# ODD2/DFD-CLIP

Hardware: AMD Instinct MI355X
Metric: 1-sec clips/sec (30x224x224 frames) ViT-B/16 (higher is better)
Workload: dtype bf16

## Files before the change

### dfd-clip_amd/build.py

```python
import hashlib
import os
import shutil
import subprocess
import sys
from concurrent.futures import ThreadPoolExecutor

PKG_DIR = os.path.dirname(os.path.abspath(__file__))
CSRC = os.path.join(PKG_DIR, "csrc")
OBJ_DIR = os.path.join(CSRC, "build")
LIB_PATH = os.path.join(PKG_DIR, "libdfdclip_hip.so")
INCLUDE = os.path.join(os.path.dirname(PKG_DIR), "include")
ARCH = "gfx950"
FLAGS = ["-O3", "-fPIC", "-std=c++17", f"--offload-arch={ARCH}", "-Wall", "-Wno-unused-function"]
NO_SCRATCH = {"gemm256e.hip": "gemm256e_kernel", "attention_mfma_xrow.hip": "attn_mfma_xrow_kernel"}


def _hipcc():
    exe = shutil.which("hipcc") or "/opt/rocm/bin/hipcc"
    if not os.path.exists(exe):
        raise RuntimeError("hipcc not found: the HIP kernels cannot be built")
    return exe


def sources():
    return sorted(f for f in os.listdir(CSRC) if f.endswith(".hip"))


def _digest(paths):
    h = hashlib.sha256()
    for p in paths:
        with open(p, "rb") as f:
            h.update(f.read())
    h.update(" ".join(FLAGS).encode())
    return h.hexdigest()


def scratch_users(report, kernel_substr):
    import re
    out, name = {}, None
    for line in report.splitlines():
        m = re.search(r"remark: Function Name: (\S+)", line)
        if m:
            name = m.group(1)
            continue
        m = re.search(r"ScratchSize \[bytes/lane\]: (\d+)", line)
        if m and name and kernel_substr in name and int(m.group(1)) > 0:
            out[name] = int(m.group(1))
    return out


def build(force=False, verbose=False, extra_flags=()):
    os.makedirs(OBJ_DIR, exist_ok=True)
    hipcc = _hipcc()
    headers = [os.path.join(CSRC, f) for f in sorted(os.listdir(CSRC)) if f.endswith(".hpp")]
    headers.append(os.path.join(INCLUDE, "dfdclip.h"))
    headers.append(os.path.join(INCLUDE, "dfdclip_ext.h"))
    headers.append(os.path.join(INCLUDE, "dfdclip_explain.h"))
    jobs, objs = [], []
    for src in sources():
        sp = os.path.join(CSRC, src)
        obj = os.path.join(OBJ_DIR, src[:-4] + ".o")
        stamp = obj + ".sha"
        dig = _digest([sp] + headers) + " ".join(extra_flags)
        objs.append(obj)
        if not force and os.path.exists(obj) and os.path.exists(stamp) and open(stamp).read() == dig:
            continue
        jobs.append((sp, obj, stamp, dig))

    def compile_one(job):
        sp, obj, stamp, dig = job
        guard = NO_SCRATCH.get(os.path.basename(sp))
        cmd = [hipcc, *FLAGS, *extra_flags, *(["-Rpass-analysis=kernel-resource-usage"] if guard else []), "-c", sp, "-o", obj]
        r = subprocess.run(cmd, capture_output=True, text=True)
        if r.returncode != 0:
            raise RuntimeError(f"hipcc failed for {sp}:\n{r.stderr}")
        if guard:
            bad = scratch_users(r.stderr, guard)
            if bad:
                raise RuntimeError(f"{sp}: kernels with hand-counted vmcnt waits must not use scratch, but: {bad}")
        elif verbose and r.stderr.strip():
            print(r.stderr, file=sys.stderr)
        with open(stamp, "w") as f:
            f.write(dig)
        return sp

    if jobs:
        with ThreadPoolExecutor(max_workers=min(6, len(jobs))) as ex:
            for done in ex.map(compile_one, jobs):
                if verbose:
                    print("built", os.path.basename(done))
    if jobs or not os.path.exists(LIB_PATH):
        r = subprocess.run([hipcc, "-shared", "-fPIC", f"--offload-arch={ARCH}", "-o", LIB_PATH, *objs],
                           capture_output=True, text=True)
        if r.returncode != 0:
            raise RuntimeError(f"link failed:\n{r.stderr}")
    return LIB_PATH


if __name__ == "__main__":
    print(build(force="--force" in sys.argv, verbose=True))
```

### dfd-clip_amd/capi.py

```python
import ctypes
import os
from ctypes import POINTER, Structure, c_char_p, c_double, c_float, c_int, c_int32, c_int64, c_size_t, c_uint32, c_void_p

import torch

PKG_DIR = os.path.dirname(os.path.abspath(__file__))
LIB_PATH = os.path.join(PKG_DIR, "libdfdclip_hip.so")

F32, BF16 = 0, 1
EPI_BIAS, EPI_BIAS_QUICKGELU, EPI_BIAS_RESIDUAL, EPI_PATCH_EMBED, EPI_QKV_EXPORT, EPI_RESIDUAL_POS, EPI_BIAS_GELU = range(7)
ABI_VERSION = 17

_DTYPE = {torch.float32: F32, torch.bfloat16: BF16}
FP8 = 2
FP8_MAX = 448.0
FP8_MIN_ROWS = 1024


class DfdError(RuntimeError):
    pass


GEMM_STREAM_OUT = 1
GEMM_SPARE_IF_FREE = 2


class GemmExtra(Structure):
    _fields_ = [("pos", c_void_p), ("cls", c_void_p), ("k_export", c_void_p), ("v_export", c_void_p),
                ("tokens", c_int32), ("frames_per_clip", c_int32), ("residual", c_void_p), ("qkv_first", c_int32),
                ("drop_rng", c_void_p), ("drop_site", c_uint32), ("drop_p", c_float), ("flags", c_uint32)]


OPTIM_SGD, OPTIM_ADAMW = 0, 1


class OptimExtra(Structure):
    _fields_ = [("kind", c_int32), ("reserved", c_int32), ("beta1", c_double), ("beta2", c_double), ("eps", c_double),
                ("step", c_int64), ("exp_avg_sq", c_void_p)]


class DropoutDesc(Structure):
    _fields_ = [("rng_state", c_void_p), ("site", c_uint32), ("p", c_float)]


class Dropout:
    __slots__ = ("rng", "site", "p")

    def __init__(self, rng, site, p):
        assert rng.is_cuda and rng.dtype == torch.int64 and rng.numel() == 2 and 0.0 <= p < 1.0
        self.rng, self.site, self.p = rng, int(site), float(p)

    def desc(self):
        return DropoutDesc(self.rng.data_ptr(), self.site, self.p)


def _drop(d):
    return ctypes.byref(d.desc()) if d is not None and d.p > 0 else None


SIGNATURES = {
    "dfd_last_error": (c_char_p, []),
    "dfd_abi_version": (c_int, []),
    "dfd_gemm_last_path": (c_int, []),
    "dfd_gemm_set_variant": (c_int, [c_int]),
    "dfd_dropout": (c_int, [c_void_p, c_int, c_void_p, c_int, c_int64, POINTER(DropoutDesc), c_void_p]),
    "dfd_device_check": (c_int, []),
    "dfd_layernorm": (c_int, [c_void_p, c_int64, c_void_p, c_void_p, c_void_p, c_int64, c_int, c_int64, c_int, c_float, c_float, c_void_p]),
    "dfd_layernorm2": (c_int, [c_void_p, c_int64, c_void_p, c_void_p, c_void_p, c_void_p, c_void_p, c_int64, c_int, c_int64, c_int, c_float,
                               c_float, c_void_p]),
    "dfd_add_layernorm": (c_int, [c_void_p, c_int64, c_void_p, c_void_p, c_int64, c_int, c_int, c_void_p, c_void_p, c_void_p, c_int64,
                                  c_int, c_int64, c_int, c_float, c_float, c_void_p]),
    "dfd_patchify": (c_int, [c_void_p, c_void_p, c_int, c_int, c_int, c_int, c_int, c_void_p]),
    "dfd_preprocess_u8": (c_int, [c_void_p, c_int, c_int, c_int, c_int, c_int, c_int, POINTER(c_float), POINTER(c_float),
                                  c_void_p, c_int, c_int, c_int, c_void_p]),
    "dfd_preprocess_geometry": (c_int, [c_int, c_int, c_int, POINTER(c_int), POINTER(c_int), POINTER(c_int), POINTER(c_int)]),
    "dfd_gemm": (c_int, [c_void_p, c_int64, c_void_p, c_int64, c_int, c_void_p, c_int64, c_int, c_void_p, c_int,
                         POINTER(GemmExtra), c_int64, c_int, c_int, c_void_p]),
    "dfd_gemm_fp8": (c_int, [c_void_p, c_int64, c_void_p, c_int64, c_void_p, c_int64, c_int, c_void_p, c_void_p, c_float, c_int,
                             POINTER(GemmExtra), c_int64, c_int, c_int, c_void_p]),
    "dfd_gemm_at_b_workspace": (c_size_t, [c_int64, c_int, c_int, c_int]),
    "dfd_gemm_at_b": (c_int, [c_void_p, c_int64, c_void_p, c_int64, c_int, c_void_p, c_int64, c_int, c_int, c_void_p, c_void_p]),
    "dfd_adapter_norm_gelu": (c_int, [c_void_p, c_int, c_void_p, c_int, c_void_p, c_void_p, c_int, c_int, c_int, c_int, c_float,
                                      c_void_p]),
    "dfd_attention_fwd": (c_int, [c_void_p, c_int64, c_void_p, c_int64, c_int, c_int, c_int, c_int, c_int, c_float, c_void_p]),
    "dfd_linear_rows": (c_int, [c_void_p, c_int64, c_void_p, c_void_p, c_void_p, c_int64, c_int, c_int, c_int, c_int, c_void_p]),
    "dfd_linear_rows_t_workspace": (c_size_t, [c_int, c_int, c_int]),
    "dfd_linear_rows_t": (c_int, [c_void_p, c_int64, c_void_p, c_void_p, c_void_p, c_int64, c_void_p, c_int64, c_int, c_int, c_int, c_int, c_void_p,
                                  c_void_p]),
    "dfd_decoder_attn_workspace": (c_size_t, [c_int, c_int, c_int, c_int]),
    "dfd_decoder_attn_fwd": (c_int, [c_void_p, c_void_p, c_void_p, c_int, c_void_p, c_void_p, c_void_p, c_void_p, c_void_p, c_void_p,
                                     c_void_p, c_int, c_int, c_int, c_int, c_int, c_int, c_void_p]),
    "dfd_decoder_attn_modes_fwd": (c_int, [c_void_p, c_void_p, c_int, c_void_p, c_void_p, c_int, c_void_p, c_void_p, c_int, c_int, c_int,
                                           c_int, c_int, c_void_p]),
    "dfd_decoder_attn_modes_bwd": (c_int, [c_void_p, c_void_p, c_int, c_void_p, c_void_p, c_int, c_void_p, c_void_p, c_int, c_int, c_int,
                                           c_int, c_int, c_void_p]),
    "dfd_decoder_attn_bwd_workspace": (c_size_t, [c_int, c_int, c_int, c_int]),
    "dfd_decoder_attn_bwd": (c_int, [c_void_p, c_void_p, c_void_p, c_int, c_void_p, c_void_p, c_void_p, c_void_p, c_void_p, c_void_p,
                                     c_void_p, c_void_p, c_void_p, c_void_p, c_void_p, c_int, c_void_p, c_int, c_int, c_int, c_int,
                                     c_int, c_void_p]),
    "dfd_adapter_norm_gelu_bwd_workspace": (c_size_t, [c_int, c_int, c_int, c_int]),
    "dfd_adapter_norm_gelu_bwd": (c_int, [c_void_p, c_int, c_void_p, c_void_p, c_int, c_void_p, c_void_p, c_void_p, c_void_p, c_void_p,
                                          c_int, c_int, c_int, c_int, c_float, c_void_p]),
    "dfd_linear_rows_bwd_weight": (c_int, [c_void_p, c_int64, c_void_p, c_int64, c_void_p, c_void_p, c_int, c_int, c_int, c_void_p]),
    "dfd_transpose_f32": (c_int, [c_void_p, c_void_p, c_int, c_int, c_void_p]),
    "dfd_sgd_blocks": (c_int64, [c_int64, c_int, c_int, c_int]),
    "dfd_sgd_step": (c_int, [c_void_p, c_int, c_int64, c_float, c_float, c_float, c_int, c_void_p, POINTER(OptimExtra)]),
    "dfd_layernorm_bwd": (c_int, [c_void_p, c_int64, c_void_p, c_void_p, c_int64, c_void_p, c_int64, c_void_p, c_void_p, c_void_p,
                                  c_int, c_int, c_float, c_int, c_void_p]),
    "dfd_quickgelu": (c_int, [c_void_p, c_void_p, c_void_p, c_int64, POINTER(DropoutDesc), c_void_p]),
    "dfd_head_bwd": (c_int, [c_void_p, c_void_p, c_void_p, c_void_p, c_void_p, c_void_p, c_void_p, c_void_p, c_int, c_int, c_int,
                             c_void_p]),
    "dfd_head_fwd": (c_int, [c_void_p, c_int64, c_void_p, c_void_p, c_void_p, c_void_p, c_void_p, c_void_p, c_int, c_int,
                             c_int, c_float, POINTER(DropoutDesc), c_void_p]),
    "dfd_adapter_bn_workspace": (c_size_t, [c_int64, c_int, c_int]),
    "dfd_adapter_bn_stats": (c_int, [c_void_p, c_int, c_void_p, c_void_p, c_void_p, c_void_p, c_void_p, c_int64, c_int, c_int, c_int,
                                     c_int, c_float, c_float, c_void_p]),
    "dfd_adapter_bn_apply": (c_int, [c_void_p, c_int, c_void_p, c_void_p, c_int, c_void_p, c_void_p, c_void_p, c_void_p,
                                     POINTER(DropoutDesc), c_int64, c_int, c_int, c_int, c_void_p]),
    "dfd_adapter_bn_bwd": (c_int, [c_void_p, c_void_p, c_int, c_void_p, c_int, c_void_p, c_void_p, c_void_p, c_void_p,
                                   POINTER(DropoutDesc), c_void_p, c_int64, c_int, c_int, c_int, c_int, c_void_p]),
    "dfd_gelu_erf": (c_int, [c_void_p, c_int, c_void_p, c_int, c_int64, POINTER(DropoutDesc), c_void_p]),
    "dfd_gelu_erf_bwd": (c_int, [c_void_p, c_int, c_void_p, c_int, c_void_p, c_int, c_int64, POINTER(DropoutDesc), c_void_p]),
    "dfd_compinv_loss_workspace": (c_size_t, [c_int, c_int]),
    "dfd_compinv_loss_fwd": (c_int, [c_void_p, c_void_p, c_int, c_int, c_int, c_int, c_int, c_int, c_void_p, c_void_p, c_void_p,
                                     c_void_p, c_void_p]),
    "dfd_compinv_loss_bwd": (c_int, [c_void_p, c_void_p, c_int, c_int, c_int, c_int, c_int, c_int, c_void_p, c_void_p, c_void_p,
                                     c_void_p, c_void_p, c_void_p]),
}

EXT_SIGNATURES = {
    "dfd_layernorm_dual": (c_int, [c_void_p, c_int64, c_void_p, c_void_p, c_void_p, c_int64, c_void_p, c_int64, c_int64, c_int, c_float,
                                   c_float, c_void_p]),
    "dfd_layernorm2_dual": (c_int, [c_void_p, c_int64, c_void_p, c_void_p, c_void_p, c_void_p, c_void_p, c_int64, c_void_p, c_int64,
                                    c_int64, c_int, c_float, c_float, c_void_p]),
    "dfd_add_layernorm_dual": (c_int, [c_void_p, c_int64, c_void_p, c_void_p, c_int64, c_int, c_int, c_void_p, c_void_p, c_void_p, c_int64,
                                       c_void_p, c_int64, c_int64, c_int, c_float, c_float, c_void_p]),
}

EXPLAIN_SIGNATURES = {
    "dfd_decoder_attn_map": (c_int, [c_void_p, c_void_p, c_int, c_void_p, c_void_p, c_void_p, c_void_p, c_void_p, c_void_p, c_int, c_int,
                                     c_int, c_int, c_int, c_void_p]),
}

HOOK_SIGNATURES = {
    "dfd_attention_set_variant": (c_int, [c_int]),
}

_lib = None


def load_library(path=None):
    global _lib
    if _lib is not None and path is None:
        return _lib
    path = path or LIB_PATH
    if not os.path.exists(path):
        raise DfdError(f"{path} not found: the HIP kernel library is not built and there is no fallback path")
    lib = ctypes.CDLL(path)
    for name, (res, args) in {**SIGNATURES, **EXT_SIGNATURES, **EXPLAIN_SIGNATURES, **HOOK_SIGNATURES}.items():
        try:
            fn = getattr(lib, name)
        except AttributeError:
            raise DfdError(f"{path} does not export {name}")
        fn.restype = res
        fn.argtypes = args
    if lib.dfd_abi_version() != ABI_VERSION:
        raise DfdError(f"{path}: ABI version {lib.dfd_abi_version()} != {ABI_VERSION}")
    _lib = lib
    return lib


def _check(rc, what):
    if rc != 0:
        raise DfdError(f"{what} failed ({rc}): {load_library().dfd_last_error().decode()}")


def _stream():
    return c_void_p(torch._C._cuda_getCurrentRawStream(torch._C._cuda_getDevice()))


def _ptr(t):
    return c_void_p(t.data_ptr()) if t is not None else c_void_p(0)


def _dev(*tensors):
    for t in tensors:
        if t is not None and not t.is_cuda:
            raise DfdError("HIP kernels need device tensors; got a CPU tensor (there is no CPU path)")


def _out_dtype(t):
    return FP8 if t.element_size() == 1 else _DTYPE[t.dtype]


def layernorm(x, gamma, beta, out, eps=1e-5, out_inv_scale=0.0):
    _dev(x, gamma, beta, out)
    assert x.dtype == torch.float32 and x.dim() == 2 and out.shape == x.shape
    assert x.stride(1) == 1 and out.stride(1) == 1
    _check(load_library().dfd_layernorm(_ptr(x), x.stride(0), _ptr(gamma), _ptr(beta), _ptr(out), out.stride(0),
                                        _out_dtype(out), x.shape[0], x.shape[1], eps, float(out_inv_scale), _stream()), "dfd_layernorm")
    return out


def layernorm2(x, gamma_a, beta_a, gamma_b, beta_b, out, eps=1e-5, out_inv_scale=0.0):
    _dev(x, gamma_a, beta_a, gamma_b, beta_b, out)
    assert x.dtype == torch.float32 and x.dim() == 2 and x.stride(1) == 1 and out.stride(1) == 1 and out.shape == x.shape
    _check(load_library().dfd_layernorm2(_ptr(x), x.stride(0), _ptr(gamma_a), _ptr(beta_a), _ptr(gamma_b), _ptr(beta_b), _ptr(out),
                                         out.stride(0), _out_dtype(out), x.shape[0], x.shape[1], eps, float(out_inv_scale), _stream()),
           "dfd_layernorm2")
    return out


def add_layernorm(x, delta, gamma, beta, out, eps=1e-5, delta2=None, store_x=True, out_inv_scale=0.0):
    _dev(x, delta, gamma, beta, out, delta2)
    assert x.dtype == torch.float32 and x.dim() == 2 and out.shape == x.shape and delta.shape == x.shape
    assert x.stride(1) == 1 and out.stride(1) == 1 and delta.stride(1) == 1
    assert delta2 is None or (delta2.dtype == delta.dtype and delta2.shape == x.shape and delta2.stride() == delta.stride())
    _check(load_library().dfd_add_layernorm(_ptr(x), x.stride(0), _ptr(delta), _ptr(delta2), delta.stride(0), _DTYPE[delta.dtype],
                                            int(bool(store_x)), _ptr(gamma), _ptr(beta), _ptr(out), out.stride(0), _out_dtype(out),
                                            x.shape[0], x.shape[1], eps, float(out_inv_scale), _stream()), "dfd_add_layernorm")
    return out


def _dual_outputs(x, out16, out8, out8_inv_scale):
    assert out16.dtype == torch.bfloat16 and out8.element_size() == 1 and out16.shape == x.shape and out8.shape == x.shape
    assert out16.stride(1) == 1 and out8.stride(1) == 1 and out8_inv_scale > 0


def layernorm_dual(x, gamma, beta, out16, out8, out8_inv_scale, eps=1e-5):
    _dev(x, gamma, beta, out16, out8)
    assert x.dtype == torch.float32 and x.dim() == 2 and x.stride(1) == 1
    _dual_outputs(x, out16, out8, out8_inv_scale)
    _check(load_library().dfd_layernorm_dual(_ptr(x), x.stride(0), _ptr(gamma), _ptr(beta), _ptr(out16), out16.stride(0), _ptr(out8),
                                             out8.stride(0), x.shape[0], x.shape[1], eps, float(out8_inv_scale), _stream()),
           "dfd_layernorm_dual")
    return out16, out8


def layernorm2_dual(x, gamma_a, beta_a, gamma_b, beta_b, out16, out8, out8_inv_scale, eps=1e-5):
    _dev(x, gamma_a, beta_a, gamma_b, beta_b, out16, out8)
    assert x.dtype == torch.float32 and x.dim() == 2 and x.stride(1) == 1
    _dual_outputs(x, out16, out8, out8_inv_scale)
    _check(load_library().dfd_layernorm2_dual(_ptr(x), x.stride(0), _ptr(gamma_a), _ptr(beta_a), _ptr(gamma_b), _ptr(beta_b), _ptr(out16),
                                              out16.stride(0), _ptr(out8), out8.stride(0), x.shape[0], x.shape[1], eps,
                                              float(out8_inv_scale), _stream()), "dfd_layernorm2_dual")
    return out16, out8


def add_layernorm_dual(x, delta, gamma, beta, out16, out8, out8_inv_scale, eps=1e-5, delta2=None, store_x=True):
    _dev(x, delta, gamma, beta, out16, out8, delta2)
    assert x.dtype == torch.float32 and x.dim() == 2 and delta.shape == x.shape and x.stride(1) == 1 and delta.stride(1) == 1
    assert delta2 is None or (delta2.dtype == delta.dtype and delta2.shape == x.shape and delta2.stride() == delta.stride())
    _dual_outputs(x, out16, out8, out8_inv_scale)
    _check(load_library().dfd_add_layernorm_dual(_ptr(x), x.stride(0), _ptr(delta), _ptr(delta2), delta.stride(0), _DTYPE[delta.dtype],
                                                 int(bool(store_x)), _ptr(gamma), _ptr(beta), _ptr(out16), out16.stride(0), _ptr(out8),
                                                 out8.stride(0), x.shape[0], x.shape[1], eps, float(out8_inv_scale), _stream()),
           "dfd_add_layernorm_dual")
    return out16, out8


def patchify(frames, out, res, patch):
    _dev(frames, out)
    assert frames.dtype == torch.float32 and frames.is_contiguous() and out.is_contiguous()
    n = frames.shape[0]
    _check(load_library().dfd_patchify(_ptr(frames), _ptr(out), _DTYPE[out.dtype], n, res, patch, out.shape[1], _stream()),
           "dfd_patchify")
    return out


def preprocess_geometry(in_h, in_w, res):
    v = [c_int() for _ in range(4)]
    _check(load_library().dfd_preprocess_geometry(in_h, in_w, res, *[ctypes.byref(i) for i in v]), "dfd_preprocess_geometry")
    return tuple(i.value for i in v)


def preprocess_u8(frames, out, res, patch, mean, std, antialias=True, patch_rows=True):
    _dev(frames, out)
    assert frames.dtype == torch.uint8 and frames.dim() == 4 and frames.shape[1] == 3
    assert frames.is_contiguous() and out.is_contiguous()
    n, _, h, w = frames.shape
    m3 = (c_float * 3)(*[float(v) for v in mean])
    s3 = (c_float * 3)(*[float(v) for v in std])
    if patch_rows:
        assert out.dim() == 2 and out.shape[0] == n * (res // patch) ** 2
        kpad = out.shape[1]
    else:
        assert tuple(out.shape) == (n, 3, res, res)
        kpad = 0
    _check(load_library().dfd_preprocess_u8(_ptr(frames), n, h, w, res, patch, int(bool(antialias)), m3, s3, _ptr(out),
                                            _DTYPE[out.dtype], 1 if patch_rows else 0, kpad, _stream()), "dfd_preprocess_u8")
    return out


_profile = {"epilogue": None, "events": [], "base": None}


def profile_gemm(epilogue=None):
    _profile["epilogue"] = epilogue
    _profile["events"] = []
    _profile["base"] = None
    if epilogue is not None:
        _profile["base"] = torch.cuda.Event(enable_timing=True)
        _profile["base"].record()


def profile_gemm_collect():
    base = _profile["base"]
    spans = [(base.elapsed_time(a), base.elapsed_time(b), flops) for a, b, flops in _profile["events"]]
    profile_gemm(None)
    return spans


def gemm(a, w, c, bias=None, epilogue=EPI_BIAS, m=None, pos=None, cls=None, k_export=None, v_export=None, tokens=0,
         frames_per_clip=0, residual=None, qkv_first=0, drop=None, stream_out=False, spare_cus=0, tile_blocks=0, spare_if_free=False):
    _dev(a, w, c, bias, pos, cls, k_export, v_export, residual)
    assert a.dtype == w.dtype and a.stride(1) == 1 and w.stride(1) == 1 and c.stride(1) == 1
    M = a.shape[0] if m is None else m
    N, K = w.shape
    assert a.shape[1] == K
    assert residual is None or (residual.dtype == c.dtype and residual.stride(0) == c.stride(0))
    assert drop is None or epilogue == EPI_RESIDUAL_POS
    assert 0 <= epilogue <= EPI_BIAS_GELU, f"unknown epilogue {epilogue}"
    extra = GemmExtra(_ptr(pos).value, _ptr(cls).value, _ptr(k_export).value, _ptr(v_export).value, tokens, frames_per_clip,
                      _ptr(residual).value, qkv_first, drop.rng.data_ptr() if drop is not None and drop.p > 0 else None,
                      drop.site if drop is not None else 0, drop.p if drop is not None else 0.0, (GEMM_STREAM_OUT if stream_out else 0) | (GEMM_SPARE_IF_FREE if spare_if_free else 0) | ((int(spare_cus) & 0xff) << 8) | ((int(tile_blocks) & 0xf) << 16))
    timed = _profile["epilogue"] == epilogue
    if timed:
        e0, e1 = torch.cuda.Event(enable_timing=True), torch.cuda.Event(enable_timing=True)
        e0.record()
    _check(load_library().dfd_gemm(_ptr(a), a.stride(0), _ptr(w), w.stride(0), _DTYPE[a.dtype], _ptr(c), c.stride(0),
                                   _DTYPE[c.dtype], _ptr(bias), epilogue, ctypes.byref(extra), M, N, K, _stream()), "dfd_gemm")
    if timed:
        e1.record()
        _profile["events"].append((e0, e1, 2.0 * M * N * K))
    return c


def gemm_fp8(a, w, c, col_scale, bias=None, epilogue=EPI_BIAS, m=None, out_inv_scale=0.0, pos=None, k_export=None, v_export=None,
             tokens=0, frames_per_clip=0, qkv_first=0, stream_out=False, spare_cus=0, spare_if_free=False):
    _dev(a, w, c, col_scale, bias, pos, k_export, v_export)
    assert a.element_size() == 1 and w.element_size() == 1 and a.stride(1) == 1 and w.stride(1) == 1 and c.stride(1) == 1
    assert col_scale.dtype == torch.float32 and col_scale.is_contiguous()
    M = a.shape[0] if m is None else m
    N, K = w.shape
    assert a.shape[1] == K and col_scale.numel() == N
    c_dtype = FP8 if c.element_size() == 1 else _DTYPE[c.dtype]
    extra = GemmExtra(_ptr(pos).value, None, _ptr(k_export).value, _ptr(v_export).value, tokens, frames_per_clip, None, qkv_first,
                      None, 0, 0.0, (GEMM_STREAM_OUT if stream_out else 0) | (GEMM_SPARE_IF_FREE if spare_if_free else 0) | ((int(spare_cus) & 0xff) << 8))
    timed = _profile["epilogue"] == epilogue
    if timed:
        e0, e1 = torch.cuda.Event(enable_timing=True), torch.cuda.Event(enable_timing=True)
        e0.record()
    _check(load_library().dfd_gemm_fp8(_ptr(a), a.stride(0), _ptr(w), w.stride(0), _ptr(c), c.stride(0), c_dtype, _ptr(col_scale),
                                       _ptr(bias), float(out_inv_scale), epilogue, ctypes.byref(extra), M, N, K, _stream()),
           "dfd_gemm_fp8")
    if timed:
        e1.record()
        _profile["events"].append((e0, e1, 2.0 * M * N * K))
    return c


def gemm_set_variant(variant):
    return load_library().dfd_gemm_set_variant(int(variant))


def gemm_last_path():
    return load_library().dfd_gemm_last_path()


def gemm_at_b_workspace_bytes(R, Ma, Nb, dtype):
    return load_library().dfd_gemm_at_b_workspace(R, Ma, Nb, _DTYPE[dtype])


def gemm_at_b(a, b, c, workspace):
    _dev(a, b, c, workspace)
    assert a.dtype == b.dtype and a.stride(1) == 1 and b.stride(1) == 1 and c.is_contiguous() and c.dtype == torch.float32
    R, Ma = a.shape
    Nb = b.shape[1]
    assert b.shape[0] == R and tuple(c.shape) == (Ma, Nb)
    assert workspace.numel() * workspace.element_size() >= gemm_at_b_workspace_bytes(R, Ma, Nb, a.dtype)
    _check(load_library().dfd_gemm_at_b(_ptr(a), a.stride(0), _ptr(b), b.stride(0), _DTYPE[a.dtype], _ptr(c), R, Ma, Nb,
                                        _ptr(workspace), _stream()), "dfd_gemm_at_b")
    return c


def adapter_norm_gelu(a, y, weight, bias, frames, patches, x, joint, eps=1e-5):
    _dev(a, y, weight, bias)
    assert (a.dtype == y.dtype or a.dtype == torch.float32) and a.is_contiguous() and y.is_contiguous()
    assert weight.is_contiguous() and bias.is_contiguous()
    _check(load_library().dfd_adapter_norm_gelu(_ptr(a), _DTYPE[a.dtype], _ptr(y), _DTYPE[y.dtype], _ptr(weight), _ptr(bias), frames,
                                                patches, x, int(joint), eps, _stream()), "dfd_adapter_norm_gelu")
    return y


def adapter_norm_gelu_bwd_workspace_bytes(frames, patches, x, joint):
    return load_library().dfd_adapter_norm_gelu_bwd_workspace(frames, patches, x, int(joint))


def adapter_norm_gelu_bwd(a, dy, da, weight, bias, dweight, dbias, workspace, frames, patches, x, joint, eps=1e-5):
    _dev(a, dy, da, weight, bias, dweight, dbias, workspace)
    assert dy.dtype == da.dtype and (a.dtype == dy.dtype or a.dtype == torch.float32)
    assert a.is_contiguous() and dy.is_contiguous() and da.is_contiguous()
    _check(load_library().dfd_adapter_norm_gelu_bwd(_ptr(a), _DTYPE[a.dtype], _ptr(dy), _ptr(da), _DTYPE[dy.dtype], _ptr(weight), _ptr(bias),
                                                    _ptr(dweight), _ptr(dbias), _ptr(workspace), frames, patches, x, int(joint),
                                                    eps, _stream()), "dfd_adapter_norm_gelu_bwd")
    return da


def attention_set_variant(variant):
    return load_library().dfd_attention_set_variant(int(variant))


def attention_fwd(qkv, out, n_frames, tokens, heads, head_dim=64):
    _dev(qkv, out)
    assert qkv.dtype == out.dtype and qkv.stride(1) == 1 and out.stride(1) == 1
    _check(load_library().dfd_attention_fwd(_ptr(qkv), qkv.stride(0), _ptr(out), out.stride(0), _DTYPE[qkv.dtype], n_frames,
                                            tokens, heads, head_dim, head_dim ** -0.5, _stream()), "dfd_attention_fwd")
    return out


def linear_rows(x, w, bias, y, epilogue=EPI_BIAS):
    _dev(x, w, bias, y)
    assert x.dtype == torch.float32 and w.dtype == torch.float32 and y.dtype == torch.float32
    assert x.stride(1) == 1 and y.stride(1) == 1 and w.is_contiguous()
    B, K = x.shape
    N = w.shape[0]
    _check(load_library().dfd_linear_rows(_ptr(x), x.stride(0), _ptr(w), _ptr(bias), _ptr(y), y.stride(0), epilogue, B, N, K,
                                          _stream()), "dfd_linear_rows")
    return y


def linear_rows_t_workspace_bytes(B, N, K):
    return load_library().dfd_linear_rows_t_workspace(B, N, K)


def linear_rows_t(x, wt, bias, y, workspace, epilogue=EPI_BIAS, residual=None):
    _dev(x, wt, bias, y, workspace, residual)
    assert residual is None or (residual.dtype == torch.float32 and residual.stride(1) == 1 and residual.shape == y.shape)
    assert x.dtype == torch.float32 and wt.dtype == torch.float32 and y.dtype == torch.float32
    assert x.stride(1) == 1 and y.stride(1) == 1 and wt.is_contiguous()
    B, K = x.shape
    N = wt.shape[1]
    assert wt.shape[0] == K and workspace.numel() * workspace.element_size() >= linear_rows_t_workspace_bytes(B, N, K)
    _check(load_library().dfd_linear_rows_t(_ptr(x), x.stride(0), _ptr(wt), _ptr(bias), _ptr(residual),
                                            residual.stride(0) if residual is not None else 0, _ptr(y), y.stride(0), epilogue, B, N, K,
                                            _ptr(workspace), _stream()), "dfd_linear_rows_t")
    return y


def decoder_attn_workspace_bytes(B, heads, d, splits):
    return load_library().dfd_decoder_attn_workspace(B, heads, d, splits)


class KvLayoutDesc(ctypes.Structure):
    _fields_ = [("row_stride", c_int64), ("frame_stride", c_int64), ("pos", c_void_p)]


def _kv_layout(x, other, pos, B, T, patches, D):
    if other is not None:
        assert other.dtype == x.dtype and other.shape == x.shape and other.stride() == x.stride()
    if x.is_contiguous() and pos is None:
        assert x.numel() == B * T * patches * D
        return None, None
    if x.is_contiguous():
        rs, fs = D, patches * D
    else:
        assert x.dim() == 3 and x.shape == (B * T, patches, D) and x.stride(2) == 1, "strided K/V must be [B*T, patches, D] views"
        fs, rs = x.stride(0), x.stride(1)
    if pos is not None:
        assert pos.dtype == torch.float32 and pos.is_contiguous() and pos.shape == (T, D) and pos.device == x.device
    lay = KvLayoutDesc(rs, fs, pos.data_ptr() if pos is not None else None)
    return ctypes.byref(lay), lay


def decoder_attn_fwd(q, k, v, frame_mask, mix, stats, workspace, splits, B, T, patches, heads, d=64, mix_softmax=None,
                     ext_weights=None, pos=None):
    _dev(q, k, v, frame_mask, mix, stats, workspace, mix_softmax, ext_weights)
    assert q.dtype == torch.float32 and q.is_contiguous()
    assert frame_mask.dtype == torch.uint8 and frame_mask.is_contiguous()
    assert ext_weights is None or (ext_weights.is_contiguous() and ext_weights.numel() == B * heads * T * patches)
    lay, _keep = _kv_layout(k, v, pos, B, T, patches, heads * d)
    _check(load_library().dfd_decoder_attn_fwd(_ptr(q), _ptr(k), _ptr(v), _DTYPE[k.dtype], lay, _ptr(frame_mask), _ptr(ext_weights),
                                               _ptr(mix), _ptr(mix_softmax), _ptr(stats), _ptr(workspace), splits, B, T, patches,
                                               heads, d, _stream()),
           "dfd_decoder_attn_fwd")
    return mix


ATTN_MODE_BITS = {"frame": 1, "temporal": 2}


def decoder_attn_modes_fwd(q, k, frame_mask, modes, scores, weights, B, T, patches, heads, d=64, pos=None):
    _dev(q, k, frame_mask, scores, weights)
    assert q.is_contiguous() and scores.is_contiguous() and weights.is_contiguous()
    assert scores.numel() == B * heads * T * patches == weights.numel()
    lay, _keep = _kv_layout(k, None, pos, B, T, patches, heads * d)
    _check(load_library().dfd_decoder_attn_modes_fwd(_ptr(q), _ptr(k), _DTYPE[k.dtype], lay, _ptr(frame_mask), modes, _ptr(scores),
                                                     _ptr(weights), B, T, patches, heads, d, _stream()),
           "dfd_decoder_attn_modes_fwd")
    return weights


def decoder_attn_map(q, k, frame_mask, stats, aff, B, T, patches, heads, d=64, ext_weights=None, branches=None, pos=None):
    _dev(q, k, frame_mask, stats, aff, ext_weights, branches)
    assert q.dtype == torch.float32 and q.is_contiguous()
    assert frame_mask.dtype == torch.uint8 and frame_mask.is_contiguous()
    n = B * heads * T * patches
    assert aff.dtype == torch.float32 and aff.is_contiguous() and aff.numel() == n
    assert stats is None or (stats.dtype == torch.float32 and stats.is_contiguous() and stats.numel() == B * heads * 2)
    assert ext_weights is None or (ext_weights.dtype == torch.float32 and ext_weights.is_contiguous() and ext_weights.numel() == n)
    assert branches is None or (branches.dtype == torch.float32 and branches.is_contiguous() and branches.numel() == 2 * n)
    lay, _keep = _kv_layout(k, None, pos, B, T, patches, heads * d)
    _check(load_library().dfd_decoder_attn_map(_ptr(q), _ptr(k), _DTYPE[k.dtype], lay, _ptr(frame_mask), _ptr(stats), _ptr(ext_weights),
                                               _ptr(aff), _ptr(branches), B, T, patches, heads, d, _stream()),
           "dfd_decoder_attn_map")
    return aff


def decoder_attn_modes_bwd(scores, v, dmix, modes, dwv_ws, dscores, B, T, patches, heads, d=64, pos=None):
    _dev(scores, v, dmix, dwv_ws, dscores)
    assert scores.is_contiguous() and dmix.is_contiguous()
    assert dwv_ws.numel() >= B * heads * T * patches and dscores.numel() == B * heads * T * patches
    lay, _keep = _kv_layout(v, None, pos, B, T, patches, heads * d)
    _check(load_library().dfd_decoder_attn_modes_bwd(_ptr(scores), _ptr(v), _DTYPE[v.dtype], lay, _ptr(dmix), modes, _ptr(dwv_ws),
                                                     _ptr(dscores), B, T, patches, heads, d, _stream()),
           "dfd_decoder_attn_modes_bwd")
    return dscores


def head_fwd(x, gamma, beta, proj, feat, raw, logits, eps=1e-5, drop=None):
    _dev(x, gamma, beta, proj, feat, raw, logits)
    B, D = x.shape
    assert proj.is_contiguous() and proj.shape[0] == D and feat.is_contiguous()
    _check(load_library().dfd_head_fwd(_ptr(x), x.stride(0), _ptr(gamma), _ptr(beta), _ptr(proj), _ptr(feat), _ptr(raw),
                                       _ptr(logits), B, D, proj.shape[1], eps, _drop(drop), _stream()), "dfd_head_fwd")
    return logits



BN_EVAL, BN_TRAIN, BN_TRAIN_UPDATE = 0, 1, 2


def adapter_bn_workspace_bytes(frames, patches, width):
    return load_library().dfd_adapter_bn_workspace(frames, patches, width)


def _bn_shape(t, frames, patches, width):
    assert t.is_contiguous() and t.numel() == frames * patches * width, (tuple(t.shape), frames, patches, width)


def adapter_bn_stats(y, stats, workspace, frames, patches, T, mode, running_mean=None, running_var=None,
                     num_batches_tracked=None, momentum=0.1, eps=1e-5):
    _dev(y, stats, workspace, running_mean, running_var, num_batches_tracked)
    width = y.shape[-1]
    _bn_shape(y, frames, patches, width)
    assert stats.dtype == torch.float32 and stats.is_contiguous() and stats.numel() == 2 * T
    for b in (running_mean, running_var):
        assert b is None or (b.dtype == torch.float32 and b.is_contiguous() and b.numel() == T)
    assert num_batches_tracked is None or num_batches_tracked.dtype == torch.int64
    assert workspace.numel() * workspace.element_size() >= adapter_bn_workspace_bytes(frames, patches, width)
    _check(load_library().dfd_adapter_bn_stats(_ptr(y), _DTYPE[y.dtype], _ptr(stats), _ptr(running_mean), _ptr(running_var),
                                               _ptr(num_batches_tracked), _ptr(workspace), frames, patches, width, T, int(mode),
                                               momentum, eps, _stream()), "dfd_adapter_bn_stats")
    return stats


def adapter_bn_apply(y, out, frames, patches, T, stats=None, gamma=None, beta=None, residual=None, pos=None, drop=None):
    _dev(y, out, stats, gamma, beta, residual, pos)
    width = y.shape[-1]
    _bn_shape(y, frames, patches, width)
    _bn_shape(out, frames, patches, width)
    assert residual is None or (residual.dtype == out.dtype and residual.is_contiguous() and residual.numel() == out.numel())
    assert pos is None or (pos.dtype == torch.float32 and pos.is_contiguous() and pos.numel() == T * width)
    _check(load_library().dfd_adapter_bn_apply(_ptr(y), _DTYPE[y.dtype], _ptr(residual), _ptr(out), _DTYPE[out.dtype], _ptr(stats),
                                               _ptr(gamma), _ptr(beta), _ptr(pos), _drop(drop), frames, patches, width, T,
                                               _stream()), "dfd_adapter_bn_apply")
    return out


def adapter_bn_bwd(y, dout, dy, stats, gamma, dgamma, dbeta, workspace, frames, patches, T, train, drop=None):
    _dev(y, dout, dy, stats, gamma, dgamma, dbeta, workspace)
    width = y.shape[-1]
    for t in (y, dout, dy):
        _bn_shape(t, frames, patches, width)
    assert dy.dtype == y.dtype and dout.dtype in (y.dtype, torch.float32)
    assert workspace.numel() * workspace.element_size() >= adapter_bn_workspace_bytes(frames, patches, width)
    _check(load_library().dfd_adapter_bn_bwd(_ptr(y), _ptr(dout), _DTYPE[dout.dtype], _ptr(dy), _DTYPE[y.dtype], _ptr(stats),
                                             _ptr(gamma), _ptr(dgamma), _ptr(dbeta), _drop(drop), _ptr(workspace), frames,
                                             patches, width, T, int(bool(train)), _stream()), "dfd_adapter_bn_bwd")
    return dy


def gelu_erf(a, out, drop=None):
    _dev(a, out)
    assert a.is_contiguous() and out.is_contiguous() and a.numel() == out.numel()
    _check(load_library().dfd_gelu_erf(_ptr(a), _DTYPE[a.dtype], _ptr(out), _DTYPE[out.dtype], a.numel(), _drop(drop), _stream()),
           "dfd_gelu_erf")
    return out


def gelu_erf_bwd(a, dh, da, drop=None):
    _dev(a, dh, da)
    assert a.is_contiguous() and dh.is_contiguous() and da.is_contiguous() and a.numel() == dh.numel() == da.numel()
    assert dh.dtype == da.dtype
    _check(load_library().dfd_gelu_erf_bwd(_ptr(a), _DTYPE[a.dtype], _ptr(dh), _DTYPE[dh.dtype], _ptr(da), _DTYPE[da.dtype], a.numel(),
                                           _drop(drop), _stream()), "dfd_gelu_erf_bwd")
    return da


def dropout(x, out, drop):
    _dev(x, out)
    assert x.is_contiguous() and out.is_contiguous() and x.numel() == out.numel() and drop is not None
    _check(load_library().dfd_dropout(_ptr(x), _DTYPE[x.dtype], _ptr(out), _DTYPE[out.dtype], x.numel(),
                                      ctypes.byref(drop.desc()), _stream()), "dfd_dropout")
    return out



def decoder_attn_bwd_workspace_bytes(B, T, heads, d=64):
    return load_library().dfd_decoder_attn_bwd_workspace(B, T, heads, d)


def decoder_attn_bwd(q, k, v, frame_mask, dmix, mix_softmax, stats, dq, dpos, workspace, B, T, patches, heads, d=64, dk=None,
                     dv=None, ext_weights=None, ext_dscores=None, pos=None):
    _dev(q, k, v, frame_mask, dmix, mix_softmax, stats, dq, dpos, workspace, dk, dv, ext_weights, ext_dscores)
    assert q.is_contiguous() and dmix.is_contiguous()
    assert mix_softmax is None or mix_softmax.is_contiguous()
    lay, _keep = _kv_layout(k, v, pos, B, T, patches, heads * d)
    _check(load_library().dfd_decoder_attn_bwd(_ptr(q), _ptr(k), _ptr(v), _DTYPE[k.dtype], lay, _ptr(frame_mask), _ptr(dmix),
                                               _ptr(mix_softmax), _ptr(stats), _ptr(ext_weights), _ptr(ext_dscores), _ptr(dq),
                                               _ptr(dpos), _ptr(dk), _ptr(dv),
                                               _DTYPE[dk.dtype] if dk is not None else F32, _ptr(workspace), B, T, patches,
                                               heads, d, _stream()), "dfd_decoder_attn_bwd")
    return dq


def linear_rows_bwd_weight(dy, x, dw, db=None):
    _dev(dy, x, dw, db)
    assert dy.stride(1) == 1 and x.stride(1) == 1 and dw.is_contiguous()
    B, N = dy.shape
    K = x.shape[1]
    assert tuple(dw.shape) == (N, K)
    _check(load_library().dfd_linear_rows_bwd_weight(_ptr(dy), dy.stride(0), _ptr(x), x.stride(0), _ptr(dw), _ptr(db), B, N, K,
                                                     _stream()), "dfd_linear_rows_bwd_weight")
    return dw


def transpose(src, dst):
    _dev(src, dst)
    assert src.is_contiguous() and dst.is_contiguous() and src.dtype == torch.float32
    R, C = src.shape
    _check(load_library().dfd_transpose_f32(_ptr(src), _ptr(dst), R, C, _stream()), "dfd_transpose_f32")
    return dst


def sgd_blocks(numel, rows=0, cols=0, mirrored=False):
    return int(load_library().dfd_sgd_blocks(int(numel), int(rows), int(cols), 1 if mirrored else 0))


def adamw_extra(beta1, beta2, eps, step, exp_avg_sq):
    _dev(exp_avg_sq)
    assert exp_avg_sq.dtype == torch.int64 and exp_avg_sq.is_contiguous() and exp_avg_sq.dim() == 1
    return OptimExtra(OPTIM_ADAMW, 0, float(beta1), float(beta2), float(eps), int(step), exp_avg_sq.data_ptr())


def sgd_step(table, n, total_blocks, lr, momentum, weight_decay, first_step, extra=None):
    _dev(table)
    assert table.dtype == torch.int64 and table.is_contiguous() and table.shape == (n, 7)
    _check(load_library().dfd_sgd_step(_ptr(table), int(n), int(total_blocks), float(lr), float(momentum), float(weight_decay),
                                       1 if first_step else 0, _stream(), None if extra is None else ctypes.byref(extra)), "dfd_sgd_step")


def layernorm_bwd(x, gamma, dy, dx, dgamma, dbeta, xhat_ws, accumulate_dx=False, eps=1e-5):
    _dev(x, gamma, dy, dx, dgamma, dbeta, xhat_ws)
    rows, cols = x.shape
    _check(load_library().dfd_layernorm_bwd(_ptr(x), x.stride(0), _ptr(gamma), _ptr(dy), dy.stride(0), _ptr(dx), dx.stride(0),
                                            _ptr(dgamma), _ptr(dbeta), _ptr(xhat_ws), rows, cols, eps, int(accumulate_dx),
                                            _stream()), "dfd_layernorm_bwd")
    return dx


def quickgelu(u, out, du=None, drop=None):
    _dev(u, out, du)
    assert u.is_contiguous() and out.is_contiguous() and (du is None or du.is_contiguous())
    _check(load_library().dfd_quickgelu(_ptr(u), _ptr(du), _ptr(out), u.numel(), _drop(drop), _stream()), "dfd_quickgelu")
    return out


def head_bwd(raw, dlogits, proj, feat, dfeat_ext, dz, dfeat, dproj):
    _dev(raw, dlogits, proj, feat, dfeat_ext, dz, dfeat, dproj)
    B, od = raw.shape
    D = proj.shape[0]
    assert dlogits.is_contiguous() and proj.is_contiguous() and feat.is_contiguous()
    _check(load_library().dfd_head_bwd(_ptr(raw), _ptr(dlogits), _ptr(proj), _ptr(feat), _ptr(dfeat_ext), _ptr(dz), _ptr(dfeat),
                                       _ptr(dproj), B, D, od, _stream()), "dfd_head_bwd")
    return dfeat



def compinv_loss_workspace_bytes(P, D):
    return int(load_library().dfd_compinv_loss_workspace(int(P), int(D)))


def _compinv_check(k, v, B, T, P, L):
    assert k.dtype == v.dtype and k.shape == v.shape and k.is_contiguous() and v.is_contiguous()
    assert k.dim() == 3 and k.shape[0] == L and k.shape[1] == B * T * P, (tuple(k.shape), B, T, P, L)


def compinv_loss_fwd(k, v, B, T, P, workspace, match, norm, recon=None):
    _dev(k, v, workspace, match, norm, recon)
    L, _, D = k.shape
    _compinv_check(k, v, B, T, P, L)
    assert workspace.dtype == torch.float32 and workspace.numel() * 4 >= compinv_loss_workspace_bytes(P, D)
    assert match.dtype == norm.dtype == torch.float32 and (recon is None or recon.dtype == torch.float32)
    _check(load_library().dfd_compinv_loss_fwd(_ptr(k), _ptr(v), _DTYPE[k.dtype], B, T, P, D, L, _ptr(workspace), _ptr(match),
                                               _ptr(norm), _ptr(recon), _stream()), "dfd_compinv_loss_fwd")
    return match


def compinv_loss_bwd(k, v, B, T, P, workspace, norm, grad, dk, dv):
    _dev(k, v, workspace, norm, grad, dk, dv)
    L, _, D = k.shape
    _compinv_check(k, v, B, T, P, L)
    assert dk.dtype == dv.dtype == k.dtype and dk.shape == dv.shape == k.shape and dk.is_contiguous() and dv.is_contiguous()
    assert grad.dtype == norm.dtype == torch.float32 and grad.numel() == 1 and norm.numel() == 1
    _check(load_library().dfd_compinv_loss_bwd(_ptr(k), _ptr(v), _DTYPE[k.dtype], B, T, P, D, L, _ptr(workspace), _ptr(norm),
                                               _ptr(grad), _ptr(dk), _ptr(dv), _stream()), "dfd_compinv_loss_bwd")
    return dk, dv
```

### dfd-clip_amd/csrc/gemm.hip

```cpp
#include "gemm_args.hpp"
#include "gelu.hpp"

namespace {

constexpr int BM = 128, BN = 128;
constexpr int ROW_BYTES = 64;
constexpr int ROW_STRIDE = 80;
constexpr int TILE_BYTES = BM * ROW_STRIDE;
constexpr int EPI_SPLITK_SLAB = 100;

template <typename CT> __device__ __forceinline__ void store_c(void* C, int64_t off, float v) {
  static_cast<CT*>(C)[off] = from_f32<CT>(v);
}

template <typename CT, int EPI>
__device__ __forceinline__ void epilogue_elem(const GemmArgs& a, int64_t m, int n, float acc) {
  if (m >= a.M || n >= a.N) return;
  if constexpr (EPI == DFD_EPI_BIAS) {
    store_c<CT>(a.C, m * a.ldc + n, acc + (a.bias ? a.bias[n] : 0.f));
  } else if constexpr (EPI == DFD_EPI_BIAS_QUICKGELU) {
    store_c<CT>(a.C, m * a.ldc + n, quick_gelu(acc + (a.bias ? a.bias[n] : 0.f)));
  } else if constexpr (EPI == DFD_EPI_BIAS_GELU) {
    store_c<CT>(a.C, m * a.ldc + n, gelu_erf(acc + (a.bias ? a.bias[n] : 0.f)));
  } else if constexpr (EPI == DFD_EPI_BIAS_RESIDUAL) {
    float* c = static_cast<float*>(a.C) + m * a.ldc + n;
    *c = *c + (acc + (a.bias ? a.bias[n] : 0.f));
  } else if constexpr (EPI == DFD_EPI_PATCH_EMBED) {
    const int P = a.tokens - 1;
    const int64_t frame = m / P;
    const int p = (int)(m - frame * P);
    float* c = static_cast<float*>(a.C);
    c[(frame * a.tokens + 1 + p) * a.ldc + n] = acc + a.pos[(int64_t)(1 + p) * a.N + n];
    if (p == 0) c[(frame * a.tokens) * a.ldc + n] = a.cls[n] + a.pos[n];
  } else if constexpr (EPI == DFD_EPI_RESIDUAL_POS) {
    const int64_t frame = m / (a.tokens - 1);
    const float p = a.pos ? a.pos[(frame % a.frames_per_clip) * a.N + n] : 0.f;
    CT* c = static_cast<CT*>(a.C) + m * a.ldc + n;
    const CT* rsd = a.residual ? static_cast<const CT*>(a.residual) + m * a.ldc + n : c;
    *c = from_f32<CT>(to_f32(*rsd) + dfd_drop_one(a.drop, (uint64_t)m * a.N + n, acc) + p);
  } else if constexpr (EPI == DFD_EPI_QKV_EXPORT) {
    const float v = acc + (a.bias ? a.bias[n] : 0.f);
    store_c<CT>(a.C, m * a.ldc + n, v);
    const int D = a.N / (3 - a.qkv_first);
    const int ne = n + a.qkv_first * D;
    if (a.k_export != nullptr && ne >= D) {
      const int64_t frame = m / a.tokens;
      const int tok = (int)(m - frame * a.tokens);
      if (tok > 0) {
        const bool is_v = ne >= 2 * D;
        const int cc = ne - (is_v ? 2 * D : D);
        const float e = v + (a.pos ? a.pos[(frame % a.frames_per_clip) * D + cc] : 0.f);
        store_c<CT>(is_v ? a.v_export : a.k_export, (frame * (a.tokens - 1) + tok - 1) * D + cc, e);
      }
    }
  }
}

template <typename T, typename CT, int EPI>
__global__ __launch_bounds__(256) void gemm128_kernel(const GemmArgs a) {
  __shared__ __attribute__((aligned(16))) unsigned char smem[4 * TILE_BYTES];
  const int tid = threadIdx.x;
  const int lane = tid & 63, wave = tid >> 6;
  const int r = lane & 31, h = lane >> 5;
  const int wm = wave >> 1, wn = wave & 1;
  const int64_t m0 = (int64_t)blockIdx.y * BM;
  const int n0 = blockIdx.x * BN;
  constexpr int KSTEP = ROW_BYTES / (int)sizeof(T);
  const int nk_all = a.K / KSTEP;
  const int per = (nk_all + (int)gridDim.z - 1) / (int)gridDim.z;
  const int kt0 = (int)blockIdx.z * per;
  const int nk = min(per, nk_all - kt0) > 0 ? min(per, nk_all - kt0) : 0;

  const unsigned char* Ab = static_cast<const unsigned char*>(a.A);
  const unsigned char* Wb = static_cast<const unsigned char*>(a.W);
  uint4 ra[2], rb[2];
  int srow[2], scol[2];
  bool va[2], vb[2];
  const unsigned char* pa[2];
  const unsigned char* pb[2];
#pragma unroll
  for (int i = 0; i < 2; ++i) {
    const int c = tid + 256 * i;
    srow[i] = c >> 2;
    scol[i] = (c & 3) * 16;
    va[i] = (m0 + srow[i]) < a.M;
    vb[i] = (n0 + srow[i]) < a.N;
    pa[i] = Ab + ((m0 + srow[i]) * a.lda) * (int64_t)sizeof(T) + scol[i];
    pb[i] = Wb + ((int64_t)(n0 + srow[i]) * a.ldw) * (int64_t)sizeof(T) + scol[i];
  }
  auto load_tile = [&](int kt) {
#pragma unroll
    for (int i = 0; i < 2; ++i) {
      ra[i] = va[i] ? *reinterpret_cast<const uint4*>(pa[i] + (int64_t)(kt0 + kt) * ROW_BYTES) : uint4{0, 0, 0, 0};
      rb[i] = vb[i] ? *reinterpret_cast<const uint4*>(pb[i] + (int64_t)(kt0 + kt) * ROW_BYTES) : uint4{0, 0, 0, 0};
    }
  };
  auto store_tile = [&](int buf) {
#pragma unroll
    for (int i = 0; i < 2; ++i) {
      *reinterpret_cast<uint4*>(smem + buf * TILE_BYTES + srow[i] * ROW_STRIDE + scol[i]) = ra[i];
      *reinterpret_cast<uint4*>(smem + (2 + buf) * TILE_BYTES + srow[i] * ROW_STRIDE + scol[i]) = rb[i];
    }
  };

  f32x16 acc[2][2];
#pragma unroll
  for (int i = 0; i < 2; ++i)
#pragma unroll
    for (int j = 0; j < 2; ++j)
#pragma unroll
      for (int e = 0; e < 16; ++e) acc[i][j][e] = 0.f;

  if (nk > 0) {
    load_tile(0);
    store_tile(0);
  }
  __syncthreads();
  for (int kt = 0; kt < nk; ++kt) {
    const int buf = kt & 1;
    if (kt + 1 < nk) load_tile(kt + 1);
    const unsigned char* As = smem + buf * TILE_BYTES + (wm * 64 + r) * ROW_STRIDE;
    const unsigned char* Bs = smem + (2 + buf) * TILE_BYTES + (wn * 64 + r) * ROW_STRIDE;
    if constexpr (sizeof(T) == 2) {
#pragma unroll
      for (int s = 0; s < 2; ++s) {
        bf16x8 fa[2], fb[2];
#pragma unroll
        for (int i = 0; i < 2; ++i) {
          fa[i] = *reinterpret_cast<const bf16x8*>(As + i * 32 * ROW_STRIDE + s * 32 + h * 16);
          fb[i] = *reinterpret_cast<const bf16x8*>(Bs + i * 32 * ROW_STRIDE + s * 32 + h * 16);
        }
#pragma unroll
        for (int i = 0; i < 2; ++i)
#pragma unroll
          for (int j = 0; j < 2; ++j) acc[i][j] = __builtin_amdgcn_mfma_f32_32x32x16_bf16(fa[i], fb[j], acc[i][j], 0, 0, 0);
      }
    } else {
      f32x4 fa[2][2], fb[2][2];
#pragma unroll
      for (int i = 0; i < 2; ++i)
#pragma unroll
        for (int q = 0; q < 2; ++q) {
          fa[i][q] = *reinterpret_cast<const f32x4*>(As + i * 32 * ROW_STRIDE + h * 32 + q * 16);
          fb[i][q] = *reinterpret_cast<const f32x4*>(Bs + i * 32 * ROW_STRIDE + h * 32 + q * 16);
        }
#pragma unroll
      for (int s = 0; s < 8; ++s)
#pragma unroll
        for (int i = 0; i < 2; ++i)
#pragma unroll
          for (int j = 0; j < 2; ++j)
            acc[i][j] = __builtin_amdgcn_mfma_f32_32x32x2f32(fa[i][s >> 2][s & 3], fb[j][s >> 2][s & 3], acc[i][j], 0, 0, 0);
    }
    if (kt + 1 < nk) store_tile(buf ^ 1);
    __syncthreads();
  }

#pragma unroll
  for (int i = 0; i < 2; ++i)
#pragma unroll
    for (int j = 0; j < 2; ++j)
#pragma unroll
      for (int e = 0; e < 16; ++e) {
        const int64_t m = m0 + wm * 64 + i * 32 + (e & 3) + 8 * (e >> 2) + 4 * h;
        const int n = n0 + wn * 64 + j * 32 + r;
        if constexpr (EPI == EPI_SPLITK_SLAB) {
          if (m < a.M && n < a.N) static_cast<float*>(a.C)[((int64_t)blockIdx.z * a.M + m) * a.ldc + n] = acc[i][j][e];
        } else {
          epilogue_elem<CT, EPI>(a, m, n, acc[i][j][e]);
        }
      }
}

template <typename T, typename CT>
int launch_gemm128(const GemmArgs& a, int epi, hipStream_t st) {
  const dim3 grid((a.N + BN - 1) / BN, (unsigned)((a.M + BM - 1) / BM)), block(256);
#define EPI_CASE(E)                                                                    \
  case E:                                                                              \
    hipLaunchKernelGGL((gemm128_kernel<T, CT, E>), grid, block, 0, st, a);             \
    break;
  switch (epi) {
    EPI_CASE(DFD_EPI_BIAS)
    EPI_CASE(DFD_EPI_BIAS_QUICKGELU)
    EPI_CASE(DFD_EPI_BIAS_GELU)
    EPI_CASE(DFD_EPI_QKV_EXPORT)
    EPI_CASE(DFD_EPI_RESIDUAL_POS)
    default:
      if constexpr (sizeof(CT) == 4) {
        switch (epi) {
          EPI_CASE(DFD_EPI_BIAS_RESIDUAL)
          EPI_CASE(DFD_EPI_PATCH_EMBED)
          default:
            dfd_set_error("dfd_gemm: unknown epilogue %d", epi);
            return DFD_ERR_INVALID_ARG;
        }
      } else {
        dfd_set_error("dfd_gemm: epilogue %d needs an f32 C", epi);
        return DFD_ERR_INVALID_ARG;
      }
  }
#undef EPI_CASE
  DFD_CHECK_LAUNCH("dfd_gemm");
  return DFD_OK;
}

template <typename T>
__global__ __launch_bounds__(256) void transpose_pad_kernel(const T* __restrict__ src, int64_t lds_, T* __restrict__ dst, int64_t R,
                                                            int C, int64_t Rp) {
  __shared__ T tile[32][33];
  const int c0 = blockIdx.x * 32;
  const int64_t r0 = (int64_t)blockIdx.y * 32;
  const int tx = threadIdx.x & 31, ty = threadIdx.x >> 5;
  for (int i = ty; i < 32; i += 8) tile[i][tx] = (r0 + i < R && c0 + tx < C) ? src[(r0 + i) * lds_ + c0 + tx] : from_f32<T>(0.f);
  __syncthreads();
  for (int i = ty; i < 32; i += 8)
    if (c0 + i < C && r0 + tx < Rp) dst[(int64_t)(c0 + i) * Rp + r0 + tx] = tile[tx][i];
}

__global__ void slab_reduce_kernel(const float* __restrict__ slabs, float* __restrict__ out, int64_t n, int splits) {
  const int64_t i = (int64_t)blockIdx.x * blockDim.x + threadIdx.x;
  if (i >= n) return;
  float s = 0.f;
  for (int z = 0; z < splits; ++z) s += slabs[(int64_t)z * n + i];
  out[i] = s;
}

void at_b_plan(int64_t R, int Ma, int Nb, int64_t* Rp, int* splits) {
  const int tiles = ((Ma + BM - 1) / BM) * ((Nb + BN - 1) / BN);
  int sp = (1024 + tiles - 1) / tiles;
  const int64_t steps = (R + 31) / 32;
  if (sp > steps / 8) sp = (int)(steps / 8 > 0 ? steps / 8 : 1);
  if (sp > 512) sp = 512;
  *splits = sp;
  *Rp = (R + 31) / 32 * 32;
}

template <typename T>
int launch_at_b(const void* A, int64_t lda, const void* B, int64_t ldb, float* C, int64_t R, int Ma, int Nb, void* workspace,
                hipStream_t st) {
  int64_t Rp;
  int splits;
  at_b_plan(R, Ma, Nb, &Rp, &splits);
  T* At = static_cast<T*>(workspace);
  T* Bt = At + (int64_t)Ma * Rp;
  size_t off = (size_t)(Ma + Nb) * Rp * sizeof(T);
  off = (off + 255) / 256 * 256;
  float* slabs = reinterpret_cast<float*>(static_cast<unsigned char*>(workspace) + off);
  const dim3 tb(256);
  hipLaunchKernelGGL((transpose_pad_kernel<T>), dim3((Ma + 31) / 32, (unsigned)(Rp / 32)), tb, 0, st, static_cast<const T*>(A), lda, At, R, Ma, Rp);
  hipLaunchKernelGGL((transpose_pad_kernel<T>), dim3((Nb + 31) / 32, (unsigned)(Rp / 32)), tb, 0, st, static_cast<const T*>(B), ldb, Bt, R, Nb, Rp);
  GemmArgs a{};
  a.A = At; a.W = Bt; a.C = slabs; a.lda = Rp; a.ldw = Rp; a.ldc = Nb; a.M = Ma; a.N = Nb; a.K = (int)Rp;
  const dim3 grid((Nb + BN - 1) / BN, (Ma + BM - 1) / BM, splits);
  hipLaunchKernelGGL((gemm128_kernel<T, float, EPI_SPLITK_SLAB>), grid, tb, 0, st, a);
  const int64_t n = (int64_t)Ma * Nb;
  hipLaunchKernelGGL(slab_reduce_kernel, dim3((unsigned)((n + 255) / 256)), tb, 0, st, slabs, C, n, splits);
  DFD_CHECK_LAUNCH("dfd_gemm_at_b");
  return DFD_OK;
}

}

static int fill_extra(GemmArgs& a, int epilogue, const dfd_gemm_extra* extra, int c_dtype, int64_t ldc, int64_t M, int N) {
  if (epilogue == DFD_EPI_PATCH_EMBED) {
    DFD_REQUIRE(extra && extra->pos && extra->cls && extra->tokens > 1, "dfd_gemm: PATCH_EMBED needs extra.pos, extra.cls, extra.tokens");
    DFD_REQUIRE(M % (extra->tokens - 1) == 0, "dfd_gemm: PATCH_EMBED M=%lld is not a whole number of frames", (long long)M);
    DFD_REQUIRE(c_dtype == DFD_F32 && ldc >= N, "dfd_gemm: PATCH_EMBED writes an f32 token matrix");
  } else {
    DFD_REQUIRE(ldc >= N, "dfd_gemm: ldc=%lld < N", (long long)ldc);
  }
  if (epilogue == DFD_EPI_QKV_EXPORT) {
    DFD_REQUIRE(extra && extra->tokens > 1 && (extra->qkv_first == 0 || extra->qkv_first == 1) && N % (3 - extra->qkv_first) == 0,
                "dfd_gemm: QKV_EXPORT needs extra.tokens, qkv_first in {0, 1} and N a multiple of the column blocks present");
    DFD_REQUIRE(M % extra->tokens == 0, "dfd_gemm: QKV_EXPORT M=%lld is not a whole number of frames", (long long)M);
    DFD_REQUIRE(!extra->k_export == !extra->v_export, "dfd_gemm: QKV_EXPORT needs both k_export and v_export or neither");
    DFD_REQUIRE(!extra->pos || extra->frames_per_clip > 0, "dfd_gemm: QKV_EXPORT with pos needs frames_per_clip");
  }
  if (epilogue == DFD_EPI_RESIDUAL_POS) {
    DFD_REQUIRE(extra && extra->tokens > 1, "dfd_gemm: RESIDUAL_POS needs extra.tokens (patches per frame + 1)");
    DFD_REQUIRE(!extra->pos || extra->frames_per_clip > 0, "dfd_gemm: RESIDUAL_POS with pos needs frames_per_clip");
  }
  if (extra) {
    a.pos = extra->pos; a.cls = extra->cls; a.k_export = extra->k_export; a.v_export = extra->v_export;
    a.residual = epilogue == DFD_EPI_RESIDUAL_POS ? extra->residual : nullptr;
    a.tokens = extra->tokens; a.frames_per_clip = extra->frames_per_clip > 0 ? extra->frames_per_clip : 1;
    a.qkv_first = epilogue == DFD_EPI_QKV_EXPORT ? extra->qkv_first : 0;
    a.stream_out = (extra->flags & DFD_GEMM_STREAM_OUT) ? 1 : 0;
    a.spare_cus = (int)((extra->flags >> DFD_GEMM_SPARE_CUS_SHIFT) & 0xff);
    a.spare_if_free = (extra->flags & DFD_GEMM_SPARE_IF_FREE) ? 1 : 0;
    a.tile_rows = 32 * (int)((extra->flags >> DFD_GEMM_TILE_BLOCKS_SHIFT) & 0xf);
    DFD_REQUIRE(a.tile_rows == 0 || a.tile_rows == 224 || a.tile_rows == 256, "dfd_gemm: tile blocks must be 0, 7 or 8");
    if (epilogue == DFD_EPI_RESIDUAL_POS && extra->drop_rng && extra->drop_p > 0.f) {
      DFD_REQUIRE(extra->drop_p < 1.f, "dfd_gemm: drop_p=%f", (double)extra->drop_p);
      const dfd_dropout_t dd{extra->drop_rng, extra->drop_site, extra->drop_p};
      a.drop = dfd_make_drop(&dd);
    }
  }
  return DFD_OK;
}

static thread_local int g_last_path = 0;
static thread_local int g_gemm_variant = 0;
extern "C" int dfd_gemm_last_path(void) { return g_last_path; }
extern "C" int dfd_gemm_set_variant(int variant) {
  const int old = g_gemm_variant;
  g_gemm_variant = variant;
  return old;
}

static int try_persistent_kernels(GemmArgs& a, int c_dtype, int epilogue, bool f8, hipStream_t st, int* path) {
  const int epi_p = epilogue == DFD_EPI_QKV_EXPORT && a.k_export == nullptr ? DFD_EPI_BIAS : epilogue;
  a.no_dynamic = g_gemm_variant != 3;
  int rc = g_gemm_variant == 1 ? 1 : (f8 ? dfd_gemm256e_f8_try : dfd_gemm256e_try)(a, c_dtype, epi_p, st);
  *path = 257;
  if (rc != 1) return rc;
  rc = (f8 ? dfd_gemm256p_f8_try : dfd_gemm256p_try)(a, c_dtype, epi_p, st);
  *path = 256;
  return rc;
}

extern "C" int dfd_gemm(const void* A, int64_t lda, const void* W, int64_t ldw, int ab_dtype, void* C, int64_t ldc,
                        int c_dtype, const float* bias, int epilogue, const dfd_gemm_extra* extra, int64_t M, int N,
                        int K, void* stream) {
  DFD_REQUIRE(A && W && C, "dfd_gemm: null pointer");
  DFD_REQUIRE(M >= 0 && N > 0 && K > 0, "dfd_gemm: bad shape M=%lld N=%d K=%d", (long long)M, N, K);
  DFD_REQUIRE(ab_dtype == DFD_F32 || ab_dtype == DFD_BF16, "dfd_gemm: ab_dtype=%d", ab_dtype);
  DFD_REQUIRE(c_dtype == DFD_F32 || c_dtype == DFD_BF16, "dfd_gemm: c_dtype=%d", c_dtype);
  DFD_REQUIRE(!(ab_dtype == DFD_F32 && c_dtype == DFD_BF16), "dfd_gemm: f32 operands with bf16 output unsupported");
  DFD_REQUIRE(K % 32 == 0, "dfd_gemm: K=%d must be a multiple of 32", K);
  const int esz = ab_dtype == DFD_F32 ? 4 : 2;
  DFD_REQUIRE(lda >= K && ldw >= K && (lda * esz) % 16 == 0 && (ldw * esz) % 16 == 0, "dfd_gemm: lda=%lld ldw=%lld must be >= K and 16-byte multiples", (long long)lda, (long long)ldw);
  DFD_REQUIRE(dfd_aligned16(A) && dfd_aligned16(W), "dfd_gemm: A and W must be 16-byte aligned");
  GemmArgs a{};
  a.A = A; a.W = W; a.C = C; a.bias = bias;
  a.lda = lda; a.ldw = ldw; a.ldc = ldc; a.M = M; a.N = N; a.K = K;
  { const int rc = fill_extra(a, epilogue, extra, c_dtype, ldc, M, N); if (rc != DFD_OK) return rc; }
  if (M == 0) return DFD_OK;
  hipStream_t st = static_cast<hipStream_t>(stream);
  if (ab_dtype == DFD_BF16) {
    int path = 0;
    int rc = try_persistent_kernels(a, c_dtype, epilogue, false, st, &path);
    if (rc == 0) g_last_path = path;
    if (rc <= 0) return rc;
    rc = dfd_gemm256_try(a, c_dtype, epilogue, st);
    if (rc == 0) g_last_path = 256;
    if (rc <= 0) return rc;
  }
  g_last_path = 128;
  if (ab_dtype == DFD_F32) return launch_gemm128<float, float>(a, epilogue, st);
  if (c_dtype == DFD_BF16) return launch_gemm128<bf16_t, bf16_t>(a, epilogue, st);
  return launch_gemm128<bf16_t, float>(a, epilogue, st);
}

extern "C" int dfd_gemm_fp8(const void* A, int64_t lda, const void* W, int64_t ldw, void* C, int64_t ldc, int c_dtype,
                            const float* col_scale, const float* bias, float out_inv_scale, int epilogue,
                            const dfd_gemm_extra* extra, int64_t M, int N, int K, void* stream) {
  DFD_REQUIRE(A && W && C && col_scale, "dfd_gemm_fp8: null pointer");
  DFD_REQUIRE(M >= 0 && N > 0 && K > 0, "dfd_gemm_fp8: bad shape M=%lld N=%d K=%d", (long long)M, N, K);
  DFD_REQUIRE(c_dtype == DFD_BF16 || c_dtype == DFD_FP8, "dfd_gemm_fp8: c_dtype=%d", c_dtype);
  DFD_REQUIRE(epilogue == DFD_EPI_BIAS || epilogue == DFD_EPI_BIAS_QUICKGELU || epilogue == DFD_EPI_BIAS_GELU || epilogue == DFD_EPI_QKV_EXPORT,
              "dfd_gemm_fp8: epilogue %d not served (BIAS, BIAS_QUICKGELU, BIAS_GELU, QKV_EXPORT)", epilogue);
  DFD_REQUIRE(c_dtype == DFD_BF16 || (epilogue != DFD_EPI_QKV_EXPORT && out_inv_scale > 0.f), "dfd_gemm_fp8: fp8 output needs out_inv_scale > 0 and a plain / QuickGELU / GELU epilogue");
  DFD_REQUIRE(lda >= K && ldw >= K && ldc >= N, "dfd_gemm_fp8: leading dimensions");
  GemmArgs a{};
  a.A = A; a.W = W; a.C = C; a.bias = bias; a.col_scale = col_scale; a.out_inv_scale = out_inv_scale;
  a.lda = lda; a.ldw = ldw; a.ldc = ldc; a.M = M; a.N = N; a.K = K;
  { const int rc = fill_extra(a, epilogue, extra, c_dtype, ldc, M, N); if (rc != DFD_OK) return rc; }
  if (M == 0) return DFD_OK;
  int path = 0;
  const int rc = try_persistent_kernels(a, c_dtype, epilogue, true, static_cast<hipStream_t>(stream), &path);
  if (rc == 1) {
    dfd_set_error("dfd_gemm_fp8: shape not served (needs M >= 1024, N %% 256 == 0, K %% 128 == 0, K >= 256, 16-byte aligned rows; got M=%lld N=%d K=%d)",
                  (long long)M, N, K);
    return DFD_ERR_INVALID_ARG;
  }
  return rc;
}

bool dfd_gemm_tn_supported(const void* A, int64_t lda, const void* B, int64_t ldb, int Ma, int Nb);
int dfd_gemm_tn_splits(int64_t R, int Ma, int Nb);
int dfd_gemm_tn_launch(const void* A, int64_t lda, const void* B, int64_t ldb, float* C, int64_t R, int Ma, int Nb,
                       float* slabs, hipStream_t st);

extern "C" size_t dfd_gemm_at_b_workspace(int64_t R, int Ma, int Nb, int dtype) {
  if (R <= 0 || Ma <= 0 || Nb <= 0) return 0;
  int64_t Rp;
  int splits;
  at_b_plan(R, Ma, Nb, &Rp, &splits);
  const size_t esz = dtype == DFD_F32 ? 4 : 2;
  size_t bytes = (size_t)(Ma + Nb) * Rp * esz;
  bytes = (bytes + 255) / 256 * 256;
  bytes += (size_t)splits * Ma * Nb * sizeof(float) + 256;
  if (dtype == DFD_BF16 && Ma % 128 == 0 && Nb % 128 == 0) {
    const size_t tn = (size_t)dfd_gemm_tn_splits(R, Ma, Nb) * Ma * Nb * sizeof(float) + 256;
    if (tn > bytes) bytes = tn;
  }
  return bytes;
}

extern "C" int dfd_gemm_at_b(const void* A, int64_t lda, const void* B, int64_t ldb, int dtype, float* C, int64_t R, int Ma,
                             int Nb, void* workspace, void* stream) {
  DFD_REQUIRE(A && B && C && workspace, "dfd_gemm_at_b: null pointer");
  DFD_REQUIRE(R > 0 && Ma > 0 && Nb > 0 && lda >= Ma && ldb >= Nb, "dfd_gemm_at_b: bad shape");
  DFD_REQUIRE(R < (int64_t)1 << 31, "dfd_gemm_at_b: R too large");
  DFD_REQUIRE(dtype == DFD_F32 || dtype == DFD_BF16, "dfd_gemm_at_b: dtype=%d", dtype);
  DFD_REQUIRE((reinterpret_cast<uintptr_t>(workspace) & 255) == 0, "dfd_gemm_at_b: workspace must be 256-byte aligned");
  hipStream_t st = static_cast<hipStream_t>(stream);
  if (dtype == DFD_BF16 && dfd_gemm_tn_supported(A, lda, B, ldb, Ma, Nb))
    return dfd_gemm_tn_launch(A, lda, B, ldb, C, R, Ma, Nb, static_cast<float*>(workspace), st);
  if (dtype == DFD_F32) return launch_at_b<float>(A, lda, B, ldb, C, R, Ma, Nb, workspace, st);
  return launch_at_b<bf16_t>(A, lda, B, ldb, C, R, Ma, Nb, workspace, st);
}
```

### dfd-clip_amd/csrc/gemm256e.hip

```cpp
#include <mutex>
#include <unordered_map>

#include "gemm256p_common.hpp"

namespace {

constexpr int UNIT = 128 * ROWB;
constexpr int DEPTH = 6;
constexpr int NB = 2 * (DEPTH - 1);

template <int EPI, int RB, bool F8, bool CF8>
__global__ __launch_bounds__(512) void gemm256e_kernel(const GemmArgs a, int tiles_m, int tiles_n) {
  static_assert(!F8 || RB == 8, "fp8 form: 256-row tiles only");
  static_assert(!CF8 || (F8 && EPI != DFD_EPI_QKV_EXPORT), "fp8 output: fp8 operands, plain, QuickGELU or GELU epilogue");
  constexpr int ESZ = F8 ? 1 : 2;
  constexpr int TMU = 32 * RB;
  constexpr int WROWS = 16 * RB;
  constexpr int HB = RB - 4;
  constexpr int NCV = F8 ? 2 : 1;
  constexpr int S1 = CF8 ? RB : 2 * RB;
  constexpr int S2 = 4 * RB;
  __shared__ __attribute__((aligned(1024))) unsigned char smem[RING + 8 * STAGE];
  const int tid = threadIdx.x;
  const int lane = tid & 63;
  const int wave = __builtin_amdgcn_readfirstlane(tid >> 6);
  const int wr = wave >> 2, wc = wave & 3;
  const int ntiles = tiles_m * tiles_n;

  const int G = gridDim.x, bid = blockIdx.x;
  const int xcd = bid & 7, q8 = G >> 3, r8 = G & 7;
  const int pos = xcd_position();

  const OperandSrds<F8, CF8> srd(a);
  const __amdgpu_buffer_rsrc_t srdA = srd.A, srdW = srd.W, srdC = srd.C;
  const v4i srdB = words(a.bias ? a.bias : reinterpret_cast<const float*>(a.W), a.bias ? a.N * 4 : 0);
  [[maybe_unused]] const v4i srdS = words(F8 ? a.col_scale : reinterpret_cast<const float*>(a.W), F8 ? a.N * 4 : 0);
  const int cnt_x = q8 + (xcd < r8 ? 1 : 0), off_x = pos - (bid >> 3);
  const v4i srdT = words(reinterpret_cast<const float*>(a.sched ? a.sched : reinterpret_cast<const uint32_t*>(a.W)), a.sched ? 8 * 128 : 0);

  const uint32_t lda2 = (uint32_t)(a.lda * ESZ), ldw2 = (uint32_t)(a.ldw * ESZ);
  const uint32_t a_last = (uint32_t)(a.M - 1) * lda2;
  uint32_t vA[2][2], vW[2];
  auto set_a = [&](const Tile& t, int ha) {
    int l = lane;
    asm volatile("" : "+v"(l));
    const uint32_t pr = (uint32_t)(l >> 3), pp = (uint32_t)(l & 7);
    const uint32_t ch0 = (pp ^ (pr >> 1)) << 4;
    const uint32_t row0 = ((uint32_t)t.m0 + (uint32_t)(WROWS * (wave >> 2) + 64 * ha + 16 * (wave & 3))) * lda2 + pr * lda2;
    vA[ha][0] = min(row0, a_last) + ch0;
    vA[ha][1] = min(row0 + 8u * lda2, a_last) + (ch0 ^ 64u);
  };
  auto set_w = [&](const Tile& t, int hb) {
    int l = lane;
    asm volatile("" : "+v"(l));
    const uint32_t pr = (uint32_t)(l >> 3), pp = (uint32_t)(l & 7);
    const uint32_t ch0 = (pp ^ (pr >> 1)) << 4;
    vW[hb] = ((uint32_t)t.n0 + (uint32_t)(64 * (wave >> 1) + 32 * hb + 16 * (wave & 1))) * ldw2 + pr * ldw2 + ch0;
  };
  auto issue = [&](int kind, int kr) {
    unsigned char* d = smem + ((kind & 1) ? 0 : 4 * UNIT) + (2 * (kind >> 1) + (kr & 1)) * UNIT + wave * 16 * ROWB;
    if (kind & 1) {
      __builtin_amdgcn_raw_ptr_buffer_load_lds(srdA, (lds_ptr_t)d, 16, vA[kind >> 1][0], kr * ROWB, 0, 0);
      __builtin_amdgcn_raw_ptr_buffer_load_lds(srdA, (lds_ptr_t)(d + 8 * ROWB), 16, vA[kind >> 1][1], kr * ROWB, 0, 0);
    } else {
      __builtin_amdgcn_raw_ptr_buffer_load_lds(srdW, (lds_ptr_t)d, 16, vW[kind >> 1], kr * ROWB, 0, 0);
      __builtin_amdgcn_raw_ptr_buffer_load_lds(srdW, (lds_ptr_t)(d + 8 * ROWB), 16, vW[kind >> 1] ^ 64u, kr * ROWB + 8 * (int)ldw2, 0, 0);
    }
  };

  const unsigned char* rdA[2];
  const unsigned char* rdW[2];
  {
    const int fr = lane & 15, fq = lane >> 4;
    const int sw = (fr >> 1) & 7;
#pragma unroll
    for (int ks = 0; ks < 2; ++ks) {
      const int cs = ((4 * ks + fq) ^ sw) << 4;
      rdA[ks] = smem + (wr * 64 + fr) * ROWB + cs;
      rdW[ks] = smem + 4 * UNIT + (wc * 32 + fr) * ROWB + cs;
    }
  }

  struct Opnd {
    v8i v;
  };
  Opnd Aa[4], X[2], Y[2];
  f32x4 acc[RB][4];
  auto read_op = [&](Opnd& o, const unsigned char* p0, const unsigned char* p1) {
    const v4i x0 = *reinterpret_cast<const v4i*>(p0), x1 = *reinterpret_cast<const v4i*>(p1);
    o.v = v8i{x0[0], x0[1], x0[2], x0[3], x1[0], x1[1], x1[2], x1[3]};
  };
  auto read_a = [&](int slot, int ha) {
#pragma unroll
    for (int i = 0; i < 4; ++i)
      if (ha == 0 || i < HB) read_op(Aa[i], rdA[0] + (2 * ha + slot) * UNIT + i * 16 * ROWB, rdA[1] + (2 * ha + slot) * UNIT + i * 16 * ROWB);
  };
  auto read_w = [&](Opnd (&w)[2], int slot, int hb) {
#pragma unroll
    for (int j = 0; j < 2; ++j) read_op(w[j], rdW[0] + (2 * hb + slot) * UNIT + j * 16 * ROWB, rdW[1] + (2 * hb + slot) * UNIT + j * 16 * ROWB);
  };
  auto chunk = [](const Opnd& o, int ks) {
    return __builtin_bit_cast(bf16x8, ks == 0 ? __builtin_shufflevector(o.v, o.v, 0, 1, 2, 3) : __builtin_shufflevector(o.v, o.v, 4, 5, 6, 7));
  };
  auto quadrant = [&](const Opnd (&w)[2], int ha, int hb) {
    asm volatile("s_waitcnt lgkmcnt(0)" ::: "memory");
    __builtin_amdgcn_sched_barrier(0);
    __builtin_amdgcn_s_setprio(1);
    if constexpr (F8) {
#pragma unroll
      for (int i = 0; i < 4; ++i)
#pragma unroll
        for (int j = 0; j < 2; ++j)
          acc[4 * ha + i][2 * hb + j] = __builtin_amdgcn_mfma_scale_f32_16x16x128_f8f6f4(w[j].v, Aa[i].v, acc[4 * ha + i][2 * hb + j], 0, 0, 0, 0x7f7f7f7f, 0,
                                                                                          0x7f7f7f7f);
#pragma unroll
      for (int i = 0; i < 4; ++i)
#pragma unroll
        for (int j = 0; j < 2; ++j) asm volatile("" : "+v"(acc[4 * ha + i][2 * hb + j]));
    } else {
#pragma unroll
      for (int ks = 0; ks < 2; ++ks)
#pragma unroll
        for (int i = 0; i < (ha == 0 ? 4 : HB); ++i)
#pragma unroll
          for (int j = 0; j < 2; ++j)
            acc[4 * ha + i][2 * hb + j] = __builtin_amdgcn_mfma_f32_16x16x32_bf16(chunk(w[j], ks), chunk(Aa[i], ks), acc[4 * ha + i][2 * hb + j], 0, 0, 0);
    }
    __builtin_amdgcn_s_setprio(0);
    __builtin_amdgcn_sched_barrier(0);
    __builtin_amdgcn_s_barrier();
    __builtin_amdgcn_sched_barrier(0);
  };

  const int nk = a.K / (F8 ? 128 : TK);
  int idx = pos;
  Tile cur = decode_tile(idx, tiles_m, tiles_n, TMU);
  set_a(cur, 0);
  set_a(cur, 1);
  set_w(cur, 0);
  set_w(cur, 1);
#pragma unroll
  for (int v = 0; v <= DEPTH; ++v) issue(v & 3, v >> 2);
  wait_vm<NB>();
  __builtin_amdgcn_s_barrier();
  if (wr == 1) __builtin_amdgcn_s_barrier();
  __builtin_amdgcn_sched_barrier(0);
  int s_prev = 0;

  [[maybe_unused]] unsigned char* const ep = smem + RING + wave * STAGE;
  const int D = EPI == DFD_EPI_QKV_EXPORT ? a.N / (3 - a.qkv_first) : 0;

  const int nk_ = a.K / (F8 ? 128 : TK);
  const bool dyn = !F8 && a.sched != nullptr && nk_ >= 6;
  const bool drawer = dyn && wave == 0;
  for (;;) {
    int nidx = idx + G;
    bool has_next = nidx < ntiles;
    Tile nxt = has_next ? decode_tile(nidx, tiles_m, tiles_n, TMU) : cur;
    uint32_t drawn = 1;
    if (drawer) {
      const uint32_t coff = (uint32_t)(xcd * 128);
      uint64_t saved_exec;
      asm volatile(
          "s_mov_b64 %1, exec\n\t"
          "s_mov_b64 exec, 1\n\t"
          "s_nop 4\n\t"
          "buffer_atomic_add %0, %2, %3, 0 offen sc0\n\t"
          "s_mov_b64 exec, %1"
          : "+v"(drawn), "=&s"(saved_exec)
          : "v"(coff), "s"(srdT)
          : "memory");
    }
#pragma unroll
    for (int i = 0; i < RB; ++i)
#pragma unroll
      for (int j = 0; j < 4; ++j) acc[i][j] = f32x4{0.f, 0.f, 0.f, 0.f};
    read_w(X, 0, 0);
    asm volatile("s_waitcnt lgkmcnt(0)" ::: "memory");
    __builtin_amdgcn_sched_barrier(0);
    float bv;
    [[maybe_unused]] float sv;
    auto load_col_vectors = [&] {
      int lb = lane;
      asm volatile("" : "+v"(lb));
      const uint32_t coff = (uint32_t)((cur.n0 + wc * 64 + lb) * 4);
      const uint32_t boff = a.bias ? coff : 0xffffffffu;
      asm volatile("s_nop 4\n\tbuffer_load_dword %0, %1, %2, 0 offen" : "=&v"(bv) : "v"(boff), "s"(srdB) : "memory");
      if constexpr (F8) asm volatile("s_nop 4\n\tbuffer_load_dword %0, %1, %2, 0 offen" : "=&v"(sv) : "v"(coff), "s"(srdS) : "memory");
    };
    auto park_col_vectors = [&] {
      int lb = lane;
      asm volatile("" : "+v"(lb), "+v"(bv));
      *reinterpret_cast<float*>(ep + lb * 4) = bv;
      if constexpr (F8) {
        asm volatile("" : "+v"(sv));
        *reinterpret_cast<float*>(ep + 256 + lb * 4) = sv;
      }
    };

    auto ktile = [&](int kt, auto par_c, auto head_c, auto end_c) {
      constexpr int PAR = decltype(par_c)::value, HEAD = decltype(head_c)::value, END = decltype(end_c)::value;
      auto seg_tail = [&](auto p_c) {
        constexpr int p = decltype(p_c)::value;
        constexpr int c = p + DEPTH + 1, kind = c & 3, dk = c >> 2;
        constexpr bool wraps = END < dk;
        const int kr = wraps ? dk - END - 1 : kt + dk;
        issue(kind, kr);
        if constexpr (END == dk) {
          if (kind == 0) set_w(nxt, 0);
          else if (kind == 1) set_a(nxt, 0);
          else if (kind == 2) set_w(nxt, 1);
          else set_a(nxt, 1);
        }
        constexpr bool stores_young = HEAD < 2 && 4 * HEAD + p <= DEPTH - 2;
        constexpr bool cv_young = END <= 1 && 4 * (1 - END) + p <= DEPTH - 2;
        if constexpr (stores_young) {
          if (drawer) {
            if (s_prev == 0) wait_vm<NB + 1>();
            else if (EPI != DFD_EPI_QKV_EXPORT || s_prev == S1) wait_vm<NB + S1 + 1>();
            else wait_vm<NB + S2 + 1>();
          } else {
            if (s_prev == 0) wait_vm<NB>();
            else if (EPI != DFD_EPI_QKV_EXPORT || s_prev == S1) wait_vm<NB + S1>();
            else wait_vm<NB + S2>();
          }
        } else {
          wait_vm<NB + (cv_young ? NCV : 0)>();
        }
        if constexpr (HEAD < 2 && 4 * HEAD + p == DEPTH - 1) {
          if (drawer) {
            const uint32_t slot_addr = (uint32_t)(uintptr_t)(lds_ptr_t)(smem + RING + 1024);
            asm volatile("" : "+v"(drawn));
            const uint32_t lane0 = (uint32_t)__builtin_amdgcn_readfirstlane((int)drawn);
            asm volatile("ds_write_b32 %0, %1\n\ts_waitcnt lgkmcnt(0)" ::"v"(slot_addr), "v"(lane0) : "memory");
          }
        }
        if constexpr (END <= 1 && 4 * (1 - END) + p == DEPTH - 1) {
          park_col_vectors();
        }
        __builtin_amdgcn_sched_barrier(0);
        __builtin_amdgcn_s_barrier();
        __builtin_amdgcn_sched_barrier(0);
      };
      using P0 = std::integral_constant<int, 0>;
      using P1 = std::integral_constant<int, 1>;
      using P2 = std::integral_constant<int, 2>;
      using P3 = std::integral_constant<int, 3>;
      if constexpr (END == 1) load_col_vectors();
      read_a(PAR, 0);
      seg_tail(P0{});
      quadrant(PAR ? Y : X, 0, 0);
      read_w(PAR ? X : Y, PAR, 1);
      seg_tail(P1{});
      quadrant(PAR ? X : Y, 0, 1);
      read_a(PAR, 1);
      seg_tail(P2{});
      quadrant(PAR ? X : Y, 1, 1);
      if constexpr (END != 0) read_w(PAR ? X : Y, PAR ^ 1, 0);
      seg_tail(P3{});
      quadrant(PAR ? Y : X, 1, 0);
    };
    using C0 = std::integral_constant<int, 0>;
    using C1 = std::integral_constant<int, 1>;
    using C2 = std::integral_constant<int, 2>;
    using C3 = std::integral_constant<int, 3>;
    using C4 = std::integral_constant<int, 4>;
    bool short_k = false;
    if constexpr (EPI == DFD_EPI_RESIDUAL_POS) short_k = nk == 4;
    if (short_k) {
      if constexpr (EPI == DFD_EPI_RESIDUAL_POS) {
        ktile(0, C0{}, C0{}, C3{});
        ktile(1, C1{}, C1{}, C2{});
        ktile(2, C0{}, C2{}, C1{});
        ktile(3, C1{}, C2{}, C0{});
      }
    } else {
      ktile(0, C0{}, C0{}, C4{});
      ktile(1, C1{}, C1{}, C4{});
      if (dyn) {
        uint32_t n;
        const uint32_t slot_addr = (uint32_t)(uintptr_t)(lds_ptr_t)(smem + RING + 1024);
        asm volatile("ds_read_b32 %0, %1\n\ts_waitcnt lgkmcnt(0)" : "=&v"(n) : "v"(slot_addr) : "memory");
        n = (uint32_t)__builtin_amdgcn_readfirstlane((int)n) - a.sched_base[xcd];
        const uint32_t r = n / (uint32_t)cnt_x;
        has_next = r < (uint32_t)(ntiles / G + 1);
        nidx = (int)((r + 1) * (uint32_t)G + (uint32_t)off_x + (n - r * (uint32_t)cnt_x));
        has_next = has_next && nidx < ntiles;
        nxt = has_next ? decode_tile(nidx, tiles_m, tiles_n, TMU) : cur;
      }
      for (int kt = 2; kt < nk - 4; kt += 2) {
        ktile(kt, C0{}, C2{}, C4{});
        ktile(kt + 1, C1{}, C2{}, C4{});
      }
      ktile(nk - 4, C0{}, C2{}, C3{});
      ktile(nk - 3, C1{}, C2{}, C2{});
      ktile(nk - 2, C0{}, C2{}, C1{});
      ktile(nk - 1, C1{}, C2{}, C0{});
    }

    f32x4 b4[4];
    [[maybe_unused]] f32x4 cs4[4];
    const int le = opaque_lane();
#pragma unroll
    for (int j = 0; j < 4; ++j) {
      b4[j] = *reinterpret_cast<const f32x4*>(ep + (j * 16 + (le >> 4) * 4) * 4);
      if constexpr (F8) cs4[j] = *reinterpret_cast<const f32x4*>(ep + 256 + (j * 16 + (le >> 4) * 4) * 4);
    }
    asm volatile("s_waitcnt lgkmcnt(0)" ::: "memory");
    const int stores = tile_epilogue<EPI, RB, F8, CF8>(a, acc, b4, cs4, ep, cur, wr, wc, le, D, srdC);
    if (!has_next) break;
    s_prev = countable_stores<RB>(stores, cur, wr, a.M);
    idx = nidx;
    cur = nxt;
  }
  wait_vm<0>();
  if (wr == 0) __builtin_amdgcn_s_barrier();
}

struct SchedSlot {
  uint32_t* dev = nullptr;
  uint32_t base[8] = {0, 0, 0, 0, 0, 0, 0, 0};
};

bool sched_prepare(GemmArgs& a, hipStream_t st, int grid, int64_t ntiles) {
  static std::mutex mu;
  static std::unordered_map<hipStream_t, SchedSlot> slots;
  static uint32_t* pool = nullptr;
  static int used = 0;
  constexpr int MAX_SLOTS = 64;
  a.sched = nullptr;
  hipStreamCaptureStatus cap = hipStreamCaptureStatusNone;
  if (hipStreamIsCapturing(st, &cap) != hipSuccess || cap != hipStreamCaptureStatusNone) {
    (void)hipGetLastError();
    return true;
  }
  std::lock_guard<std::mutex> lock(mu);
  auto it = slots.find(st);
  if (it == slots.end()) {
    if (pool == nullptr) {
      if (hipMalloc(reinterpret_cast<void**>(&pool), MAX_SLOTS * 8 * 128) != hipSuccess || hipMemset(pool, 0, MAX_SLOTS * 8 * 128) != hipSuccess) {
        (void)hipGetLastError();
        pool = nullptr;
        return true;
      }
    }
    if (used >= MAX_SLOTS) return true;
    SchedSlot sl;
    sl.dev = pool + used * 8 * 32;
    ++used;
    it = slots.emplace(st, sl).first;
  }
  SchedSlot& sl = it->second;
  a.sched = sl.dev;
  const int q8 = grid >> 3, r8 = grid & 7;
  const int64_t full = ntiles / grid, rem = ntiles % grid;
  for (int x = 0; x < 8; ++x) {
    a.sched_base[x] = sl.base[x];
    const int cnt = q8 + (x < r8 ? 1 : 0);
    const int off = x < r8 ? x * (q8 + 1) : r8 * (q8 + 1) + (x - r8) * q8;
    int64_t last = rem - off;
    last = last < 0 ? 0 : (last > cnt ? cnt : last);
    sl.base[x] += (uint32_t)(full * cnt + last);
  }
  return true;
}

struct Gemm256e {
  static constexpr const char* name = "ping-pong";
  static constexpr bool spare_if_free = true;
  static constexpr bool serves(int epi, bool f8) {
    return epi == DFD_EPI_BIAS || epi == DFD_EPI_BIAS_QUICKGELU || epi == DFD_EPI_BIAS_GELU || epi == DFD_EPI_QKV_EXPORT || (!f8 && epi == DFD_EPI_RESIDUAL_POS);
  }
  static bool depth_ok(const GemmArgs& a, int esz, int nk, int epi) {
    if ((nk < 6 && !(epi == DFD_EPI_RESIDUAL_POS && nk == 4)) || (nk & 1)) return false;
    return (a.ldw * esz) % 128 == 0;
  }
  static void prepare(GemmArgs& a, hipStream_t st, const TilePlan& p, bool f8) {
    if (!f8 && a.K / TK >= 6 && a.no_dynamic == 0) sched_prepare(a, st, p.grid, p.ntiles);
    else a.sched = nullptr;
  }
  template <int EPI, int RB, bool F8, bool CF8>
  static void run(int grid, hipStream_t st, const GemmArgs& a, int tiles_m, int tiles_n) {
    hipLaunchKernelGGL((gemm256e_kernel<EPI, RB, F8, CF8>), dim3(grid), dim3(512), 0, st, a, tiles_m, tiles_n);
  }
};

}

int dfd_gemm256e_try(const GemmArgs& a, int c_dtype, int epi, hipStream_t st) { return try_persistent<Gemm256e, false>(a, c_dtype, epi, st); }

int dfd_gemm256e_f8_try(const GemmArgs& a, int c_dtype, int epi, hipStream_t st) { return try_persistent<Gemm256e, true>(a, c_dtype, epi, st); }
```

### dfd-clip_amd/csrc/gemm256p.hip

```cpp
#include "gemm256p_common.hpp"

namespace {

template <int EPI, int RB, bool F8, bool CF8>
__global__ __launch_bounds__(512) void gemm256p_kernel(const GemmArgs a, int tiles_m, int tiles_n) {
  static_assert(!F8 || RB == 8, "fp8 form: 256-row tiles only");
  static_assert(!CF8 || (F8 && EPI != DFD_EPI_QKV_EXPORT), "fp8 output: fp8 operands, plain, QuickGELU or GELU epilogue");
  constexpr int ESZ = F8 ? 1 : 2;
  constexpr int TMU = 32 * RB;
  constexpr int WROWS = 16 * RB;
  constexpr int HB = RB - 4;
  __shared__ __attribute__((aligned(1024))) unsigned char smem[RING + 8 * STAGE];
  const int tid = threadIdx.x;
  const int lane = tid & 63;
  const int wave = __builtin_amdgcn_readfirstlane(tid >> 6);
  const int wr = wave >> 2, wc = wave & 3;
  const int ntiles = tiles_m * tiles_n;

  const int G = gridDim.x;
  const int pos = xcd_position();

  const OperandSrds<F8, CF8> srd(a);
  const __amdgpu_buffer_rsrc_t srdA = srd.A, srdW = srd.W, srdC = srd.C;
  [[maybe_unused]] const __amdgpu_buffer_rsrc_t srdS = make_srd(F8 ? a.col_scale : reinterpret_cast<const float*>(a.W), F8 ? a.N * 4 : 0);
  const __amdgpu_buffer_rsrc_t srdB = make_srd(a.bias ? a.bias : reinterpret_cast<const float*>(a.W), a.bias ? a.N * 4 : 0);

  uint32_t vA[4], vW[4];
  const uint32_t lda2 = (uint32_t)(a.lda * ESZ), ldw2 = (uint32_t)(a.ldw * ESZ);
  const uint32_t a_last = (uint32_t)(a.M - 1) * lda2;
  auto set_a = [&](const Tile& t) {
    int l = lane;
    asm volatile("" : "+v"(l));
    const uint32_t pr = (uint32_t)(l >> 3), pp = (uint32_t)(l & 7);
    const uint32_t ch0 = (pp ^ (pr >> 1)) << 4;
    const uint32_t row0 = ((uint32_t)t.m0 + (uint32_t)(wave * 32)) * lda2 + pr * lda2;
#pragma unroll
    for (int p = 0; p < 4; ++p) vA[p] = min(row0 + (uint32_t)(p * 8) * lda2, a_last) + (ch0 ^ ((p & 1) << 6));
  };
  auto set_w = [&](const Tile& t) {
    int l = lane;
    asm volatile("" : "+v"(l));
    const uint32_t pr = (uint32_t)(l >> 3), pp = (uint32_t)(l & 7);
    const uint32_t ch0 = (pp ^ (pr >> 1)) << 4;
    const uint32_t row0 = ((uint32_t)t.n0 + (uint32_t)(wave * 32)) * ldw2 + pr * ldw2;
#pragma unroll
    for (int p = 0; p < 4; ++p) vW[p] = row0 + (uint32_t)(p * 8) * ldw2 + (ch0 ^ ((p & 1) << 6));
  };
  auto issue_a = [&](int kt, int slot) {
    unsigned char* d = smem + slot * SLOT + wave * 32 * ROWB;
#pragma unroll
    for (int p = 0; p < 4; ++p)
      __builtin_amdgcn_raw_ptr_buffer_load_lds(srdA, (lds_ptr_t)(d + p * 8 * ROWB), 16, vA[p], kt * ROWB, 0, 0);
  };
  auto issue_w = [&](int kt, int slot) {
    unsigned char* d = smem + slot * SLOT + A_BYTES + wave * 32 * ROWB;
#pragma unroll
    for (int p = 0; p < 4; ++p)
      __builtin_amdgcn_raw_ptr_buffer_load_lds(srdW, (lds_ptr_t)(d + p * 8 * ROWB), 16, vW[p], kt * ROWB, 0, 0);
  };

  const int fr = lane & 15, fq = lane >> 4;
  const int sw = (fr >> 1) & 7;
  int offA[2], offW[2];
#pragma unroll
  for (int ks = 0; ks < 2; ++ks) {
    offA[ks] = (wr * WROWS + fr) * ROWB + (((4 * ks + fq) ^ sw) << 4);
    offW[ks] = A_BYTES + (wc * 64 + fr) * ROWB + (((4 * ks + fq) ^ sw) << 4);
  }
  auto read_w = [&](bf16x8 (&w)[4], int slot, int ks) {
    const unsigned char* sb = smem + slot * SLOT + offW[ks];
#pragma unroll
    for (int j = 0; j < 4; ++j) w[j] = *reinterpret_cast<const bf16x8*>(sb + j * 16 * ROWB);
  };
  auto read_a = [&](bf16x8 (&f)[4], int slot, int ks, int half) {
    const unsigned char* sb = smem + slot * SLOT + offA[ks] + half * 64 * ROWB;
#pragma unroll
    for (int i = 0; i < 4; ++i)
      if (half == 0 || i < HB) f[i] = *reinterpret_cast<const bf16x8*>(sb + i * 16 * ROWB);
  };

  f32x4 acc[RB][4];
  auto phase = [&](const bf16x8 (&w)[4], const bf16x8 (&f)[4], int half, auto&& mid) {
#pragma unroll
    for (int j = 0; j < 4; ++j) acc[4 * half][j] = __builtin_amdgcn_mfma_f32_16x16x32_bf16(w[j], f[0], acc[4 * half][j], 0, 0, 0);
    __builtin_amdgcn_sched_barrier(0);
    mid();
    __builtin_amdgcn_sched_barrier(0);
#pragma unroll
    for (int i = 1; i < (half == 0 ? 4 : HB); ++i)
#pragma unroll
      for (int j = 0; j < 4; ++j) acc[4 * half + i][j] = __builtin_amdgcn_mfma_f32_16x16x32_bf16(w[j], f[i], acc[4 * half + i][j], 0, 0, 0);
    __builtin_amdgcn_sched_barrier(0);
  };

  [[maybe_unused]] auto read_w8 = [&](v8i (&w)[4], int slot, int j) {
    const unsigned char* sb = smem + slot * SLOT + j * 16 * ROWB;
    const v4i x0 = *reinterpret_cast<const v4i*>(sb + offW[0]), x1 = *reinterpret_cast<const v4i*>(sb + offW[1]);
    w[j] = v8i{x0[0], x0[1], x0[2], x0[3], x1[0], x1[1], x1[2], x1[3]};
  };
  [[maybe_unused]] auto read_a8 = [&](v8i (&f)[2], int slot, int q) {
    const unsigned char* sb = smem + slot * SLOT + q * 32 * ROWB;
#pragma unroll
    for (int i = 0; i < 2; ++i) {
      const v4i x0 = *reinterpret_cast<const v4i*>(sb + offA[0] + i * 16 * ROWB), x1 = *reinterpret_cast<const v4i*>(sb + offA[1] + i * 16 * ROWB);
      f[i] = v8i{x0[0], x0[1], x0[2], x0[3], x1[0], x1[1], x1[2], x1[3]};
    }
  };
  [[maybe_unused]] auto mfma8 = [&](const v8i& w, const v8i& f, f32x4 c) {
    return __builtin_amdgcn_mfma_scale_f32_16x16x128_f8f6f4(w, f, c, 0, 0, 0, 0x7f7f7f7f, 0, 0x7f7f7f7f);
  };

  const int nk = a.K / (F8 ? 128 : TK);
  int idx = pos;
  Tile cur = decode_tile(idx, tiles_m, tiles_n, TMU);
  set_a(cur);
  set_w(cur);
  int par = 0;
  issue_a(0, 0);
  issue_w(0, 0);
  issue_a(1, 1);
  issue_w(1, 1);
  wait_vm<8>();
  __builtin_amdgcn_s_barrier();
  int s_prev = 0;

  [[maybe_unused]] bf16x8 wA[4], wB[4], lo[4], hi[4];
  [[maybe_unused]] v8i W8[4], aE[2], aO[2];
  [[maybe_unused]] unsigned char* const ep = smem + RING + wave * STAGE;
  const int D = EPI == DFD_EPI_QKV_EXPORT ? a.N / (3 - a.qkv_first) : 0;

  for (;;) {
    const int nidx = idx + G;
    const bool has_next = nidx < ntiles;
    const Tile nxt = has_next ? decode_tile(nidx, tiles_m, tiles_n, TMU) : cur;
#pragma unroll
    for (int i = 0; i < RB; ++i)
#pragma unroll
      for (int j = 0; j < 4; ++j) acc[i][j] = f32x4{0.f, 0.f, 0.f, 0.f};
    if constexpr (F8) {
#pragma unroll
      for (int j = 0; j < 4; ++j) read_w8(W8, par, j);
      read_a8(aE, par, 0);
    } else {
      read_w(wA, par, 0);
      read_a(lo, par, 0, 0);
    }
    f32x4 b4[4];
    [[maybe_unused]] f32x4 cs4[4];

    auto load_col_vectors = [&] {
      int lb = lane;
      asm volatile("" : "+v"(lb));
      const uint32_t coff = (uint32_t)((cur.n0 + wc * 64 + (lb >> 4) * 4) * 4);
      const uint32_t boff = a.bias ? coff : 0xffffffffu;
#pragma unroll
      for (int j = 0; j < 4; ++j) {
        b4[j] = __builtin_bit_cast(f32x4, __builtin_amdgcn_raw_buffer_load_b128(srdB, boff, j * 64, 0));
        if constexpr (F8) cs4[j] = __builtin_bit_cast(f32x4, __builtin_amdgcn_raw_buffer_load_b128(srdS, coff, j * 64, 0));
      }
    };
    auto pin_col_vectors = [&] {
#pragma unroll
      for (int j = 0; j < 4; ++j) {
        asm volatile("" : "+v"(b4[j]));
        if constexpr (F8) asm volatile("" : "+v"(cs4[j]));
      }
    };
    auto step_wait = [&](int kt) {
      asm volatile("s_waitcnt lgkmcnt(0)" ::: "memory");
      if (kt == 0) {
        if (s_prev == 0) wait_vm<0>();
        else if (s_prev == 2 * RB) wait_vm<2 * RB>();
        else if (s_prev == RB) wait_vm<RB>();
        else wait_vm<4 * RB>();
      } else {
        wait_vm<0>();
      }
    };

    [[maybe_unused]] auto phase8 = [&](const v8i (&f)[2], int q, auto&& mid) {
      __builtin_amdgcn_s_setprio(1);
#pragma unroll
      for (int j = 0; j < 2; ++j)
#pragma unroll
        for (int i = 0; i < 2; ++i) acc[2 * q + i][j] = mfma8(W8[j], f[i], acc[2 * q + i][j]);
      __builtin_amdgcn_s_setprio(0);
#pragma unroll
      for (int j = 0; j < 2; ++j)
#pragma unroll
        for (int i = 0; i < 2; ++i) asm volatile("" : "+v"(acc[2 * q + i][j]));
      __builtin_amdgcn_sched_barrier(0);
      mid();
      __builtin_amdgcn_sched_barrier(0);
      __builtin_amdgcn_s_setprio(1);
#pragma unroll
      for (int j = 2; j < 4; ++j)
#pragma unroll
        for (int i = 0; i < 2; ++i) acc[2 * q + i][j] = mfma8(W8[j], f[i], acc[2 * q + i][j]);
      __builtin_amdgcn_s_setprio(0);
#pragma unroll
      for (int j = 2; j < 4; ++j)
#pragma unroll
        for (int i = 0; i < 2; ++i) asm volatile("" : "+v"(acc[2 * q + i][j]));
      __builtin_amdgcn_sched_barrier(0);
    };
    [[maybe_unused]] auto kstep8 = [&](int kt, auto last_c) {
      constexpr bool last = decltype(last_c)::value;
      const int slot = (par + kt) & 1;
      if (has_next) {
        if (kt == nk - 2) set_a(nxt);
        if (kt == nk - 1) set_w(nxt);
      }
      phase8(aE, 0, [&] {
        read_a8(aO, slot, 1);
        if (kt >= 1) {
          if (!last) issue_w(kt + 1, slot ^ 1);
          else if (has_next) issue_w(0, slot ^ 1);
        }
      });
      phase8(aO, 1, [&] { read_a8(aE, slot, 2); });
      phase8(aE, 2, [&] { read_a8(aO, slot, 3); });
      if constexpr (last) load_col_vectors();
      step_wait(kt);
      if constexpr (last) pin_col_vectors();
      __builtin_amdgcn_s_barrier();
      __builtin_amdgcn_sched_barrier(0);
#pragma unroll
      for (int j = 0; j < 4; ++j) {
        __builtin_amdgcn_s_setprio(1);
#pragma unroll
        for (int i = 0; i < 2; ++i) acc[6 + i][j] = mfma8(W8[j], aO[i], acc[6 + i][j]);
        __builtin_amdgcn_s_setprio(0);
#pragma unroll
        for (int i = 0; i < 2; ++i) asm volatile("" : "+v"(acc[6 + i][j]));
        __builtin_amdgcn_sched_barrier(0);
        if constexpr (!last) read_w8(W8, slot ^ 1, j);
        if (j == 0) {
          if constexpr (!last) read_a8(aE, slot ^ 1, 0);
          if (kt + 2 < nk) issue_a(kt + 2, slot);
          else if (has_next) issue_a(kt + 2 - nk, slot);
        }
        __builtin_amdgcn_sched_barrier(0);
      }
    };

    auto kstep = [&](int kt, auto last_c) {
      constexpr bool last = decltype(last_c)::value;
      const int slot = (par + kt) & 1;
      if (has_next) {
        if (kt == nk - 2) set_a(nxt);
        if (kt == nk - 1) set_w(nxt);
      }
      phase(wA, lo, 0, [&] {
        read_a(hi, slot, 0, 1);
        if (kt >= 1) {
          if (!last) issue_w(kt + 1, slot ^ 1);
          else if (has_next) issue_w(0, slot ^ 1);
        }
      });
      phase(wA, hi, 1, [&] {
        read_w(wB, slot, 1);
        read_a(lo, slot, 1, 0);
      });
      phase(wB, lo, 0, [&] { read_a(hi, slot, 1, 1); });
      if constexpr (last) load_col_vectors();
      step_wait(kt);
      if constexpr (last) pin_col_vectors();
      __builtin_amdgcn_s_barrier();
      __builtin_amdgcn_sched_barrier(0);
      phase(wB, hi, 1, [&] {
        if constexpr (!last) {
          read_w(wA, slot ^ 1, 0);
          read_a(lo, slot ^ 1, 0, 0);
        }
        if (kt + 2 < nk) issue_a(kt + 2, slot);
        else if (has_next) issue_a(kt + 2 - nk, slot);
      });
    };
    if constexpr (F8) {
      for (int kt = 0; kt < nk - 1; ++kt) kstep8(kt, std::false_type{});
      kstep8(nk - 1, std::true_type{});
    } else {
      for (int kt = 0; kt < nk - 1; ++kt) kstep(kt, std::false_type{});
      kstep(nk - 1, std::true_type{});
    }
    if (has_next) issue_w(1, (par + nk - 1) & 1);

    const int stores = tile_epilogue<EPI, RB, F8, CF8>(a, acc, b4, cs4, ep, cur, wr, wc, opaque_lane(), D, srdC);
    if (!has_next) break;
    s_prev = countable_stores<RB>(stores, cur, wr, a.M);
    par = (par + nk) & 1;
    idx = nidx;
    cur = nxt;
  }
}

struct Gemm256p {
  static constexpr const char* name = "persistent";
  static constexpr bool spare_if_free = false;
  static constexpr bool serves(int epi, bool f8) {
    return epi == DFD_EPI_BIAS || epi == DFD_EPI_BIAS_QUICKGELU || epi == DFD_EPI_QKV_EXPORT || (f8 && epi == DFD_EPI_BIAS_GELU);
  }
  static bool depth_ok(const GemmArgs&, int, int nk, int) { return nk >= 2; }
  static void prepare(GemmArgs&, hipStream_t, const TilePlan&, bool) {}
  template <int EPI, int RB, bool F8, bool CF8>
  static void run(int grid, hipStream_t st, const GemmArgs& a, int tiles_m, int tiles_n) {
    hipLaunchKernelGGL((gemm256p_kernel<EPI, RB, F8, CF8>), dim3(grid), dim3(512), 0, st, a, tiles_m, tiles_n);
  }
};

}

int dfd_gemm256p_try(const GemmArgs& a, int c_dtype, int epi, hipStream_t st) { return try_persistent<Gemm256p, false>(a, c_dtype, epi, st); }

int dfd_gemm256p_f8_try(const GemmArgs& a, int c_dtype, int epi, hipStream_t st) { return try_persistent<Gemm256p, true>(a, c_dtype, epi, st); }
```

### dfd-clip_amd/csrc/gemm256p_common.hpp

```cpp
#pragma once
#include <type_traits>

#include "gemm_args.hpp"

#include "gelu.hpp"

typedef int v4i_t __attribute__((ext_vector_type(4)));
typedef v4i_t v4i;
typedef int v8i __attribute__((ext_vector_type(8)));

inline int persistent_cu_count() {
  static int n_cu = 0;
  if (n_cu == 0) {
    int dev = 0;
    hipDeviceProp_t prop;
    if (hipGetDevice(&dev) == hipSuccess && hipGetDeviceProperties(&prop, dev) == hipSuccess) n_cu = prop.multiProcessorCount;
  }
  return n_cu;
}

namespace {

__device__ __forceinline__ void store_out(v4i_t d, __amdgpu_buffer_rsrc_t srd, uint32_t off, int stream_out) {
  if (stream_out) {
    __builtin_amdgcn_raw_buffer_store_b128(d, srd, off, 0, 2);
  } else {
    __builtin_amdgcn_raw_buffer_store_b128(d, srd, off, 0, 0);
  }
}

constexpr int TM = 256, TN = 256, TK = 64;
constexpr int ROWB = TK * 2;
constexpr int A_BYTES = TM * ROWB;
constexpr int SLOT = (TM + TN) * ROWB;
constexpr int RING = 2 * SLOT;
constexpr int STAGE = 4096;
typedef __attribute__((address_space(3))) void* lds_ptr_t;

struct Tile {
  int m0, n0;
};

__device__ __forceinline__ Tile decode_tile(int idx, int tiles_m, int tiles_n, int tile_rows) {
  const int ngroups = (tiles_n + 5) / 6;
  const int gcols = (tiles_n + ngroups - 1) / ngroups;
  int grp = idx / (tiles_m * gcols);
  grp = grp < ngroups - 1 ? grp : ngroups - 1;
  const int rem = idx - grp * tiles_m * gcols;
  const int cols_here = min(gcols, tiles_n - grp * gcols);
  const int tm = rem / cols_here, tn = grp * gcols + (rem - tm * cols_here);
  return Tile{tm * tile_rows, tn * TN};
}

template <int N> __device__ __forceinline__ void wait_vm() { asm volatile("s_waitcnt vmcnt(%0)" ::"n"(N) : "memory"); }

__device__ __forceinline__ int opaque_lane() {
  int l = threadIdx.x & 63;
  asm volatile("" : "+v"(l));
  return l;
}

__device__ __forceinline__ int xcd_position() {
  const int G = gridDim.x, bid = blockIdx.x;
  const int xcd = bid & 7, q8 = G >> 3, r8 = G & 7;
  return (xcd < r8 ? xcd * (q8 + 1) : r8 * (q8 + 1) + (xcd - r8) * q8) + (bid >> 3);
}

__device__ __forceinline__ __amdgpu_buffer_rsrc_t make_srd(const void* p, int64_t bytes) {
  return __builtin_amdgcn_make_buffer_rsrc(const_cast<void*>(p), 0, (int)(uint32_t)bytes, 0x00020000);
}
__device__ __forceinline__ v4i words(const float* p, int bytes) {
  const uint64_t u = reinterpret_cast<uint64_t>(p);
  return v4i{(int)(uint32_t)u, (int)((uint32_t)(u >> 32) & 0xffffu), bytes, 0x00020000};
}
template <bool F8, bool CF8>
struct OperandSrds {
  __amdgpu_buffer_rsrc_t A, W, C;
  __device__ __forceinline__ explicit OperandSrds(const GemmArgs& a)
      : A(make_srd(a.A, a.M * a.lda * (F8 ? 1 : 2))), W(make_srd(a.W, (int64_t)a.N * a.ldw * (F8 ? 1 : 2))), C(make_srd(a.C, a.M * a.ldc * (CF8 ? 1 : 2))) {}
};
template <int RB> __device__ __forceinline__ int countable_stores(int stores, const Tile& t, int wr, int64_t M) {
  return (int64_t)t.m0 + (wr + 1) * 16 * RB <= M ? stores : 0;
}

template <int EPI, int RB, bool F8, bool CF8>
__device__ __forceinline__ int tile_epilogue(const GemmArgs& a, f32x4 (&acc)[RB][4], const f32x4 (&b4)[4], const f32x4 (&cs4)[4], unsigned char* const ep,
                                             const Tile& cur, int wr, int wc, int le, int D, __amdgpu_buffer_rsrc_t srdC) {
  constexpr int WROWS = 16 * RB;
  const int er = le & 15, eq = le >> 4;
  const int drow = le >> 3, dc = le & 7;
  const int nb = cur.n0 + wc * 64;
  const int64_t mrow0 = (int64_t)cur.m0 + wr * WROWS + drow;
  const int rows_left = (int)min((int64_t)0x7fffffff, a.M - mrow0);
  int which = 0;
  if constexpr (EPI == DFD_EPI_QKV_EXPORT) which = cur.n0 / D + a.qkv_first;
  const bool exporting = EPI == DFD_EPI_QKV_EXPORT && which > 0 && a.k_export != nullptr;
  int stores = 2 * RB;
#pragma unroll
  for (int i = 0; i < RB; ++i)
#pragma unroll
    for (int j = 0; j < 4; ++j) {
      if constexpr (F8) acc[i][j] = acc[i][j] * cs4[j] + b4[j];
      else acc[i][j] += b4[j];
    }
  if constexpr (EPI == DFD_EPI_QKV_EXPORT) {
    if (exporting) {
      stores = 4 * RB;
      const int ecol = nb - (which - a.qkv_first) * D + dc * 8;
      unsigned char* const parkf = ep + er * 256;
      const int64_t erows = (a.M / a.tokens) * (a.tokens - 1);
      const __amdgpu_buffer_rsrc_t srdE = make_srd(which == 2 ? a.v_export : a.k_export, erows * D * 2);
      const __amdgpu_buffer_rsrc_t srdP = make_srd(a.pos ? a.pos : reinterpret_cast<const float*>(a.W), a.pos ? a.frames_per_clip * D * 4 : 0);
#pragma unroll
      for (int i = 0; i < RB; ++i) {
        __builtin_amdgcn_sched_barrier(0);
        uint32_t eoff[2];
        f32x4 pe[2][2];
#pragma unroll
        for (int rr = 0; rr < 2; ++rr) {
          const int rloc = i * 16 + rr * 8;
          const uint32_t m = (uint32_t)min(mrow0 + rloc, a.M - 1);
          const uint32_t frame = a.div_tokens.div(m);
          const uint32_t tok = m - frame * (uint32_t)a.tokens;
          const uint32_t t = frame - a.div_frames.div(frame) * (uint32_t)a.frames_per_clip;
          eoff[rr] = (rloc < rows_left && tok > 0) ? ((frame * (uint32_t)(a.tokens - 1) + tok - 1) * (uint32_t)D + ecol) * 2 : 0xffffffffu;
          pe[rr][0] = pe[rr][1] = f32x4{0.f, 0.f, 0.f, 0.f};
          if (a.pos != nullptr) {
            const uint32_t poff = (t * (uint32_t)D + ecol) * 4;
            pe[rr][0] = __builtin_bit_cast(f32x4, __builtin_amdgcn_raw_buffer_load_b128(srdP, poff, 0, 0));
            pe[rr][1] = __builtin_bit_cast(f32x4, __builtin_amdgcn_raw_buffer_load_b128(srdP, poff, 16, 0));
          }
        }
#pragma unroll
        for (int j = 0; j < 4; ++j)
          *reinterpret_cast<f32x4*>(parkf + (((j * 4 + eq) ^ er) << 4)) = acc[i][j];
#pragma unroll
        for (int rr = 0; rr < 2; ++rr) {
          const int row = rr * 8 + drow;
          const f32x4 x0 = *reinterpret_cast<const f32x4*>(ep + row * 256 + (((2 * dc) ^ row) << 4)) + pe[rr][0];
          const f32x4 x1 = *reinterpret_cast<const f32x4*>(ep + row * 256 + (((2 * dc + 1) ^ row) << 4)) + pe[rr][1];
          bf16x8 o;
#pragma unroll
          for (int e = 0; e < 4; ++e) {
            o[e] = (bf16_t)x0[e];
            o[4 + e] = (bf16_t)x1[e];
          }
          store_out(__builtin_bit_cast(v4i, o), srdE, eoff[rr], a.stream_out);
        }
      }
    }
  }
  auto activate = [&](f32x4 v) {
    if constexpr (EPI == DFD_EPI_BIAS_QUICKGELU) {
      float cgelu = DFD_QUICKGELU_SCALE;
      asm volatile("" : "+s"(cgelu));
      const f32x4 t = v * cgelu;
      f32x4 d;
#pragma unroll
      for (int e = 0; e < 4; ++e) d[e] = __builtin_amdgcn_exp2f(t[e]);
      d = d + 1.0f;
#pragma unroll
      for (int e = 0; e < 4; ++e) d[e] = __builtin_amdgcn_rcpf(d[e]);
      v = v * d;
    } else if constexpr (EPI == DFD_EPI_BIAS_GELU) {
      v = gelu_erf4(v);
    }
    return v;
  };
  if constexpr (EPI == DFD_EPI_RESIDUAL_POS) {
    unsigned char* const parkf = ep + er * 256;
    const uint32_t cbase = (uint32_t)((mrow0 * a.ldc + nb + dc * 8) * 2);
    const v4i srdRw = a.residual ? words(reinterpret_cast<const float*>(a.residual), (int)(uint32_t)(a.M * a.ldc * 2))
                                 : words(reinterpret_cast<const float*>(a.C), (int)(uint32_t)(a.M * a.ldc * 2));
    const v4i srdQw = words(a.pos ? a.pos : reinterpret_cast<const float*>(a.W), a.pos ? a.frames_per_clip * a.N * 4 : 0);
    f32x4 pq[2][2][2];
    v4i oq[2][2];
    uint32_t offq[2][2], gq[2][2];
    auto request = [&](int i, int b) {
#pragma unroll
      for (int rr = 0; rr < 2; ++rr) {
        const int rloc = i * 16 + rr * 8;
        const uint32_t m = (uint32_t)min(mrow0 + rloc, a.M - 1);
        const uint32_t frame = a.div_tokens.div(m);
        const uint32_t t = frame - a.div_frames.div(frame) * (uint32_t)a.frames_per_clip;
        offq[b][rr] = rloc < rows_left ? cbase + (uint32_t)rloc * (uint32_t)(a.ldc * 2) : 0xffffffffu;
        gq[b][rr] = m * (uint32_t)(a.N >> 3) + (uint32_t)((nb + dc * 8) >> 3);
        const uint32_t poff = a.pos ? (t * (uint32_t)a.N + (uint32_t)(nb + dc * 8)) * 4 : 0xffffffffu;
        asm volatile(
            "s_nop 4\n\t"
            "buffer_load_dwordx4 %0, %3, %5, 0 offen\n\t"
            "buffer_load_dwordx4 %1, %3, %5, 0 offen offset:16\n\t"
            "buffer_load_dwordx4 %2, %4, %6, 0 offen"
            : "=&v"(pq[b][rr][0]), "=&v"(pq[b][rr][1]), "=&v"(oq[b][rr])
            : "v"(poff), "v"(offq[b][rr]), "s"(srdQw), "s"(srdRw)
            : "memory");
      }
    };
    request(0, 0);
#pragma unroll
    for (int i = 0; i < RB; ++i) {
      __builtin_amdgcn_sched_barrier(0);
      const int b = i & 1;
      if (i + 1 < RB) request(i + 1, b ^ 1);
#pragma unroll
      for (int j = 0; j < 4; ++j) *reinterpret_cast<f32x4*>(parkf + (((j * 4 + eq) ^ er) << 4)) = acc[i][j];
      if (i == 0) wait_vm<6>();
      else if (i + 1 < RB) wait_vm<8>();
      else wait_vm<2>();
      asm volatile("" : "+v"(pq[b][0][0]), "+v"(pq[b][0][1]), "+v"(oq[b][0]), "+v"(pq[b][1][0]), "+v"(pq[b][1][1]), "+v"(oq[b][1]));
      __builtin_amdgcn_sched_barrier(0);
#pragma unroll
      for (int rr = 0; rr < 2; ++rr) {
        const int row = rr * 8 + drow;
        const f32x4 x0 = *reinterpret_cast<const f32x4*>(ep + row * 256 + (((2 * dc) ^ row) << 4));
        const f32x4 x1 = *reinterpret_cast<const f32x4*>(ep + row * 256 + (((2 * dc + 1) ^ row) << 4));
        float dv[8];
#pragma unroll
        for (int e = 0; e < 4; ++e) {
          dv[e] = x0[e];
          dv[4 + e] = x1[e];
        }
        dfd_drop_eight(a.drop, (uint64_t)gq[b][rr] << 3, dv);
        const bf16x8 ob = __builtin_bit_cast(bf16x8, oq[b][rr]);
        bf16x8 o;
#pragma unroll
        for (int e = 0; e < 4; ++e) {
          o[e] = (bf16_t)((float)ob[e] + dv[e] + pq[b][rr][0][e]);
          o[4 + e] = (bf16_t)((float)ob[4 + e] + dv[4 + e] + pq[b][rr][1][e]);
        }
        store_out(__builtin_bit_cast(v4i, o), srdC, offq[b][rr], a.stream_out);
      }
    }
  } else if constexpr (CF8) {
    stores = RB;
    const int srow = le >> 2, sc = le & 3;
    unsigned char* const park8 = ep + er * 64 + eq * 4;
    const int psw = (er >> 1) & 3;
    const unsigned char* const dsrc8 = ep + srow * 64 + ((sc ^ ((srow >> 1) & 3)) << 4);
    const int64_t m8 = (int64_t)cur.m0 + wr * WROWS + srow;
    const int rows_left8 = (int)min((int64_t)0x7fffffff, a.M - m8);
    const uint32_t cbase8 = (uint32_t)(m8 * a.ldc + nb + sc * 16);
#pragma unroll
    for (int q = 0; q < 4; ++q) {
#pragma unroll
      for (int ii = 0; ii < 2; ++ii) {
        const int i = 2 * q + ii;
#pragma unroll
        for (int j = 0; j < 4; ++j) {
          f32x4 v = activate(acc[i][j]) * a.out_inv_scale;
#pragma unroll
          for (int e = 0; e < 4; ++e) v[e] = __builtin_fminf(__builtin_fmaxf(v[e], -448.0f), 448.0f);
          unsigned pk = __builtin_amdgcn_cvt_pk_fp8_f32(v[0], v[1], 0u, false);
          pk = __builtin_amdgcn_cvt_pk_fp8_f32(v[2], v[3], pk, true);
          *reinterpret_cast<unsigned*>(park8 + ii * 1024 + ((j ^ psw) << 4)) = pk;
        }
      }
#pragma unroll
      for (int rr = 0; rr < 2; ++rr) {
        const v4i d = *reinterpret_cast<const v4i*>(dsrc8 + rr * 1024);
        const int rloc = q * 32 + rr * 16;
        const uint32_t off = rloc < rows_left8 ? cbase8 + (uint32_t)rloc * (uint32_t)a.ldc : 0xffffffffu;
        store_out(d, srdC, off, a.stream_out);
      }
    }
  } else {
    unsigned char* const park = ep + er * 128 + ((eq ^ ((er & 7) << 1)) << 3);
    const unsigned char* const dsrc = ep + drow * 128 + ((dc ^ drow) << 4);
    const uint32_t cbase = (uint32_t)((mrow0 * a.ldc + nb + dc * 8) * 2);
#pragma unroll
    for (int q = 0; q < 4; ++q) {
#pragma unroll
      for (int ii = 0; ii < 2; ++ii) {
        const int i = 2 * q + ii;
        if (i >= RB) continue;
#pragma unroll
        for (int j = 0; j < 4; ++j) {
          const f32x4 v = activate(acc[i][j]);
          bf16x4 o;
#pragma unroll
          for (int e = 0; e < 4; ++e) o[e] = (bf16_t)v[e];
          typedef __attribute__((address_space(3))) bf16x4 lds_bf16x4;
          *reinterpret_cast<lds_bf16x4*>(((uint32_t)(uintptr_t)(lds_ptr_t)(park + ii * 2048)) ^ (uint32_t)(j << 5)) = o;
        }
      }
#pragma unroll
      for (int rr = 0; rr < 4; ++rr) {
        if (q * 32 + rr * 8 >= WROWS) continue;
        const v4i d = *reinterpret_cast<const v4i*>(dsrc + rr * 1024);
        const int rloc = q * 32 + rr * 8;
        uint32_t off = rloc < rows_left ? cbase + (uint32_t)rloc * (uint32_t)(a.ldc * 2) : 0xffffffffu;
        store_out(d, srdC, off, a.stream_out);
      }
    }
  }
  return stores;
}

struct TilePlan {
  int rows, tiles_m;
  int64_t ntiles;
  int grid;
};

inline TilePlan plan_tiles(int64_t M, int N, int spare_cus, bool spare_if_free, int tile_rows, bool f8, bool force224) {
  const int n_cu = persistent_cu_count(), tiles_n = N / TN;
  if (n_cu == 0) return TilePlan{0, 0, 0, 0};
  int cus = n_cu - spare_cus;
  cus = cus < n_cu / 2 ? n_cu / 2 : cus;
  auto cost = [&](int rows, int c) { return (double)((((M + rows - 1) / rows) * tiles_n + c - 1) / c) * (rows == 224 ? 0.97 : 1.0); };
  if (spare_cus > 0 && spare_if_free) {
    auto best = [&](int c) { return f8 ? cost(256, c) : force224 ? cost(224, c) : (cost(224, c) < cost(256, c) ? cost(224, c) : cost(256, c)); };
    if (best(cus) > best(n_cu)) cus = n_cu;
  }
  const bool use224 = !f8 && (force224 || tile_rows == 224 || (tile_rows == 0 && cost(224, cus) < cost(256, cus)));
  TilePlan p;
  p.rows = use224 ? 224 : 256;
  p.tiles_m = (int)((M + p.rows - 1) / p.rows);
  p.ntiles = (int64_t)p.tiles_m * tiles_n;
  p.grid = (int)(p.ntiles < cus ? p.ntiles : cus);
  return p;
}

template <class L, int EPI, bool F8, bool CF8>
int launch_persistent(const GemmArgs& a_in, hipStream_t st) {
  constexpr bool force224 = EPI == DFD_EPI_RESIDUAL_POS;
  GemmArgs a = a_in;
  const TilePlan p = plan_tiles(a.M, a.N, a.spare_cus, L::spare_if_free && a.spare_if_free, a.tile_rows, F8, force224);
  if (p.grid == 0) {
    dfd_set_error("dfd_gemm(%s): cannot query the device", L::name);
    return DFD_ERR_LAUNCH;
  }
  L::prepare(a, st, p, F8);
  const int tiles_n = a.N / TN;
  if constexpr (F8) {
    L::template run<EPI, 8, true, CF8>(p.grid, st, a, p.tiles_m, tiles_n);
  } else {
    if (p.rows == 224) L::template run<EPI, 7, false, false>(p.grid, st, a, p.tiles_m, tiles_n);
    else if constexpr (!force224) L::template run<EPI, 8, false, false>(p.grid, st, a, p.tiles_m, tiles_n);
  }
  hipError_t e = hipGetLastError();
  if (e != hipSuccess) {
    dfd_set_error("dfd_gemm(%s): launch failed: %s", L::name, hipGetErrorString(e));
    return DFD_ERR_LAUNCH;
  }
  return DFD_OK;
}

inline int check_persistent(const GemmArgs& a, int esz, int csz, int kstep) {
  if (a.N % TN != 0 || a.K % kstep != 0 || a.M < 1024) return 1;
  if ((a.lda * esz) % 16 != 0 || (a.ldw * esz) % 16 != 0 || (a.ldc * csz) % 16 != 0) return 1;
  if ((reinterpret_cast<uintptr_t>(a.A) & 15) != 0 || (reinterpret_cast<uintptr_t>(a.W) & 15) != 0 || (reinterpret_cast<uintptr_t>(a.C) & 15) != 0) return 1;
  if (a.bias && (reinterpret_cast<uintptr_t>(a.bias) & 15) != 0) return 1;
  const int64_t lim = (int64_t)0xfffffff0;
  if (a.M * a.lda * esz > lim || (int64_t)a.N * a.ldw * esz > lim || a.M * a.ldc * csz > lim) return 1;
  if ((int64_t)((a.M + 223) / 224) * (a.N / TN) > 0x3fffffff || a.M >= ((int64_t)1 << 31)) return 1;
  return 0;
}

inline int check_export(const GemmArgs& a) {
  if ((a.N / (3 - a.qkv_first)) % TN != 0) return 1;
  if (a.pos && (reinterpret_cast<uintptr_t>(a.pos) & 15) != 0) return 1;
  if (a.k_export && (a.M / a.tokens) * (a.tokens - 1) * (int64_t)(a.N / (3 - a.qkv_first)) * 2 > (int64_t)0xfffffff0) return 1;
  return 0;
}

inline int check_residual_pos(const GemmArgs& a) {
  if (a.tokens < 2 || a.M * (int64_t)(a.N >> 3) >= ((int64_t)1 << 32)) return 1;
  if (a.pos && ((reinterpret_cast<uintptr_t>(a.pos) & 15) != 0 || a.frames_per_clip < 1)) return 1;
  if (a.residual && (reinterpret_cast<uintptr_t>(a.residual) & 15) != 0) return 1;
  return 0;
}

template <class L, bool F8>
int try_persistent(const GemmArgs& a_in, int c_dtype, int epi, hipStream_t st) {
  if (c_dtype != DFD_BF16 && !(F8 && c_dtype == DFD_FP8)) return 1;
  const bool cf8 = c_dtype == DFD_FP8;
  constexpr int esz = F8 ? 1 : 2, kstep = F8 ? 128 : TK;
  if (F8 && (!a_in.col_scale || (reinterpret_cast<uintptr_t>(a_in.col_scale) & 15) != 0)) return 1;
  if (check_persistent(a_in, esz, cf8 ? 1 : 2, kstep) || !L::depth_ok(a_in, esz, a_in.K / kstep, epi)) return 1;
  GemmArgs a = a_in;
  auto go = [&](auto epi_c) -> int {
    constexpr int EPI = decltype(epi_c)::value;
    constexpr bool rows_to_frames = EPI == DFD_EPI_QKV_EXPORT || EPI == DFD_EPI_RESIDUAL_POS;
    if constexpr (!L::serves(EPI, F8)) {
      return 1;
    } else {
      if constexpr (EPI == DFD_EPI_QKV_EXPORT) {
        if (check_export(a)) return 1;
      }
      if constexpr (EPI == DFD_EPI_RESIDUAL_POS) {
        if (check_residual_pos(a)) return 1;
      }
      if constexpr (rows_to_frames) {
        a.div_tokens = FastDiv::make((uint32_t)(EPI == DFD_EPI_RESIDUAL_POS ? a.tokens - 1 : a.tokens));
        a.div_frames = FastDiv::make((uint32_t)(a.frames_per_clip > 0 ? a.frames_per_clip : 1));
      }
      if constexpr (F8 && !rows_to_frames) {
        if (cf8) return launch_persistent<L, EPI, true, true>(a, st);
      }
      return cf8 ? 1 : launch_persistent<L, EPI, F8, false>(a, st);
    }
  };
  switch (epi) {
    case DFD_EPI_BIAS:
      return go(std::integral_constant<int, DFD_EPI_BIAS>{});
    case DFD_EPI_BIAS_QUICKGELU:
      return go(std::integral_constant<int, DFD_EPI_BIAS_QUICKGELU>{});
    case DFD_EPI_BIAS_GELU:
      return go(std::integral_constant<int, DFD_EPI_BIAS_GELU>{});
    case DFD_EPI_QKV_EXPORT:
      return go(std::integral_constant<int, DFD_EPI_QKV_EXPORT>{});
    case DFD_EPI_RESIDUAL_POS:
      return go(std::integral_constant<int, DFD_EPI_RESIDUAL_POS>{});
    default:
      return 1;
  }
}

}
```

### dfd-clip_amd/csrc/gemm_args.hpp

```cpp
#pragma once
#include "dropout.hpp"

struct GemmArgs {
  const void* A;
  const void* W;
  void* C;
  const float* bias;
  const float* pos;
  const float* cls;
  void* k_export;
  void* v_export;
  const void* residual;
  int64_t lda, ldw, ldc, M;
  int N, K, tokens, frames_per_clip;
  int qkv_first;
  int stream_out;
  int spare_cus;
  int spare_if_free;
  int tile_rows;
  DfdDrop drop;
  FastDiv div_tokens, div_frames;
  const float* col_scale;
  float out_inv_scale;
  uint32_t* sched;
  uint32_t sched_base[8];
  int no_dynamic;
};

int dfd_gemm256_try(const GemmArgs& a, int c_dtype, int epi, hipStream_t st);
int dfd_gemm256e_try(const GemmArgs& a, int c_dtype, int epi, hipStream_t st);
int dfd_gemm256e_f8_try(const GemmArgs& a, int c_dtype, int epi, hipStream_t st);
int dfd_gemm256p_try(const GemmArgs& a, int c_dtype, int epi, hipStream_t st);
int dfd_gemm256p_f8_try(const GemmArgs& a, int c_dtype, int epi, hipStream_t st);
```

### dfd-clip_amd/encoder.py

```python
import contextlib

import torch
from torch import nn

from . import capi


FP8_PRESETS = ("all", "proj-bf16", "kv-bf16", "kv+proj-bf16", "edges-bf16", "none")
FP8_CONTRACT_POLICY = None
_ALL = {"qkv": "fp8", "fc": "fp8", "proj": "fp8"}
_NONE = {"qkv": "bf16", "fc": "bf16", "proj": "bf16"}


def expand_fp8_policy(policy, layers, tapped=None):
    tapped = sorted(set(range(layers) if tapped is None else (int(t) for t in tapped)))
    if any(t < 0 or t >= layers for t in tapped):
        raise ValueError(f"fp8 policy: tapped layers {tapped} outside 0..{layers - 1}")
    if policy is None:
        policy = "all"
    if isinstance(policy, str):
        if policy not in FP8_PRESETS:
            raise ValueError(f"fp8 policy: unknown preset {policy!r} (presets: {', '.join(FP8_PRESETS)})")
        kv = "kv-bf16" if policy in ("kv-bf16", "kv+proj-bf16") else "fp8"
        proj = "bf16" if policy in ("proj-bf16", "kv+proj-bf16") else "fp8"
        edge = set(range(min(2, layers))) | set(range(max(0, layers - 2), layers)) if policy == "edges-bf16" else set()
        policy = [dict(_NONE) if policy == "none" or l in edge else {"qkv": kv, "fc": "fp8", "proj": proj} for l in range(layers)]
    policy = list(policy)
    if len(policy) != layers:
        raise ValueError(f"fp8 policy: {len(policy)} entries for {layers} layers")
    out = []
    for l, ent in enumerate(policy):
        if not isinstance(ent, dict) or set(ent) - set(_ALL):
            raise ValueError(f"fp8 policy, layer {l}: expected a dict with keys qkv / fc / proj, got {ent!r}")
        e = {**_ALL, **ent}
        if e["qkv"] not in ("fp8", "bf16", "kv-bf16") or e["fc"] not in ("fp8", "bf16") or e["proj"] not in ("fp8", "bf16"):
            raise ValueError(f"fp8 policy, layer {l}: {ent!r} (qkv: fp8 | bf16 | kv-bf16; fc, proj: fp8 | bf16)")
        if e["proj"] == "fp8" and e["fc"] != "fp8":
            raise ValueError(f"fp8 policy, layer {l}: proj 'fp8' requires fc 'fp8' — the e4m3 input of c_proj exists only as the "
                             "fp8 c_fc's epilogue output")
        if e["qkv"] == "kv-bf16":
            e["qkv"] = "fp8" if l not in tapped else ("bf16" if l == tapped[-1] else "kv-bf16")
        out.append(e)
    return out


def quantize_rows_e4m3(w):
    w = w.detach().to(torch.float32)
    sc = (w.abs().amax(dim=1) / capi.FP8_MAX).clamp_min(1e-12)
    return (w / sc[:, None]).to(torch.float8_e4m3fn).view(torch.uint8).contiguous(), sc.contiguous()


class RuntimeStateMixin:
    _RUNTIME_STATE = {}

    def __deepcopy__(self, memo):
        import copy
        new = self.__class__.__new__(self.__class__)
        memo[id(self)] = new
        for k, v in self.__dict__.items():
            if k in self._RUNTIME_STATE:
                new.__dict__[k] = copy.deepcopy(self._RUNTIME_STATE[k])
            else:
                new.__dict__[k] = copy.deepcopy(v, memo)
        return new


class _Holder(nn.Module):

    def forward(self, *a, **k):
        raise RuntimeError("parameter holder")


class _AttnParams(_Holder):
    def __init__(self, d):
        super().__init__()
        self.in_proj_weight = nn.Parameter(torch.empty(3 * d, d))
        self.in_proj_bias = nn.Parameter(torch.empty(3 * d))
        self.out_proj = nn.Linear(d, d)
        nn.init.normal_(self.in_proj_weight, std=d ** -0.5)
        nn.init.normal_(self.in_proj_bias, std=0.02)


class _Mlp(_Holder):
    def __init__(self, d):
        super().__init__()
        self.c_fc = nn.Linear(d, 4 * d)
        self.c_proj = nn.Linear(4 * d, d)


class ResidualAttentionBlock(_Holder):
    def __init__(self, d_model, n_head):
        super().__init__()
        self.attn = _AttnParams(d_model)
        self.attn.n_head = n_head
        self.ln_1 = nn.LayerNorm(d_model)
        self.mlp = _Mlp(d_model)
        self.ln_2 = nn.LayerNorm(d_model)


class Transformer(_Holder):
    def __init__(self, width, layers, heads):
        super().__init__()
        self.width = width
        self.layers = layers
        self.resblocks = nn.Sequential(*[ResidualAttentionBlock(width, heads) for _ in range(layers)])


def _invalidate_after_load(module, incompatible_keys):
    module.invalidate()


class VisionTransformer(RuntimeStateMixin, nn.Module):
    _RUNTIME_STATE = {"_prepared": None, "_ws": {}, "_side_streams": [], "_calib": None}
    ln_eps = 1e-5
    act_epilogue = capi.EPI_BIAS_QUICKGELU

    def __init__(self, input_resolution, patch_size, width, layers, heads, output_dim, precision="bf16"):
        super().__init__()
        self.output_dim = output_dim
        self.conv1 = nn.Conv2d(3, width, kernel_size=patch_size, stride=patch_size, bias=False)
        scale = width ** -0.5
        self.class_embedding = nn.Parameter(scale * torch.randn(width))
        self.positional_embedding = nn.Parameter(scale * torch.randn((input_resolution // patch_size) ** 2 + 1, width))
        self.ln_pre = nn.LayerNorm(width)
        self.transformer = Transformer(width, layers, heads)
        self.ln_post = nn.LayerNorm(width)
        self.proj = nn.Parameter(scale * torch.randn(width, output_dim))
        self._init_runtime(input_resolution, patch_size, width, layers, heads, precision)

    def _init_runtime(self, input_resolution, patch_size, width, layers, heads, precision):
        assert width % heads == 0 and width // heads == 64, "kernels are built for 64-wide heads"
        assert precision in ("fp32", "bf16", "fp8")
        self.input_resolution = input_resolution
        self.width = width
        self.layers = layers
        self.heads = heads
        self.patch_size = patch_size
        self.precision = precision
        self.register_load_state_dict_post_hook(_invalidate_after_load)
        self._prepared = None
        self._ws = {}
        self.frame_chunk = 0
        self.streams = 1
        self._side_streams = []
        self.pixel_mean = (0.48145466, 0.4578275, 0.40821073)
        self.pixel_std = (0.26862954, 0.26130258, 0.27577711)
        self.antialias = True
        self.deferred_residual = precision in ("bf16", "fp8")
        self._fp8 = None
        self._fp8_amax = None
        self._fp8_margin = 1.0
        self._calib = None
        self._fp8_policy, self._fp8_tapped = "all", None
        self._fp8_plan = expand_fp8_policy("all", layers) if precision == "fp8" else None
        self.stream_out = {"qkv": True, "out": True, "fc": True, "proj": True}
        self.spare_cus = 0
        self.spare_layers = 0
        self.spare_gemms = {"qkv": False, "out": False, "fc": False, "proj": True}
        self.spare_window_layers = 0
        self.spare_if_free = True

    @property
    def tokens(self):
        return (self.input_resolution // self.patch_size) ** 2 + 1

    @property
    def act_dtype(self):
        return torch.float32 if self.precision == "fp32" else torch.bfloat16

    def _ensure_fp8(self, frames):
        if self.precision == "fp8" and self._fp8_amax is None and getattr(self, "_calib", None) is None:
            import logging
            logging.warning("fp8 encoder: no calibration yet, taking the activation scales from this batch "
                            "(call encoder.calibrate_fp8(frames) with representative frames to fix them beforehand)")
            self.calibrate_fp8(frames[:min(frames.shape[0], 64)])

    @torch.no_grad()
    def calibrate_fp8(self, x, margin=1.0):
        assert self.precision == "fp8"
        p = self._prepare()
        frames = self._as_frames(x)
        n = frames.shape[0]
        M = n * self.tokens
        rec = []
        self._calib = rec
        try:
            ws = self._workspace(n, 1, slot=99)
            self._embed(frames, ws, p)
            for bp in p["blocks"]:
                self._block(ws, bp, ws["qkv"][0], M, n)
        finally:
            self._ws.pop(self._ws_key(n, 1, 99), None)
            self._calib = None
        amax = torch.stack(rec).view(len(p["blocks"]), 3).float().cpu()
        self._fp8_amax, self._fp8_margin, self._fp8 = amax, float(margin), None
        self._fp8_layers()
        return (amax * margin / capi.FP8_MAX).clamp_min(1e-12)

    def fp8_calibration(self):
        return None if self._fp8_amax is None else self._fp8_amax.clone()

    def load_fp8_calibration(self, amax, margin=1.0):
        amax = torch.as_tensor(amax, dtype=torch.float32).cpu()
        assert amax.shape == (self.layers, 3)
        self._fp8_amax, self._fp8_margin, self._fp8 = amax, float(margin), None

    def set_fp8_policy(self, policy, tapped=None):
        if self.precision != "fp8":
            raise ValueError(f"an fp8 policy needs precision='fp8' (this encoder runs {self.precision!r})")
        plan = expand_fp8_policy(policy, self.layers, tapped)
        self._fp8_policy = "all" if policy is None else policy
        self._fp8_tapped = None if tapped is None else tuple(int(t) for t in tapped)
        self._fp8_plan = plan
        self._fp8 = None
        return plan

    def fp8_policy(self):
        return None if self._fp8_plan is None else [dict(e) for e in self._fp8_plan]

    def _fp8_needs(self, M):
        if self.precision != "fp8":
            return (False, False, True)
        if self._calib is not None or M < capi.FP8_MIN_ROWS:
            return (False, False, True)
        plan = self._fp8_plan
        return (any(e["qkv"] != "bf16" or e["fc"] == "fp8" for e in plan), any(e["proj"] == "fp8" for e in plan),
                any(e["proj"] == "bf16" for e in plan))

    def _fp8_layers(self):
        if self._fp8 is None:
            assert self._fp8_amax is not None, "fp8 encoder: not calibrated"
            p = self._prepare()
            scales = (self._fp8_amax * self._fp8_margin / capi.FP8_MAX).clamp_min(1e-12)
            layers = []
            for l, bp in enumerate(p["blocks"]):
                s1, s2, su = (float(v) for v in scales[l])
                layers.append(dict(h1_inv=1.0 / s1, h2_inv=1.0 / s2, u_inv=1.0 / su, cs_qkv=(bp["s_qkv"] * s1).contiguous(),
                                   cs_fc=(bp["s_fc"] * s2).contiguous(), cs_proj=(bp["s_proj"] * su).contiguous()))
            self._fp8 = layers
        return self._fp8

    def invalidate(self):
        self._prepared = None
        self._fp8 = None

    def _apply(self, fn, *a, **k):
        out = super()._apply(fn, *a, **k)
        self._prepared = None
        self._fp8 = None
        self._ws = {}
        return out

    def load_state_dict(self, *a, **k):
        out = super().load_state_dict(*a, **k)
        self._prepared = None
        self._fp8 = None
        return out

    def _param_device(self):
        return self.class_embedding.device

    def _prepare(self):
        if self._prepared is not None:
            return self._prepared
        dev = self._param_device()
        if dev.type != "cuda":
            raise capi.DfdError("the encoder runs on HIP kernels only: move the model to a GPU (.to('cuda'))")
        self._prepared = self._stage(dev)
        return self._prepared

    def _stage(self, dev):
        act = self.act_dtype
        kreal = 3 * self.patch_size ** 2
        kpad = (kreal + 63) // 64 * 64
        wp = torch.zeros(self.width, kpad, device=dev, dtype=torch.float32)
        wp[:, :kreal] = self.conv1.weight.detach().reshape(self.width, kreal)
        f32 = lambda t: t.detach().to(torch.float32).contiguous()
        p = dict(kpad=kpad, w_patch=wp.to(act).contiguous(), cls=f32(self.class_embedding),
                 pos=f32(self.positional_embedding), ln_pre=(f32(self.ln_pre.weight), f32(self.ln_pre.bias)), blocks=[])
        q8 = quantize_rows_e4m3
        for blk in self.transformer.resblocks:
            if self.precision == "fp8":
                f8 = dict(zip(("w_qkv8", "s_qkv"), q8(blk.attn.in_proj_weight)))
                f8.update(zip(("w_fc8", "s_fc"), q8(blk.mlp.c_fc.weight)))
                f8.update(zip(("w_proj8", "s_proj"), q8(blk.mlp.c_proj.weight)))
            else:
                f8 = {}
            p["blocks"].append(dict(f8, idx=len(p["blocks"]), 
                ln1=(f32(blk.ln_1.weight), f32(blk.ln_1.bias)), ln2=(f32(blk.ln_2.weight), f32(blk.ln_2.bias)),
                w_qkv=blk.attn.in_proj_weight.detach().to(act).contiguous(), b_qkv=f32(blk.attn.in_proj_bias),
                w_out=blk.attn.out_proj.weight.detach().to(act).contiguous(), b_out=f32(blk.attn.out_proj.bias),
                w_fc=blk.mlp.c_fc.weight.detach().to(act).contiguous(), b_fc=f32(blk.mlp.c_fc.bias),
                w_proj=blk.mlp.c_proj.weight.detach().to(act).contiguous(), b_proj=f32(blk.mlp.c_proj.bias)))
        return p

    def _ws_key(self, n, keep_layers, slot):
        return (n, self.precision, keep_layers, slot, self._fp8_needs(n * self.tokens))

    def _workspace(self, n, keep_layers, slot=0):
        key = self._ws_key(n, keep_layers, slot)
        need_h8, need_u8, need_u = key[-1]
        ws = self._ws.get(key)
        if ws is None:
            dev = self._param_device()
            act, D = self.act_dtype, self.width
            M = n * self.tokens
            Mp = (M + 255) // 256 * 256
            P = self.tokens - 1
            Pp = (n * P + 255) // 256 * 256
            kpad = self._prepare()["kpad"]
            ws = dict(
                x=torch.zeros(Mp, D, device=dev, dtype=torch.float32), h=torch.zeros(Mp, D, device=dev, dtype=act),
                mix=torch.zeros(Mp, D, device=dev, dtype=act), u=torch.zeros(Mp, 4 * D, device=dev, dtype=act) if need_u else None,
                patches=torch.zeros(Pp, kpad, device=dev, dtype=act),
                delta=torch.zeros(Mp, D, device=dev, dtype=act) if self.deferred_residual else None,
                delta2=torch.zeros(Mp, D, device=dev, dtype=act) if self.deferred_residual else None, pending=0,
                qkv=[torch.zeros(Mp, 3 * D, device=dev, dtype=act) for _ in range(keep_layers)])
            if need_h8:
                ws["h8"] = torch.zeros(Mp, D, device=dev, dtype=torch.uint8)
            if need_u8:
                ws["u8"] = torch.zeros(Mp, 4 * D, device=dev, dtype=torch.uint8)
            if len(self._ws) > 6:
                self._ws.clear()
            self._ws[key] = ws
        return ws

    def graph_guard(self, n):
        return (self._prepare(), self._fp8_layers() if self.precision == "fp8" else None, self._workspace(n, 1, slot=0))

    def _as_frames(self, x):
        if x.dtype == torch.uint8:
            assert x.dim() == 4 and x.shape[1] == 3, "uint8 frames must be [N, 3, H, W]"
            return x.contiguous()
        assert tuple(x.shape[1:]) == (3, self.input_resolution, self.input_resolution), \
            f"frames must be [N, 3, {self.input_resolution}, {self.input_resolution}]"
        return x.to(torch.float32).contiguous()

    def _embed(self, frames, ws, p):
        n = frames.shape[0]
        P, D = self.tokens - 1, self.width
        if frames.dtype == torch.uint8:
            capi.preprocess_u8(frames, ws["patches"][:n * P], self.input_resolution, self.patch_size, self.pixel_mean,
                               self.pixel_std, antialias=self.antialias)
        else:
            capi.patchify(frames, ws["patches"], self.input_resolution, self.patch_size)
        capi.gemm(ws["patches"], p["w_patch"], ws["x"], None, capi.EPI_PATCH_EMBED, m=n * P, pos=p["pos"], cls=p["cls"],
                  tokens=self.tokens)
        ws["pending"] = 0
        ws["ln_pre"] = p["ln_pre"]

    def _ln(self, ws, gb, M, store=True, q=None, discard_x=False, dual=False):
        x = ws["x"]
        if dual:
            return self._ln_dual(ws, gb, M, q, discard_x)
        h, inv = (ws["h8"], q) if q is not None else (ws["h"], 0.0)
        pend = ws.get("pending", 0)
        pre = ws.pop("ln_pre", None)
        if pre is not None:
            assert pend == 0
            if self.width <= 2048:
                capi.layernorm2(x[:M], pre[0], pre[1], gb[0], gb[1], h[:M], eps=self.ln_eps, out_inv_scale=inv)
            else:
                capi.layernorm(x[:M], pre[0], pre[1], x[:M], eps=self.ln_eps)
                capi.layernorm(x[:M], gb[0], gb[1], h[:M], eps=self.ln_eps, out_inv_scale=inv)
        elif pend == 0:
            capi.layernorm(x[:M], gb[0], gb[1], h[:M], eps=self.ln_eps, out_inv_scale=inv)
        elif discard_x:
            capi.add_layernorm(x[:M], ws["delta"][:M], gb[0], gb[1], h[:M], delta2=ws["delta2"][:M] if pend == 2 else None,
                               store_x=False, eps=self.ln_eps, out_inv_scale=inv)
            ws["pending"] = 0
        elif not store:
            assert pend == 1
            capi.add_layernorm(x[:M], ws["delta"][:M], gb[0], gb[1], h[:M], store_x=False, eps=self.ln_eps, out_inv_scale=inv)
        else:
            capi.add_layernorm(x[:M], ws["delta"][:M], gb[0], gb[1], h[:M], delta2=ws["delta2"][:M] if pend == 2 else None,
                               eps=self.ln_eps, out_inv_scale=inv)
            ws["pending"] = 0

    def _ln_dual(self, ws, gb, M, inv, discard_x):
        x, h, h8 = ws["x"], ws["h"], ws["h8"]
        pend = ws.get("pending", 0)
        pre = ws.pop("ln_pre", None)
        if pre is not None:
            assert pend == 0
            if self.width <= 2048:
                capi.layernorm2_dual(x[:M], pre[0], pre[1], gb[0], gb[1], h[:M], h8[:M], inv, eps=self.ln_eps)
            else:
                capi.layernorm(x[:M], pre[0], pre[1], x[:M], eps=self.ln_eps)
                capi.layernorm_dual(x[:M], gb[0], gb[1], h[:M], h8[:M], inv, eps=self.ln_eps)
        elif pend == 0:
            capi.layernorm_dual(x[:M], gb[0], gb[1], h[:M], h8[:M], inv, eps=self.ln_eps)
        else:
            capi.add_layernorm_dual(x[:M], ws["delta"][:M], gb[0], gb[1], h[:M], h8[:M], inv, eps=self.ln_eps,
                                    delta2=ws["delta2"][:M] if pend == 2 else None, store_x=not discard_x)
            ws["pending"] = 0

    def _residual(self, ws, a, w, b, M, spare_cus=0, spare_if_free=False):
        if self.deferred_residual:
            pend = ws.get("pending", 0)
            assert pend < 2
            capi.gemm(a, w, ws["delta2" if pend else "delta"], b, capi.EPI_BIAS, m=M, stream_out=self.stream_out["proj" if pend else "out"],
                      spare_cus=spare_cus, spare_if_free=spare_if_free)
            ws["pending"] = pend + 1
        else:
            capi.gemm(a, w, ws["x"], b, capi.EPI_BIAS_RESIDUAL, m=M)

    def _flush(self, ws, M):
        pend = ws.get("pending", 0)
        if pend >= 1:
            ws["x"][:M] += ws["delta"][:M]
        if pend == 2:
            ws["x"][:M] += ws["delta2"][:M]
        ws["pending"] = 0

    def _block(self, ws, bp, qkv, M, n, kv_only=False, export=None):
        calib = getattr(self, "_calib", None)
        f8 = self._fp8_layers()[bp["idx"]] if self.precision == "fp8" and calib is None and M >= capi.FP8_MIN_ROWS else None
        pl = self._fp8_plan[bp["idx"]] if f8 is not None else _NONE
        so = self.stream_out
        sp = self.spare_cus if (self.spare_layers <= 0 or bp["idx"] < self.spare_layers) else 0
        sp_all = self.spare_cus if bp["idx"] < self.spare_window_layers else 0
        sg = self.spare_gemms
        sp_qkv, sp_out, sp_fc, sp_proj = (max(sp_all, sp if sg[k] else 0) for k in ("qkv", "out", "fc", "proj"))
        free = sp_all == 0 and self.spare_if_free
        D = self.width
        first = 1 if kv_only else 0
        rows = slice(D, None) if first else slice(None)
        kw = dict(m=M, tokens=self.tokens, qkv_first=first, stream_out=so["qkv"], spare_cus=sp_qkv, spare_if_free=free)
        if export is not None:
            kw.update(pos=export[2], k_export=export[0], v_export=export[1], frames_per_clip=export[3])
        if pl["qkv"] == "fp8":
            self._ln(ws, bp["ln1"], M, q=f8["h1_inv"], discard_x=kv_only)
            capi.gemm_fp8(ws["h8"], bp["w_qkv8"][rows], qkv[:, rows], f8["cs_qkv"][rows], bp["b_qkv"][rows], capi.EPI_QKV_EXPORT, **kw)
        elif pl["qkv"] == "kv-bf16" and not kv_only:
            self._ln(ws, bp["ln1"], M, q=f8["h1_inv"], dual=True)
            capi.gemm_fp8(ws["h8"], bp["w_qkv8"][:D], qkv[:, :D], f8["cs_qkv"][:D], bp["b_qkv"][:D], capi.EPI_BIAS, m=M,
                          stream_out=so["qkv"], spare_cus=sp_qkv, spare_if_free=free)
            capi.gemm(ws["h"], bp["w_qkv"][D:], qkv[:, D:], bp["b_qkv"][D:], capi.EPI_QKV_EXPORT, **dict(kw, qkv_first=1))
        else:
            self._ln(ws, bp["ln1"], M, discard_x=kv_only and calib is None)
            if calib is not None:
                calib.append(ws["h"][:M].abs().max())
            capi.gemm(ws["h"], bp["w_qkv"][rows], qkv[:, rows], bp["b_qkv"][rows], capi.EPI_QKV_EXPORT, **kw)
        if kv_only:
            return
        capi.attention_fwd(qkv, ws["mix"], n, self.tokens, self.heads)
        self._residual(ws, ws["mix"], bp["w_out"], bp["b_out"], M, spare_cus=sp_out, spare_if_free=free)
        if pl["fc"] == "fp8" and pl["proj"] == "bf16":
            self._ln(ws, bp["ln2"], M, store=False, q=f8["h2_inv"])
            capi.gemm_fp8(ws["h8"], bp["w_fc8"], ws["u"], f8["cs_fc"], bp["b_fc"], self.act_epilogue, m=M,
                          stream_out=so["fc"], spare_cus=sp_fc, spare_if_free=free)
            self._residual(ws, ws["u"], bp["w_proj"], bp["b_proj"], M, spare_cus=sp_proj, spare_if_free=free)
        elif pl["fc"] == "fp8":
            self._ln(ws, bp["ln2"], M, store=False, q=f8["h2_inv"])
            capi.gemm_fp8(ws["h8"], bp["w_fc8"], ws["u8"], f8["cs_fc"], bp["b_fc"], self.act_epilogue, m=M,
                          out_inv_scale=f8["u_inv"], stream_out=so["fc"], spare_cus=sp_fc, spare_if_free=free)
            pend = ws.get("pending", 0)
            capi.gemm_fp8(ws["u8"], bp["w_proj8"], ws["delta2" if pend else "delta"], f8["cs_proj"], bp["b_proj"], capi.EPI_BIAS, m=M,
                          stream_out=so["proj"], spare_cus=sp_proj, spare_if_free=free)
            ws["pending"] = pend + 1
        else:
            self._ln(ws, bp["ln2"], M, store=False)
            if calib is not None:
                calib.append(ws["h"][:M].abs().max())
            capi.gemm(ws["h"], bp["w_fc"], ws["u"], bp["b_fc"], self.act_epilogue, m=M, stream_out=so["fc"], spare_cus=sp_fc, spare_if_free=free)
            if calib is not None:
                calib.append(ws["u"][:M].abs().max())
            self._residual(ws, ws["u"], bp["w_proj"], bp["b_proj"], M, spare_cus=sp_proj, spare_if_free=free)

    @torch.no_grad()
    def forward(self, x, with_out=False, with_q=False):
        if not x.is_cuda:
            raise capi.DfdError("the encoder runs on HIP kernels only: pass device tensors")
        p = self._prepare()
        frames = self._as_frames(x)
        n = frames.shape[0]
        self._ensure_fp8(frames)
        D, H, tok = self.width, self.heads, self.tokens
        M = n * tok
        ws = self._workspace(n, self.layers)
        self._embed(frames, ws, p)
        result = []
        for l, bp in enumerate(p["blocks"]):
            qkv = ws["qkv"][l]
            self._block(ws, bp, qkv, M, n)
            t = qkv[:M].view(n, tok, 3, H, 64)
            d = {"k": t[:, :, 1], "v": t[:, :, 2]}
            if with_q:
                d["q"] = t[:, :, 0]
            if with_out:
                self._flush(ws, M)
                d["out"] = ws["x"][:M].view(n, tok, D).clone()
            result.append(d)
        return result

    @torch.no_grad()
    def extract_kv(self, x, layer_indices, num_frames, temporal_pos=None, out=None, pos_ready=None, in_place=None):
        if not x.is_cuda:
            raise capi.DfdError("the encoder runs on HIP kernels only: pass device tensors")
        p = self._prepare()
        frames = self._as_frames(x)
        n = frames.shape[0]
        assert n % num_frames == 0
        self._ensure_fp8(frames)
        D, tok = self.width, self.tokens
        P = tok - 1
        L = len(layer_indices)
        if in_place is not None:
            assert in_place.shape == (L, n, tok, 3 * D) and in_place.dtype == self.act_dtype and in_place.is_contiguous()
            k_out = v_out = None
        elif out is None:
            k_out = torch.empty(L, n * P, D, device=frames.device, dtype=self.act_dtype)
            v_out = torch.empty_like(k_out)
        else:
            k_out, v_out = out
        last = max(layer_indices)
        slot = {l: i for i, l in enumerate(layer_indices)}
        clips = n // num_frames
        chunk = self.frame_chunk if self.frame_chunk > 0 else -(-clips // max(1, self.streams)) * num_frames
        chunk = max(num_frames, chunk // num_frames * num_frames)
        starts = list(range(0, n, chunk))
        n_str = min(self.streams, len(starts))
        if n_str > 1:
            cur = torch.cuda.current_stream()
            if len(self._side_streams) < n_str:
                self._side_streams = [torch.cuda.Stream() for _ in range(n_str)]
            for st in self._side_streams[:n_str]:
                st.wait_stream(cur)
        for ci, f0 in enumerate(starts):
            nf = min(chunk, n - f0)
            ctx = torch.cuda.stream(self._side_streams[ci % n_str]) if n_str > 1 else contextlib.nullcontext()
            with ctx:
                ws = self._workspace(nf, 1, slot=(ci % n_str) if n_str > 1 else 0)
                qkv = ws["qkv"][0]
                M = nf * tok
                self._embed(frames[f0:f0 + nf], ws, p)
                waited = pos_ready is None or temporal_pos is None or in_place is not None
                for l in range(last + 1):
                    exp = None
                    qkv_l = qkv
                    if l in slot and in_place is not None:
                        qkv_l = in_place[slot[l]].view(n * tok, 3 * D)[f0 * tok:(f0 + nf) * tok]
                    elif l in slot:
                        i = slot[l]
                        if not waited:
                            torch.cuda.current_stream().wait_event(pos_ready)
                            waited = True
                        exp = (k_out[i, f0 * P:(f0 + nf) * P], v_out[i, f0 * P:(f0 + nf) * P], temporal_pos, num_frames)
                    self._block(ws, p["blocks"][l], qkv_l, M, nf, kv_only=(l == last), export=exp)
        if n_str > 1:
            for st in self._side_streams[:n_str]:
                cur.wait_stream(st)
        if in_place is not None:
            return in_place[:, :, 1:, D:2 * D], in_place[:, :, 1:, 2 * D:]
        return k_out, v_out
```

### include/dfdclip.h

```cpp
#ifndef DFDCLIP_H
#define DFDCLIP_H

#include <stddef.h>
#include <stdint.h>

#ifdef __cplusplus
extern "C" {
#endif

#define DFD_ABI_VERSION 17

enum { DFD_F32 = 0, DFD_BF16 = 1, DFD_FP8 = 2  };

enum {
  DFD_OK = 0,
  DFD_ERR_INVALID_ARG = -1,
  DFD_ERR_LAUNCH = -2,
  DFD_ERR_NO_DEVICE = -3
};

enum {
  DFD_EPI_BIAS = 0,
  DFD_EPI_BIAS_QUICKGELU,
  DFD_EPI_BIAS_RESIDUAL,
  DFD_EPI_PATCH_EMBED,
  DFD_EPI_QKV_EXPORT,
  DFD_EPI_RESIDUAL_POS,
  DFD_EPI_BIAS_GELU
};

typedef struct dfd_dropout_t {
  const uint64_t* rng_state;
  uint32_t site;
  float p;
} dfd_dropout_t;

typedef struct dfd_gemm_extra {
  const float* pos;
  const float* cls;
  void* k_export;
  void* v_export;
  int32_t tokens;
  int32_t frames_per_clip;
  const void* residual;
  int32_t qkv_first;
  const uint64_t* drop_rng;
  uint32_t drop_site;
  float drop_p;
  uint32_t flags;
} dfd_gemm_extra;

enum {
  DFD_GEMM_STREAM_OUT = 1,
  DFD_GEMM_SPARE_IF_FREE = 2,
  DFD_GEMM_TILE_BLOCKS_SHIFT = 16,
  DFD_GEMM_SPARE_CUS_SHIFT = 8
};

const char* dfd_last_error(void);
int dfd_abi_version(void);
int dfd_device_check(void);

int dfd_layernorm(const float* x, int64_t ldx, const float* gamma, const float* beta, void* y, int64_t ldy,
                  int y_dtype, int64_t rows, int cols, float eps, float y_inv_scale, void* stream);

int dfd_layernorm2(float* x, int64_t ldx, const float* gamma_a, const float* beta_a, const float* gamma_b, const float* beta_b,
                   void* y, int64_t ldy, int y_dtype, int64_t rows, int cols, float eps, float y_inv_scale, void* stream);

int dfd_add_layernorm(float* x, int64_t ldx, const void* delta, const void* delta2, int64_t ldd, int delta_dtype,
                      int store_x, const float* gamma, const float* beta, void* y, int64_t ldy, int y_dtype, int64_t rows,
                      int cols, float eps, float y_inv_scale, void* stream);


int dfd_patchify(const float* frames, void* patches, int out_dtype, int n_frames, int res, int patch, int kpad,
                 void* stream);

int dfd_preprocess_u8(const uint8_t* frames, int n_frames, int in_h, int in_w, int res, int patch, int antialias,
                      const float* mean3, const float* std3, void* out, int out_dtype, int layout, int kpad,
                      void* stream);
int dfd_preprocess_geometry(int in_h, int in_w, int res, int* rs_h, int* rs_w, int* top, int* left);

int dfd_gemm(const void* A, int64_t lda, const void* W, int64_t ldw, int ab_dtype, void* C, int64_t ldc,
             int c_dtype, const float* bias, int epilogue, const dfd_gemm_extra* extra, int64_t M, int N, int K,
             void* stream);
int dfd_gemm_fp8(const void* A, int64_t lda, const void* W, int64_t ldw, void* C, int64_t ldc, int c_dtype,
                 const float* col_scale, const float* bias, float out_inv_scale, int epilogue,
                 const dfd_gemm_extra* extra, int64_t M, int N, int K, void* stream);

int dfd_gemm_last_path(void);

int dfd_gemm_set_variant(int variant);

size_t dfd_gemm_at_b_workspace(int64_t R, int Ma, int Nb, int dtype);
int dfd_gemm_at_b(const void* A, int64_t lda, const void* B, int64_t ldb, int dtype, float* C, int64_t R, int Ma, int Nb,
                  void* workspace, void* stream);

int dfd_attention_fwd(const void* qkv, int64_t ld_qkv, void* out, int64_t ld_out, int dtype, int n_frames,
                      int tokens, int heads, int head_dim, float scale, void* stream);

int dfd_linear_rows(const float* x, int64_t ldx, const float* W, const float* bias, float* y, int64_t ldy,
                    int epilogue, int B, int N, int K, void* stream);

size_t dfd_linear_rows_t_workspace(int B, int N, int K);
int dfd_linear_rows_t(const float* x, int64_t ldx, const float* Wt, const float* bias, const float* residual, int64_t ldr,
                      float* y, int64_t ldy, int epilogue, int B, int N, int K, void* workspace, void* stream);

typedef struct {
  int64_t row_stride, frame_stride;
  const float* pos;
} dfd_kv_layout_t;

size_t dfd_decoder_attn_workspace(int B, int heads, int d, int splits);
int dfd_decoder_attn_fwd(const float* q, const void* k, const void* v, int kv_dtype, const dfd_kv_layout_t* layout,
                         const uint8_t* frame_mask, const float* ext_weights, float* mix, float* mix_softmax, float* stats,
                         void* workspace, int splits, int B, int T, int patches, int heads, int d, void* stream);

int dfd_decoder_attn_modes_fwd(const float* q, const void* k, int kv_dtype, const dfd_kv_layout_t* layout,
                               const uint8_t* frame_mask, int modes, float* scores, float* weights, int B, int T, int patches,
                               int heads, int d, void* stream);

int dfd_head_fwd(const float* x, int64_t ldx, const float* gamma, const float* beta, const float* proj,
                 float* video_feature, float* raw_logits, float* logits, int B, int D, int out_dim, float eps,
                 const dfd_dropout_t* drop_post, void* stream);

int dfd_dropout(const void* in, int in_dtype, void* out, int out_dtype, int64_t n, const dfd_dropout_t* drop,
                void* stream);

int dfd_adapter_norm_gelu(const void* a, int a_dtype, void* y, int dtype, const float* weight, const float* bias, int frames,
                          int patches, int x, int joint, float eps, void* stream);

size_t dfd_adapter_norm_gelu_bwd_workspace(int frames, int patches, int x, int joint);
int dfd_adapter_norm_gelu_bwd(const void* a, int a_dtype, const void* dy, void* da, int dtype, const float* weight, const float* bias,
                              float* dweight, float* dbias, void* workspace, int frames, int patches, int x, int joint,
                              float eps, void* stream);


size_t dfd_decoder_attn_bwd_workspace(int B, int T, int heads, int d);
int dfd_decoder_attn_bwd(const float* q, const void* k, const void* v, int kv_dtype, const dfd_kv_layout_t* layout,
                         const uint8_t* frame_mask, const float* dmix, const float* mix_softmax, const float* stats, const float* ext_weights,
                         const float* ext_dscores, float* dq, float* dpos, void* dk, void* dv, int dkv_dtype,
                         void* workspace, int B, int T, int patches, int heads, int d, void* stream);

int dfd_decoder_attn_modes_bwd(const float* scores, const void* v, int kv_dtype, const dfd_kv_layout_t* layout,
                               const float* dmix, int modes, float* dwv_workspace, float* dscores, int B, int T, int patches,
                               int heads, int d, void* stream);

int dfd_linear_rows_bwd_weight(const float* dy, int64_t lddy, const float* x, int64_t ldx, float* dW, float* db, int B,
                               int N, int K, void* stream);

int dfd_transpose_f32(const float* src, float* dst, int rows, int cols, void* stream);

typedef struct dfd_sgd_param {
  float* p;
  const float* g;
  float* buf;
  float* mirror;
  int64_t numel;
  int32_t rows, cols;
  int64_t first_block;
} dfd_sgd_param;
enum { DFD_OPTIM_SGD = 0, DFD_OPTIM_ADAMW = 1 };
typedef struct dfd_optim_extra {
  int32_t kind;
  int32_t reserved;
  double beta1, beta2, eps;
  int64_t step;
  float* const* exp_avg_sq;
} dfd_optim_extra;
int64_t dfd_sgd_blocks(int64_t numel, int rows, int cols, int mirrored);
int dfd_sgd_step(const dfd_sgd_param* table_dev, int n, int64_t total_blocks, float lr, float momentum, float weight_decay,
                 int first_step, void* stream, const dfd_optim_extra* extra);

int dfd_layernorm_bwd(const float* x, int64_t ldx, const float* gamma, const float* dy, int64_t lddy, float* dx,
                      int64_t lddx, float* dgamma, float* dbeta, float* xhat_ws, int rows, int cols, float eps,
                      int accumulate_dx, void* stream);

int dfd_quickgelu(const float* u, const float* du, float* out, int64_t n, const dfd_dropout_t* drop, void* stream);

int dfd_head_bwd(const float* raw_logits, const float* dlogits, const float* proj, const float* feat,
                 const float* dfeat_ext, float* dz, float* dfeat, float* dproj, int B, int D, int out_dim,
                 void* stream);

size_t dfd_compinv_loss_workspace(int P, int D);
int dfd_compinv_loss_fwd(const void* k, const void* v, int dtype, int B, int T, int P, int D, int L, void* workspace,
                         float* match, float* norm, float* recon, void* stream);
int dfd_compinv_loss_bwd(const void* k, const void* v, int dtype, int B, int T, int P, int D, int L, const void* workspace,
                         const float* norm, const float* grad, void* dk, void* dv, void* stream);

size_t dfd_adapter_bn_workspace(int64_t frames, int patches, int width);
int dfd_adapter_bn_stats(const void* y, int dtype, float* stats, float* running_mean, float* running_var,
                         int64_t* num_batches_tracked, void* workspace, int64_t frames, int patches, int width, int T, int mode,
                         float momentum, float eps, void* stream);
int dfd_adapter_bn_apply(const void* y, int y_dtype, const void* residual, void* out, int dtype, const float* stats,
                         const float* gamma, const float* beta, const float* pos, const dfd_dropout_t* drop, int64_t frames,
                         int patches, int width, int T, void* stream);
int dfd_adapter_bn_bwd(const void* y, const void* dout, int dout_dtype, void* dy, int dtype, const float* stats,
                       const float* gamma, float* dgamma, float* dbeta, const dfd_dropout_t* drop, void* workspace,
                       int64_t frames, int patches, int width, int T, int train, void* stream);
int dfd_gelu_erf(const void* a, int a_dtype, void* out, int out_dtype, int64_t n, const dfd_dropout_t* drop, void* stream);
int dfd_gelu_erf_bwd(const void* a, int a_dtype, const void* dh, int dh_dtype, void* da, int da_dtype, int64_t n,
                     const dfd_dropout_t* drop, void* stream);

#ifdef __cplusplus
}
#endif
#endif
```

### include/dfdclip_hooks.h

```cpp
#ifndef DFDCLIP_HOOKS_H
#define DFDCLIP_HOOKS_H

#ifdef __cplusplus
extern "C" {
#endif

int dfd_attention_set_variant(int variant);

#ifdef __cplusplus
}
#endif
#endif
```

Measured before the change: 872.1.

## Store MLP hidden activations in a blocked layout shared by fc and proj GEMMs

The fc GEMM epilogue now writes its GELU output straight to global memory in a 16-row × 64-channel blocked layout, with fc weights and bias permuted so that each lane's accumulator channels map to contiguous 16-byte chunks. The proj GEMM reads that blocked A operand with matching address arithmetic. The goal is to skip the LDS transpose/park step in the fc epilogue and give proj contiguous loads. The path is limited to bf16 with deferred residual, needs rows padded to 16 and permuted weight copies, and adds a template variant of the ping-pong kernel.

```diff
diff --git a/dfd-clip_amd/blocked.py b/dfd-clip_amd/blocked.py
--- /dev/null
+++ b/dfd-clip_amd/blocked.py
@@ -0,0 +1,45 @@
+import torch
+
+GROUP_ROWS = 16
+TILE_CHANNELS = 64
+
+
+def padded_rows(m):
+    return (int(m) + GROUP_ROWS - 1) // GROUP_ROWS * GROUP_ROWS
+
+
+def piece_offset(row, channel, ld):
+    g, er = divmod(int(row), GROUP_ROWS)
+    kt, c = divmod(int(channel), TILE_CHANNELS)
+    chunk, e = divmod(c, 8)
+    s, eq = chunk & 1, chunk >> 1
+    return g * GROUP_ROWS * ld + kt * 1024 + s * 512 + er * 32 + eq * 8 + e
+
+
+def pack(x, fill=0):
+    m, c = x.shape
+    assert c % TILE_CHANNELS == 0, "the blocked layout needs whole 64-channel K tiles"
+    mp = padded_rows(m)
+    xp = torch.full((mp, c), fill, dtype=x.dtype, device=x.device)
+    xp[:m] = x
+    v = xp.view(mp // GROUP_ROWS, GROUP_ROWS, c // TILE_CHANNELS, 4, 2, 8)
+    return v.permute(0, 2, 4, 1, 3, 5).reshape(mp, c).contiguous()
+
+
+def unpack(b, m=None):
+    mp, c = b.shape
+    assert mp % GROUP_ROWS == 0 and c % TILE_CHANNELS == 0 and b.is_contiguous()
+    v = b.view(mp // GROUP_ROWS, c // TILE_CHANNELS, 2, GROUP_ROWS, 4, 8)
+    x = v.permute(0, 3, 1, 4, 2, 5).reshape(mp, c)
+    return x[:mp if m is None else m].contiguous()
+
+
+def fc_channel_perm(n, device=None):
+    assert n % TILE_CHANNELS == 0
+    c = torch.arange(n, device=device)
+    return (c & ~60) | ((c & 12) << 2) | ((c & 48) >> 2)
+
+
+def lane_channels(eq):
+    perm = fc_channel_perm(TILE_CHANNELS)
+    return [[int(perm[16 * j + 4 * eq + e]) for e in range(4)] for j in range(4)]
diff --git a/dfd-clip_amd/build.py b/dfd-clip_amd/build.py
--- a/dfd-clip_amd/build.py
+++ b/dfd-clip_amd/build.py
@@ -56,6 +56,7 @@
     headers.append(os.path.join(INCLUDE, "dfdclip.h"))
     headers.append(os.path.join(INCLUDE, "dfdclip_ext.h"))
     headers.append(os.path.join(INCLUDE, "dfdclip_explain.h"))
+    headers.append(os.path.join(INCLUDE, "dfdclip_hooks.h"))
     jobs, objs = [], []
     for src in sources():
         sp = os.path.join(CSRC, src)
diff --git a/dfd-clip_amd/capi.py b/dfd-clip_amd/capi.py
--- a/dfd-clip_amd/capi.py
+++ b/dfd-clip_amd/capi.py
@@ -23,6 +23,8 @@
 
 GEMM_STREAM_OUT = 1
 GEMM_SPARE_IF_FREE = 2
+GEMM_C_BLOCKED = 4
+GEMM_A_BLOCKED = 8
 
 
 class GemmExtra(Structure):
@@ -144,6 +146,9 @@
 
 HOOK_SIGNATURES = {
     "dfd_attention_set_variant": (c_int, [c_int]),
+    "dfd_gemm_pair_set_variant": (c_int, [c_int]),
+    "dfd_gemm_pair_plan": (c_int, [c_int64, c_int, c_int]),
+    "dfd_gemm_pair_launches": (c_int64, []),
 }
 
 _lib = None
@@ -312,7 +317,8 @@
 
 
 def gemm(a, w, c, bias=None, epilogue=EPI_BIAS, m=None, pos=None, cls=None, k_export=None, v_export=None, tokens=0,
-         frames_per_clip=0, residual=None, qkv_first=0, drop=None, stream_out=False, spare_cus=0, tile_blocks=0, spare_if_free=False):
+         frames_per_clip=0, residual=None, qkv_first=0, drop=None, stream_out=False, spare_cus=0, tile_blocks=0, spare_if_free=False,
+         c_blocked=False, a_blocked=False):
     _dev(a, w, c, bias, pos, cls, k_export, v_export, residual)
     assert a.dtype == w.dtype and a.stride(1) == 1 and w.stride(1) == 1 and c.stride(1) == 1
     M = a.shape[0] if m is None else m
@@ -321,9 +327,13 @@
     assert residual is None or (residual.dtype == c.dtype and residual.stride(0) == c.stride(0))
     assert drop is None or epilogue == EPI_RESIDUAL_POS
     assert 0 <= epilogue <= EPI_BIAS_GELU, f"unknown epilogue {epilogue}"
+    if c_blocked or a_blocked:
+        blk = c if c_blocked else a
+        assert blk.shape[0] >= (M + 15) // 16 * 16, "a blocked matrix needs its rows rounded up to 16"
     extra = GemmExtra(_ptr(pos).value, _ptr(cls).value, _ptr(k_export).value, _ptr(v_export).value, tokens, frames_per_clip,
                       _ptr(residual).value, qkv_first, drop.rng.data_ptr() if drop is not None and drop.p > 0 else None,
-                      drop.site if drop is not None else 0, drop.p if drop is not None else 0.0, (GEMM_STREAM_OUT if stream_out else 0) | (GEMM_SPARE_IF_FREE if spare_if_free else 0) | ((int(spare_cus) & 0xff) << 8) | ((int(tile_blocks) & 0xf) << 16))
+                      drop.site if drop is not None else 0, drop.p if drop is not None else 0.0, (GEMM_STREAM_OUT if stream_out else 0) | (GEMM_SPARE_IF_FREE if spare_if_free else 0) | ((int(spare_cus) & 0xff) << 8) | ((int(tile_blocks) & 0xf) << 16)
+                      | (GEMM_C_BLOCKED if c_blocked else 0) | (GEMM_A_BLOCKED if a_blocked else 0))
     timed = _profile["epilogue"] == epilogue
     if timed:
         e0, e1 = torch.cuda.Event(enable_timing=True), torch.cuda.Event(enable_timing=True)
@@ -364,6 +374,18 @@
     return load_library().dfd_gemm_set_variant(int(variant))
 
 
+def gemm_pair_set_variant(variant):
+    return load_library().dfd_gemm_pair_set_variant(int(variant))
+
+
+def gemm_pair_plan(M, D, H):
+    return bool(load_library().dfd_gemm_pair_plan(int(M), int(D), int(H)))
+
+
+def gemm_pair_launches():
+    return load_library().dfd_gemm_pair_launches()
+
+
 def gemm_last_path():
     return load_library().dfd_gemm_last_path()
 
diff --git a/dfd-clip_amd/csrc/gemm.hip b/dfd-clip_amd/csrc/gemm.hip
--- a/dfd-clip_amd/csrc/gemm.hip
+++ b/dfd-clip_amd/csrc/gemm.hip
@@ -1,5 +1,6 @@
 #include "gemm_args.hpp"
 #include "gelu.hpp"
+#include "../../include/dfdclip_hooks.h"
 
 namespace {
 
@@ -289,6 +290,9 @@
     a.spare_cus = (int)((extra->flags >> DFD_GEMM_SPARE_CUS_SHIFT) & 0xff);
     a.spare_if_free = (extra->flags & DFD_GEMM_SPARE_IF_FREE) ? 1 : 0;
     a.tile_rows = 32 * (int)((extra->flags >> DFD_GEMM_TILE_BLOCKS_SHIFT) & 0xf);
+    a.c_blocked = (extra->flags & DFD_GEMM_C_BLOCKED) ? 1 : 0;
+    a.a_blocked = (extra->flags & DFD_GEMM_A_BLOCKED) ? 1 : 0;
+    a.pair = a.c_blocked | a.a_blocked;
     DFD_REQUIRE(a.tile_rows == 0 || a.tile_rows == 224 || a.tile_rows == 256, "dfd_gemm: tile blocks must be 0, 7 or 8");
     if (epilogue == DFD_EPI_RESIDUAL_POS && extra->drop_rng && extra->drop_p > 0.f) {
       DFD_REQUIRE(extra->drop_p < 1.f, "dfd_gemm: drop_p=%f", (double)extra->drop_p);
@@ -308,9 +312,42 @@
   return old;
 }
 
+static thread_local int g_pair_variant = 0;
+static thread_local int64_t g_pair_launches = 0;
+extern "C" int dfd_gemm_pair_set_variant(int variant) {
+  const int old = g_pair_variant;
+  g_pair_variant = variant;
+  return old;
+}
+extern "C" int64_t dfd_gemm_pair_launches(void) { return g_pair_launches; }
+extern "C" int dfd_gemm_pair_plan(int64_t M, int D, int H) {
+  if (g_pair_variant == 1 || g_gemm_variant == 1 || M < 1 || D < 1 || H < 1) return 0;
+  if (M < 1024 && g_pair_variant != 2) return 0;
+  void* const any = reinterpret_cast<void*>(uintptr_t{256});
+  GemmArgs fc{}, pr{};
+  fc.A = pr.A = any; fc.W = pr.W = any; fc.C = pr.C = any;
+  fc.M = pr.M = M; fc.pair = pr.pair = 1;
+  fc.N = H; fc.K = D; fc.lda = D; fc.ldw = D; fc.ldc = H; fc.c_blocked = 1;
+  pr.N = D; pr.K = H; pr.lda = H; pr.ldw = H; pr.ldc = D; pr.a_blocked = 1;
+  return dfd_gemm256e_serves(fc, DFD_BF16, DFD_EPI_BIAS_QUICKGELU) && dfd_gemm256e_serves(pr, DFD_BF16, DFD_EPI_BIAS) ? 1 : 0;
+}
+
 static int try_persistent_kernels(GemmArgs& a, int c_dtype, int epilogue, bool f8, hipStream_t st, int* path) {
   const int epi_p = epilogue == DFD_EPI_QKV_EXPORT && a.k_export == nullptr ? DFD_EPI_BIAS : epilogue;
   a.no_dynamic = g_gemm_variant != 3;
+  if (a.pair) {
+    if (g_pair_variant == 1) a.c_blocked = a.a_blocked = 0;
+    *path = 257;
+    const int rc = f8 || g_gemm_variant == 1 ? 1 : dfd_gemm256e_try(a, c_dtype, epi_p, st);
+    if (rc == 1) {
+      dfd_set_error("dfd_gemm: DFD_GEMM_C_BLOCKED / DFD_GEMM_A_BLOCKED: the ping-pong kernel does not serve this call (bf16, N %% 256 == 0, "
+                    "K %% 128 == 0, K >= 384, ld %% 64 == 0, BIAS_QUICKGELU / BIAS_GELU for C, BIAS for A; got M=%lld N=%d K=%d)",
+                    (long long)a.M, a.N, a.K);
+      return DFD_ERR_INVALID_ARG;
+    }
+    if (rc == 0 && (a.c_blocked || a.a_blocked)) ++g_pair_launches;
+    return rc;
+  }
   int rc = g_gemm_variant == 1 ? 1 : (f8 ? dfd_gemm256e_f8_try : dfd_gemm256e_try)(a, c_dtype, epi_p, st);
   *path = 257;
   if (rc != 1) return rc;
diff --git a/dfd-clip_amd/csrc/gemm256e.hip b/dfd-clip_amd/csrc/gemm256e.hip
--- a/dfd-clip_amd/csrc/gemm256e.hip
+++ b/dfd-clip_amd/csrc/gemm256e.hip
@@ -9,7 +9,7 @@
 constexpr int DEPTH = 6;
 constexpr int NB = 2 * (DEPTH - 1);
 
-template <int EPI, int RB, bool F8, bool CF8>
+template <int EPI, int RB, bool F8, bool CF8, bool ABLK = false>
 __global__ __launch_bounds__(512) void gemm256e_kernel(const GemmArgs a, int tiles_m, int tiles_n) {
   static_assert(!F8 || RB == 8, "fp8 form: 256-row tiles only");
   static_assert(!CF8 || (F8 && EPI != DFD_EPI_QKV_EXPORT), "fp8 output: fp8 operands, plain, QuickGELU or GELU epilogue");
@@ -20,6 +20,9 @@
   constexpr int NCV = F8 ? 2 : 1;
   constexpr int S1 = CF8 ? RB : 2 * RB;
   constexpr int S2 = 4 * RB;
+  static_assert(!ABLK || (!F8 && EPI == DFD_EPI_BIAS), "blocked A: bf16 operands, plain epilogue");
+  constexpr bool C_BLK = !F8 && (EPI == DFD_EPI_BIAS_QUICKGELU || EPI == DFD_EPI_BIAS_GELU);
+  constexpr bool A_BLK = ABLK;
   __shared__ __attribute__((aligned(1024))) unsigned char smem[RING + 8 * STAGE];
   const int tid = threadIdx.x;
   const int lane = tid & 63;
@@ -31,7 +34,7 @@
   const int xcd = bid & 7, q8 = G >> 3, r8 = G & 7;
   const int pos = xcd_position();
 
-  const OperandSrds<F8, CF8> srd(a);
+  const OperandSrds<F8, CF8, A_BLK, C_BLK> srd(a);
   const __amdgpu_buffer_rsrc_t srdA = srd.A, srdW = srd.W, srdC = srd.C;
   const v4i srdB = words(a.bias ? a.bias : reinterpret_cast<const float*>(a.W), a.bias ? a.N * 4 : 0);
   [[maybe_unused]] const v4i srdS = words(F8 ? a.col_scale : reinterpret_cast<const float*>(a.W), F8 ? a.N * 4 : 0);
@@ -40,15 +43,25 @@
 
   const uint32_t lda2 = (uint32_t)(a.lda * ESZ), ldw2 = (uint32_t)(a.ldw * ESZ);
   const uint32_t a_last = (uint32_t)(a.M - 1) * lda2;
+  constexpr bool a_blk = A_BLK;
+  constexpr int a_kstep = a_blk ? (int)DFD_BLK_UNIT : ROWB;
   uint32_t vA[2][2], vW[2];
   auto set_a = [&](const Tile& t, int ha) {
     int l = lane;
     asm volatile("" : "+v"(l));
     const uint32_t pr = (uint32_t)(l >> 3), pp = (uint32_t)(l & 7);
-    const uint32_t ch0 = (pp ^ (pr >> 1)) << 4;
-    const uint32_t row0 = ((uint32_t)t.m0 + (uint32_t)(WROWS * (wave >> 2) + 64 * ha + 16 * (wave & 3))) * lda2 + pr * lda2;
-    vA[ha][0] = min(row0, a_last) + ch0;
-    vA[ha][1] = min(row0 + 8u * lda2, a_last) + (ch0 ^ 64u);
+    if constexpr (a_blk) {
+      const uint32_t c0 = pp ^ (pr >> 1);
+      const uint32_t r0 = (uint32_t)t.m0 + (uint32_t)(WROWS * (wave >> 2) + 64 * ha + 16 * (wave & 3)) + pr;
+      const uint32_t m_last = (uint32_t)(a.M - 1);
+      vA[ha][0] = dfd_blk_row(min(r0, m_last), lda2) + dfd_blk_chunk(c0);
+      vA[ha][1] = dfd_blk_row(min(r0 + 8u, m_last), lda2) + dfd_blk_chunk(c0 ^ 4u);
+    } else {
+      const uint32_t ch0 = (pp ^ (pr >> 1)) << 4;
+      const uint32_t row0 = ((uint32_t)t.m0 + (uint32_t)(WROWS * (wave >> 2) + 64 * ha + 16 * (wave & 3))) * lda2 + pr * lda2;
+      vA[ha][0] = min(row0, a_last) + ch0;
+      vA[ha][1] = min(row0 + 8u * lda2, a_last) + (ch0 ^ 64u);
+    }
   };
   auto set_w = [&](const Tile& t, int hb) {
     int l = lane;
@@ -60,8 +73,8 @@
   auto issue = [&](int kind, int kr) {
     unsigned char* d = smem + ((kind & 1) ? 0 : 4 * UNIT) + (2 * (kind >> 1) + (kr & 1)) * UNIT + wave * 16 * ROWB;
     if (kind & 1) {
-      __builtin_amdgcn_raw_ptr_buffer_load_lds(srdA, (lds_ptr_t)d, 16, vA[kind >> 1][0], kr * ROWB, 0, 0);
-      __builtin_amdgcn_raw_ptr_buffer_load_lds(srdA, (lds_ptr_t)(d + 8 * ROWB), 16, vA[kind >> 1][1], kr * ROWB, 0, 0);
+      __builtin_amdgcn_raw_ptr_buffer_load_lds(srdA, (lds_ptr_t)d, 16, vA[kind >> 1][0], kr * a_kstep, 0, 0);
+      __builtin_amdgcn_raw_ptr_buffer_load_lds(srdA, (lds_ptr_t)(d + 8 * ROWB), 16, vA[kind >> 1][1], kr * a_kstep, 0, 0);
     } else {
       __builtin_amdgcn_raw_ptr_buffer_load_lds(srdW, (lds_ptr_t)d, 16, vW[kind >> 1], kr * ROWB, 0, 0);
       __builtin_amdgcn_raw_ptr_buffer_load_lds(srdW, (lds_ptr_t)(d + 8 * ROWB), 16, vW[kind >> 1] ^ 64u, kr * ROWB + 8 * (int)ldw2, 0, 0);
@@ -307,7 +320,7 @@
       if constexpr (F8) cs4[j] = *reinterpret_cast<const f32x4*>(ep + 256 + (j * 16 + (le >> 4) * 4) * 4);
     }
     asm volatile("s_waitcnt lgkmcnt(0)" ::: "memory");
-    const int stores = tile_epilogue<EPI, RB, F8, CF8>(a, acc, b4, cs4, ep, cur, wr, wc, le, D, srdC);
+    const int stores = tile_epilogue<EPI, RB, F8, CF8, C_BLK>(a, acc, b4, cs4, ep, cur, wr, wc, le, D, srdC);
     if (!has_next) break;
     s_prev = countable_stores<RB>(stores, cur, wr, a.M);
     idx = nidx;
@@ -368,6 +381,7 @@
 struct Gemm256e {
   static constexpr const char* name = "ping-pong";
   static constexpr bool spare_if_free = true;
+  static constexpr bool blocked_layout = true;
   static constexpr bool serves(int epi, bool f8) {
     return epi == DFD_EPI_BIAS || epi == DFD_EPI_BIAS_QUICKGELU || epi == DFD_EPI_BIAS_GELU || epi == DFD_EPI_QKV_EXPORT || (!f8 && epi == DFD_EPI_RESIDUAL_POS);
   }
@@ -381,7 +395,13 @@
   }
   template <int EPI, int RB, bool F8, bool CF8>
   static void run(int grid, hipStream_t st, const GemmArgs& a, int tiles_m, int tiles_n) {
-    hipLaunchKernelGGL((gemm256e_kernel<EPI, RB, F8, CF8>), dim3(grid), dim3(512), 0, st, a, tiles_m, tiles_n);
+    if constexpr (!F8 && EPI == DFD_EPI_BIAS) {
+      if (a.a_blocked) {
+        hipLaunchKernelGGL((gemm256e_kernel<EPI, RB, F8, CF8, true>), dim3(grid), dim3(512), 0, st, a, tiles_m, tiles_n);
+        return;
+      }
+    }
+    hipLaunchKernelGGL((gemm256e_kernel<EPI, RB, F8, CF8, false>), dim3(grid), dim3(512), 0, st, a, tiles_m, tiles_n);
   }
 };
 
@@ -389,4 +409,6 @@
 
 int dfd_gemm256e_try(const GemmArgs& a, int c_dtype, int epi, hipStream_t st) { return try_persistent<Gemm256e, false>(a, c_dtype, epi, st); }
 
+int dfd_gemm256e_serves(const GemmArgs& a, int c_dtype, int epi) { return persistent_serves<Gemm256e, false>(a, c_dtype, epi) == 0; }
+
 int dfd_gemm256e_f8_try(const GemmArgs& a, int c_dtype, int epi, hipStream_t st) { return try_persistent<Gemm256e, true>(a, c_dtype, epi, st); }
diff --git a/dfd-clip_amd/csrc/gemm256p.hip b/dfd-clip_amd/csrc/gemm256p.hip
--- a/dfd-clip_amd/csrc/gemm256p.hip
+++ b/dfd-clip_amd/csrc/gemm256p.hip
@@ -298,6 +298,7 @@
 struct Gemm256p {
   static constexpr const char* name = "persistent";
   static constexpr bool spare_if_free = false;
+  static constexpr bool blocked_layout = false;
   static constexpr bool serves(int epi, bool f8) {
     return epi == DFD_EPI_BIAS || epi == DFD_EPI_BIAS_QUICKGELU || epi == DFD_EPI_QKV_EXPORT || (f8 && epi == DFD_EPI_BIAS_GELU);
   }
diff --git a/dfd-clip_amd/csrc/gemm256p_common.hpp b/dfd-clip_amd/csrc/gemm256p_common.hpp
--- a/dfd-clip_amd/csrc/gemm256p_common.hpp
+++ b/dfd-clip_amd/csrc/gemm256p_common.hpp
@@ -4,6 +4,7 @@
 #include "gemm_args.hpp"
 
 #include "gelu.hpp"
+#include "gemm_blocked.hpp"
 
 typedef int v4i_t __attribute__((ext_vector_type(4)));
 typedef v4i_t v4i;
@@ -73,17 +74,19 @@
   const uint64_t u = reinterpret_cast<uint64_t>(p);
   return v4i{(int)(uint32_t)u, (int)((uint32_t)(u >> 32) & 0xffffu), bytes, 0x00020000};
 }
-template <bool F8, bool CF8>
+template <bool F8, bool CF8, bool ABLK = false, bool CBLK = false>
 struct OperandSrds {
   __amdgpu_buffer_rsrc_t A, W, C;
   __device__ __forceinline__ explicit OperandSrds(const GemmArgs& a)
-      : A(make_srd(a.A, a.M * a.lda * (F8 ? 1 : 2))), W(make_srd(a.W, (int64_t)a.N * a.ldw * (F8 ? 1 : 2))), C(make_srd(a.C, a.M * a.ldc * (CF8 ? 1 : 2))) {}
+      : A(make_srd(a.A, rows(a.M, ABLK && a.a_blocked) * a.lda * (F8 ? 1 : 2))), W(make_srd(a.W, (int64_t)a.N * a.ldw * (F8 ? 1 : 2))),
+        C(make_srd(a.C, rows(a.M, CBLK && a.c_blocked) * a.ldc * (CF8 ? 1 : 2))) {}
+  static __device__ __forceinline__ int64_t rows(int64_t M, bool blocked) { return blocked ? (M + 15) & ~(int64_t)15 : M; }
 };
 template <int RB> __device__ __forceinline__ int countable_stores(int stores, const Tile& t, int wr, int64_t M) {
   return (int64_t)t.m0 + (wr + 1) * 16 * RB <= M ? stores : 0;
 }
 
-template <int EPI, int RB, bool F8, bool CF8>
+template <int EPI, int RB, bool F8, bool CF8, bool BLK = false>
 __device__ __forceinline__ int tile_epilogue(const GemmArgs& a, f32x4 (&acc)[RB][4], const f32x4 (&b4)[4], const f32x4 (&cs4)[4], unsigned char* const ep,
                                              const Tile& cur, int wr, int wc, int le, int D, __amdgpu_buffer_rsrc_t srdC) {
   constexpr int WROWS = 16 * RB;
@@ -263,6 +266,26 @@
         store_out(d, srdC, off, a.stream_out);
       }
     }
+  } else if (BLK && a.c_blocked) {
+    const int row0 = wr * WROWS + er;
+    const int rows_left_b = (int)min((int64_t)0x7fffffff, a.M - ((int64_t)cur.m0 + row0));
+    const uint32_t ldc2 = (uint32_t)(a.ldc * 2);
+    const uint32_t cbase = dfd_blk_row((uint32_t)cur.m0 + (uint32_t)row0, ldc2) + (uint32_t)(nb >> 6) * DFD_BLK_UNIT + (uint32_t)eq * 16u;
+#pragma unroll
+    for (int i = 0; i < RB; ++i) {
+#pragma unroll
+      for (int s = 0; s < 2; ++s) {
+        const f32x4 v0 = activate(acc[i][2 * s]), v1 = activate(acc[i][2 * s + 1]);
+        bf16x8 o;
+#pragma unroll
+        for (int e = 0; e < 4; ++e) {
+          o[e] = (bf16_t)v0[e];
+          o[4 + e] = (bf16_t)v1[e];
+        }
+        const uint32_t off = i * 16 < rows_left_b ? cbase + (uint32_t)i * (ldc2 * 16u) + (uint32_t)s * 1024u : 0xffffffffu;
+        store_out(__builtin_bit_cast(v4i, o), srdC, off, a.stream_out);
+      }
+    }
   } else {
     unsigned char* const park = ep + er * 128 + ((eq ^ ((er & 7) << 1)) << 3);
     const unsigned char* const dsrc = ep + drow * 128 + ((dc ^ drow) << 4);
@@ -347,13 +370,16 @@
 }
 
 inline int check_persistent(const GemmArgs& a, int esz, int csz, int kstep) {
-  if (a.N % TN != 0 || a.K % kstep != 0 || a.M < 1024) return 1;
+  if (a.N % TN != 0 || a.K % kstep != 0 || (a.M < 1024 && !a.pair)) return 1;
   if ((a.lda * esz) % 16 != 0 || (a.ldw * esz) % 16 != 0 || (a.ldc * csz) % 16 != 0) return 1;
   if ((reinterpret_cast<uintptr_t>(a.A) & 15) != 0 || (reinterpret_cast<uintptr_t>(a.W) & 15) != 0 || (reinterpret_cast<uintptr_t>(a.C) & 15) != 0) return 1;
   if (a.bias && (reinterpret_cast<uintptr_t>(a.bias) & 15) != 0) return 1;
   const int64_t lim = (int64_t)0xfffffff0;
-  if (a.M * a.lda * esz > lim || (int64_t)a.N * a.ldw * esz > lim || a.M * a.ldc * csz > lim) return 1;
+  const int64_t Mr = a.pair ? (a.M + 15) & ~(int64_t)15 : a.M;
+  if (Mr * a.lda * esz > lim || (int64_t)a.N * a.ldw * esz > lim || Mr * a.ldc * csz > lim) return 1;
   if ((int64_t)((a.M + 223) / 224) * (a.N / TN) > 0x3fffffff || a.M >= ((int64_t)1 << 31)) return 1;
+  if ((a.c_blocked || a.a_blocked) && (esz != 2 || csz != 2)) return 1;
+  if ((a.c_blocked && a.ldc % 64 != 0) || (a.a_blocked && a.lda % 64 != 0)) return 1;
   return 0;
 }
 
@@ -372,12 +398,23 @@
 }
 
 template <class L, bool F8>
-int try_persistent(const GemmArgs& a_in, int c_dtype, int epi, hipStream_t st) {
+int persistent_serves(const GemmArgs& a_in, int c_dtype, int epi) {
   if (c_dtype != DFD_BF16 && !(F8 && c_dtype == DFD_FP8)) return 1;
   const bool cf8 = c_dtype == DFD_FP8;
   constexpr int esz = F8 ? 1 : 2, kstep = F8 ? 128 : TK;
   if (F8 && (!a_in.col_scale || (reinterpret_cast<uintptr_t>(a_in.col_scale) & 15) != 0)) return 1;
   if (check_persistent(a_in, esz, cf8 ? 1 : 2, kstep) || !L::depth_ok(a_in, esz, a_in.K / kstep, epi)) return 1;
+  if (!L::serves(epi, F8)) return 1;
+  if ((a_in.c_blocked || a_in.a_blocked) && !L::blocked_layout) return 1;
+  if (a_in.c_blocked && epi != DFD_EPI_BIAS_QUICKGELU && epi != DFD_EPI_BIAS_GELU) return 1;
+  if (a_in.a_blocked && epi != DFD_EPI_BIAS) return 1;
+  return 0;
+}
+
+template <class L, bool F8>
+int try_persistent(const GemmArgs& a_in, int c_dtype, int epi, hipStream_t st) {
+  if (persistent_serves<L, F8>(a_in, c_dtype, epi)) return 1;
+  const bool cf8 = c_dtype == DFD_FP8;
   GemmArgs a = a_in;
   auto go = [&](auto epi_c) -> int {
     constexpr int EPI = decltype(epi_c)::value;
diff --git a/dfd-clip_amd/csrc/gemm_args.hpp b/dfd-clip_amd/csrc/gemm_args.hpp
--- a/dfd-clip_amd/csrc/gemm_args.hpp
+++ b/dfd-clip_amd/csrc/gemm_args.hpp
@@ -25,10 +25,12 @@
   uint32_t* sched;
   uint32_t sched_base[8];
   int no_dynamic;
+  int c_blocked, a_blocked, pair;
 };
 
 int dfd_gemm256_try(const GemmArgs& a, int c_dtype, int epi, hipStream_t st);
 int dfd_gemm256e_try(const GemmArgs& a, int c_dtype, int epi, hipStream_t st);
+int dfd_gemm256e_serves(const GemmArgs& a, int c_dtype, int epi);
 int dfd_gemm256e_f8_try(const GemmArgs& a, int c_dtype, int epi, hipStream_t st);
 int dfd_gemm256p_try(const GemmArgs& a, int c_dtype, int epi, hipStream_t st);
 int dfd_gemm256p_f8_try(const GemmArgs& a, int c_dtype, int epi, hipStream_t st);
diff --git a/dfd-clip_amd/csrc/gemm_blocked.hpp b/dfd-clip_amd/csrc/gemm_blocked.hpp
--- /dev/null
+++ b/dfd-clip_amd/csrc/gemm_blocked.hpp
@@ -0,0 +1,15 @@
+#pragma once
+#include <cstdint>
+
+#if defined(__HIPCC__) || defined(__CUDACC__)
+#define DFD_BLK_FN __host__ __device__ __forceinline__
+#else
+#define DFD_BLK_FN inline
+#endif
+
+constexpr uint32_t DFD_BLK_UNIT = 2048;
+
+DFD_BLK_FN uint32_t dfd_blk_row(uint32_t r, uint32_t ld_bytes) { return (r >> 4) * (ld_bytes * 16u) + (r & 15u) * 64u; }
+DFD_BLK_FN uint32_t dfd_blk_chunk(uint32_t c) { return (c & 1u) * 1024u + (c >> 1) * 16u; }
+
+DFD_BLK_FN uint32_t dfd_blk_true_channel(uint32_t c) { return (c & ~60u) | ((c & 12u) << 2) | ((c & 48u) >> 2); }
diff --git a/dfd-clip_amd/encoder.py b/dfd-clip_amd/encoder.py
--- a/dfd-clip_amd/encoder.py
+++ b/dfd-clip_amd/encoder.py
@@ -3,7 +3,7 @@
 import torch
 from torch import nn
 
-from . import capi
+from . import blocked, capi
 
 
 FP8_PRESETS = ("all", "proj-bf16", "kv-bf16", "kv+proj-bf16", "edges-bf16", "none")
@@ -267,7 +267,22 @@
         if dev.type != "cuda":
             raise capi.DfdError("the encoder runs on HIP kernels only: move the model to a GPU (.to('cuda'))")
         self._prepared = self._stage(dev)
+        self._stage_blocked_fc(self._prepared)
         return self._prepared
+
+    def _stage_blocked_fc(self, p):
+        if self.act_dtype != torch.bfloat16:
+            return
+        for bp in p["blocks"]:
+            H = bp["w_fc"].shape[0]
+            if H % 64 == 0 and bp["w_proj"].shape[1] == H:
+                idx = blocked.fc_channel_perm(H, device=bp["w_fc"].device)
+                bp["w_fc_blk"], bp["b_fc_blk"] = bp["w_fc"][idx].contiguous(), bp["b_fc"][idx].contiguous()
+
+    def _pair_blocked(self, bp, M, pl=_NONE):
+        if "w_fc_blk" not in bp or not self.deferred_residual or pl["fc"] == "fp8" or pl["proj"] == "fp8":
+            return False
+        return capi.gemm_pair_plan(M, self.width, bp["w_fc"].shape[0])
 
     def _stage(self, dev):
         act = self.act_dtype
@@ -395,12 +410,12 @@
                                     delta2=ws["delta2"][:M] if pend == 2 else None, store_x=not discard_x)
             ws["pending"] = 0
 
-    def _residual(self, ws, a, w, b, M, spare_cus=0, spare_if_free=False):
+    def _residual(self, ws, a, w, b, M, spare_cus=0, spare_if_free=False, a_blocked=False):
         if self.deferred_residual:
             pend = ws.get("pending", 0)
             assert pend < 2
             capi.gemm(a, w, ws["delta2" if pend else "delta"], b, capi.EPI_BIAS, m=M, stream_out=self.stream_out["proj" if pend else "out"],
-                      spare_cus=spare_cus, spare_if_free=spare_if_free)
+                      spare_cus=spare_cus, spare_if_free=spare_if_free, a_blocked=a_blocked)
             ws["pending"] = pend + 1
         else:
             capi.gemm(a, w, ws["x"], b, capi.EPI_BIAS_RESIDUAL, m=M)
@@ -463,10 +478,13 @@
             self._ln(ws, bp["ln2"], M, store=False)
             if calib is not None:
                 calib.append(ws["h"][:M].abs().max())
-            capi.gemm(ws["h"], bp["w_fc"], ws["u"], bp["b_fc"], self.act_epilogue, m=M, stream_out=so["fc"], spare_cus=sp_fc, spare_if_free=free)
+            blk = self._pair_blocked(bp, M, pl)
+            w_fc, b_fc = (bp["w_fc_blk"], bp["b_fc_blk"]) if blk else (bp["w_fc"], bp["b_fc"])
+            capi.gemm(ws["h"], w_fc, ws["u"], b_fc, self.act_epilogue, m=M, stream_out=so["fc"], spare_cus=sp_fc, spare_if_free=free,
+                      c_blocked=blk)
             if calib is not None:
-                calib.append(ws["u"][:M].abs().max())
-            self._residual(ws, ws["u"], bp["w_proj"], bp["b_proj"], M, spare_cus=sp_proj, spare_if_free=free)
+                calib.append((blocked.unpack(ws["u"][:blocked.padded_rows(M)], M) if blk else ws["u"][:M]).abs().max())
+            self._residual(ws, ws["u"], bp["w_proj"], bp["b_proj"], M, spare_cus=sp_proj, spare_if_free=free, a_blocked=blk)
 
     @torch.no_grad()
     def forward(self, x, with_out=False, with_q=False):
diff --git a/include/dfdclip.h b/include/dfdclip.h
--- a/include/dfdclip.h
+++ b/include/dfdclip.h
@@ -53,6 +53,8 @@
 enum {
   DFD_GEMM_STREAM_OUT = 1,
   DFD_GEMM_SPARE_IF_FREE = 2,
+  DFD_GEMM_C_BLOCKED = 4,
+  DFD_GEMM_A_BLOCKED = 8,
   DFD_GEMM_TILE_BLOCKS_SHIFT = 16,
   DFD_GEMM_SPARE_CUS_SHIFT = 8
 };
diff --git a/include/dfdclip_hooks.h b/include/dfdclip_hooks.h
--- a/include/dfdclip_hooks.h
+++ b/include/dfdclip_hooks.h
@@ -1,5 +1,7 @@
 #ifndef DFDCLIP_HOOKS_H
 #define DFDCLIP_HOOKS_H
+
+#include <stdint.h>
 
 #ifdef __cplusplus
 extern "C" {
@@ -7,6 +9,10 @@
 
 int dfd_attention_set_variant(int variant);
 
+int dfd_gemm_pair_set_variant(int variant);
+int dfd_gemm_pair_plan(int64_t M, int D, int H);
+int64_t dfd_gemm_pair_launches(void);
+
 #ifdef __cplusplus
 }
 #endif
```

New measurement: 881.8, median of 6. +1.1%, better.
